# apple/ml-unigen

Measured on AMD Instinct MI355X. Metric: train-step samples/s (1.5B, 256^2 img), higher is better.
Workload: dtype bf16

## Files before the change

### include/unigen_hip.h

```cpp
#ifndef UNIGEN_HIP_H
#define UNIGEN_HIP_H

#include <stdint.h>
#include <hip/hip_runtime_api.h>

#ifdef __cplusplus
extern "C" {
#endif

#define UG_ABI_VERSION 7

const char* ug_last_error(void);
int ug_abi_version(void);

typedef struct ug_handle ug_handle;
int ug_create(ug_handle** out);
int ug_destroy(ug_handle* h);

#define UG_EPI_BF16 0
#define UG_EPI_F32 1
#define UG_EPI_RESID 2
int ug_gemm_bf16(const ug_handle* h, const void* A, int64_t lda, int a_kmajor, const void* B, int64_t ldb, int b_kmajor,
                 void* C, int64_t ldc, int64_t M, int64_t N, int64_t K, int epilogue, const void* bias,
                 const float* resid, int64_t ldr, int beta, const float* alpha_dev, int policy, hipStream_t stream);
#define UG_GEMM_NARROW_EPILOGUE 0x100
#define UG_GEMM_ONE_BARRIER 0x200
#define UG_GEMM_TWO_BARRIERS 0x400
#define UG_GEMM_POLICY_AUTO_BITS 0xff

int ug_cast_f32_bf16(const float* in, void* out, int64_t n, hipStream_t stream);

int ug_gemm_bf16_swiglu_bwd(const ug_handle* h, const void* dy, int64_t ld_dy, const void* w_down, int64_t ldw, const void* gu,
                            int64_t ld_gu, void* dgu, int64_t ld_dgu, int64_t M, int64_t I, int64_t K, hipStream_t stream);
int ug_gemm_set_fused_tile_height(int rows);
int ug_gemm_bf16_qkv_rope(const ug_handle* h, const void* x, int64_t ldx, const void* w, int64_t ldw, const void* bias, void* qkv,
                          int64_t ldq, int64_t M, int64_t N, int64_t K, const float* cos_tab, const float* sin_tab, int64_t L,
                          int64_t rope_cols, int head_dim, hipStream_t stream);
int ug_gemm_bf16_swiglu(const ug_handle* h, const void* x, int64_t ldx, const void* w_gate_up, int64_t ldw, void* gu,
                        int64_t ld_gu, void* act, int64_t ld_act, int64_t M, int64_t I, int64_t K, hipStream_t stream);

int ug_gemm_bf16_wgrad_group(int n, const void* const* dy, const int64_t* ld_dy, const void* const* x, const int64_t* ld_x,
                             float* const* dw, const int64_t* ld_dw, const int64_t* rows, const int64_t* cols,
                             const int* beta, const int64_t* K, hipStream_t stream);

int ug_rmsnorm_fwd(const float* x, const float* w, void* y, float* rstd, int64_t rows, int64_t cols,
                   float eps, int out_f32, hipStream_t stream);
int ug_rmsnorm_bwd(const void* dy, const float* x, const float* rstd, const float* w, float* dres,
                   float* dw, void* dres_bf16, int64_t rows, int64_t cols, hipStream_t stream);
int ug_rope(void* qkv, const float* cos_tab, const float* sin_tab, int64_t tokens, int64_t L, int64_t ldq,
            int nheads, int head_dim, int backward, hipStream_t stream);
int ug_swiglu_fwd(const void* gate_up, void* act, int64_t tokens, int64_t I, hipStream_t stream);
int ug_swiglu_bwd(const void* gate_up, const void* dact, void* dgate_up, int64_t tokens, int64_t I,
                  hipStream_t stream);
int ug_gelu(const void* x, const void* dy_or_null, void* out, int64_t n, hipStream_t stream);
int ug_embed_fwd(const int64_t* ids, const float* W, float* out, int64_t tokens, int64_t H, int64_t V,
                 int* err_flag, hipStream_t stream);
int ug_embed_bwd(const int64_t* ids, const float* dout, float* dW, int64_t tokens, int64_t H, int64_t V,
                 hipStream_t stream);
int ug_embed_bwd_sorted(const int64_t* ids_sorted, const int64_t* order, const float* rows, float* dW, int64_t n,
                        int64_t H, int64_t V, float scale, hipStream_t stream);
int ug_gather_rows_bf16(const void* in, int64_t ld_in, const int64_t* idx, void* out, int64_t ld_out,
                        int64_t n, int64_t C, int scatter, hipStream_t stream);
int ug_colsum_bf16(const void* in, int64_t ld, float* out, int64_t R, int64_t C, hipStream_t stream);

#define UG_MASK_F32 0
#define UG_MASK_BF16 1
#define UG_MASK_I64 2
#define UG_MASK_BOOL 3
int ug_attn_mask_compress(const void* mask, int mask_dtype, int64_t stride_b, int64_t stride_row,
                          uint64_t* bits, uint8_t* tileany, int64_t B, int64_t L, int* err_flag,
                          hipStream_t stream);
int ug_attn_mask_causal(const uint8_t* key_valid , uint64_t* bits, uint8_t* tileany,
                        int64_t B, int64_t L, hipStream_t stream);
int ug_attn_fwd(const void* q, const void* k, const void* v, int64_t ldq, void* o,
                int64_t ldo, float* lse, const uint64_t* bits, const uint8_t* tileany, int64_t B, int64_t L,
                int64_t Lp, int H, int HKV, int head_dim, float scale, hipStream_t stream);
int ug_attn_bwd(const void* q, const void* k, const void* v, int64_t ldq,
                const void* o, const void* dout, int64_t ldo, const float* lse,
                float* delta, void* dq, void* dk, void* dv, int64_t ldg, const uint64_t* bits,
                const uint8_t* tileany, int64_t B, int64_t L, int64_t Lp, int H, int HKV, int head_dim,
                float scale, float* dkv_ws, const float* rope_cos, const float* rope_sin, float* dbias_qkv, hipStream_t stream);

int ug_kv_store(const void* qkv, int64_t ldq, int64_t k_col, int64_t v_col, void* cache_k, void* cache_v,
                int64_t rows, int64_t L, int HKV, int head_dim, int64_t Tmax, const int* pos_dev, int pos_host,
                hipStream_t stream);
int ug_rope_at(void* qkv, const float* cos_tab, const float* sin_tab, int64_t rows, int64_t ldq, int nheads,
               int head_dim, const int* pos_dev, int64_t max_pos, hipStream_t stream);
int ug_attn_decode(const void* q, int64_t ldq, const void* cache_k, const void* cache_v, const uint8_t* key_valid,
                   void* o, int64_t ldo, int64_t rows, int H, int HKV, int head_dim, int64_t Tmax,
                   const int* len_dev, float scale, hipStream_t stream);
int ug_attn_prefill_cached(const void* q, int64_t ldq, const void* cache_k, const void* cache_v,
                           const uint8_t* key_valid , void* o, int64_t ldo,
                           int64_t rows, int64_t S, int64_t P, int H, int HKV, int head_dim, int64_t Tmax,
                           float scale, hipStream_t stream);
int ug_gemv_bf16(const void* x, int64_t ldx, int64_t R, const void* W, int64_t ldw, float* acc, int64_t acc_stride_r,
                 int64_t acc_stride_n, int64_t N, int64_t K, hipStream_t stream);
int ug_decode_finish_resid_norm(float* acc, int64_t ldacc, float* x, const float* w, void* xn, int64_t rows, int64_t cols,
                                float eps, int* pos_inc, int* len_inc, hipStream_t stream);
int ug_decode_gemv(const void* x, int64_t ldx, int64_t R, const void* W, int64_t ldw, float* acc, int64_t ldacc, int64_t N,
                   int64_t K, float* zero0, int64_t n0, float* zero1, int64_t n1, float* ss_zero, hipStream_t stream);
int ug_decode_gemv_resid_norm(const float* x_in, const float* pending, int64_t ld_pending, const float* norm_w, float* x_out,
                              float* ss_out, int64_t R, const void* W, int64_t ldw, float* acc, int64_t ldacc, int64_t N,
                              int64_t K, float* zero0, int64_t n0, float* zero1, int64_t n1, float* ss_zero,
                              hipStream_t stream);
int ug_decode_gemv_swiglu(const float* gate_up_acc, int64_t ld_gu, const float* ss_in, float eps, int64_t norm_cols, int64_t R,
                          const void* W, int64_t ldw, float* acc, int64_t ldacc, int64_t N, int64_t K, float* zero0, int64_t n0,
                          float* zero1, int64_t n1, float* ss_zero, hipStream_t stream);
int ug_attn_decode_fused(const float* acc_qkv, int64_t ldacc, const float* ss_in, float eps, int64_t norm_cols, const void* bias,
                         const float* cos_tab, const float* sin_tab, const int* pos_dev, void* cache_k, void* cache_v,
                         const uint8_t* key_valid, void* o, int64_t ldo, int64_t rows, int H, int HKV, int head_dim,
                         int64_t Tmax, int64_t max_pos, float scale, hipStream_t stream);
int ug_decode_sw_supported(int64_t hidden, int64_t inter, int64_t q_dim, int head_dim);
int ug_decode_sw_kblock(const void* x, int64_t ldx, int64_t R, const void* W, int64_t ldw, float* acc, int64_t ldacc, int64_t N, int64_t K,
                        float* zero0, int64_t n0, float* zero1, int64_t n1, float* ss_zero, hipStream_t stream);
int ug_decode_sw_resid(const void* x, int64_t ldx, int64_t R, const void* W, int64_t ldw, int64_t N, int64_t K, float* h,
                       hipStream_t stream);
int ug_decode_sw_gate_up(const float* h, const float* pend, int64_t ld_pend, float* x_out, const float* norm_w, float eps, int64_t R,
                         int64_t H, const void* W, int64_t ldw, int64_t I, void* act, int64_t ld_act, hipStream_t stream);
int ug_decode_sw_head(const float* h, const float* pend, int64_t ld_pend, float* x_out, const float* norm_w, float eps, int64_t R,
                      int64_t H, const void* W, int64_t ldw, int64_t N, float* logits, int64_t ld_logits, int* pos_inc, int* len_inc,
                      hipStream_t stream);
int ug_skinny_finish(const float* acc, const void* bias, void* out_bf16, float* resid, int64_t M, int64_t N,
                     int mode, hipStream_t stream);
int ug_gemv_bf16_ord(const void* x, int64_t ldx, int64_t R, const void* W, int64_t ldw, float* part, int64_t ldpart, int64_t part_stride,
                     int64_t N, int64_t K, hipStream_t stream);
int ug_skinny_finish_ord(const float* parts, int64_t nparts, int64_t part_stride, const void* bias, void* out_bf16, float* out_f32,
                         float* resid, int64_t M, int64_t N, hipStream_t stream);
int ug_decode_gemv_resid_norm_ord(const float* x_in, const float* pend_parts, int64_t ld_pending, int64_t npend, const float* norm_w,
                                  float* x_out, float* ss_part, int64_t R, const void* W, int64_t ldw, float* part, int64_t ldpart,
                                  int64_t N, int64_t K, hipStream_t stream);
int ug_attn_decode_fused_ord(const float* qkv_part, int64_t ldpart, int64_t nparts, const float* ss_part, float eps, int64_t norm_cols,
                             const void* bias, const float* cos_tab, const float* sin_tab, const int* pos_dev, void* cache_k,
                             void* cache_v, const uint8_t* key_valid, void* o, int64_t ldo, int64_t rows, int H, int HKV, int head_dim,
                             int64_t Tmax, int64_t max_pos, float scale, hipStream_t stream);
int ug_decode_sw_kblock_ord(const void* x, int64_t ldx, int64_t R, const void* W, int64_t ldw, float* part, int64_t ldpart, int64_t N,
                            int64_t K, hipStream_t stream);
int ug_decode_finish_resid_norm_ord(const float* parts, int64_t ldp, int64_t nparts, float* x, const float* w, void* xn, int64_t rows,
                                    int64_t cols, float eps, int* pos_inc, int* len_inc, hipStream_t stream);

int ug_t2i_assemble(const int64_t* text_ids, const int64_t* text_offsets, const int64_t* conv_start, int64_t n_start,
                    const int64_t* conv_end, int64_t n_end, const int64_t* image_in, const int64_t* image_labels, int64_t B,
                    int64_t n_image, int64_t max_seq_len, int64_t pad_id, int64_t soi_id, int64_t eoi_id, int64_t ignore_id,
                    int64_t* input_ids, int64_t* labels, uint8_t* attn01, hipStream_t stream);
int ug_attn_mask_from_ids(const int64_t* ids, int64_t B, int64_t L, int64_t pad_id, int64_t soi_id, int64_t eoi_id, int mode,
                          int* meta_ws, uint8_t* flags_ws, uint64_t* bits, uint8_t* tileany, hipStream_t stream);

int ug_maskgit_train_mask(const int64_t* tokens, const float* scores, const float* num_masked, int64_t B, int64_t n,
                          int64_t mask_id, int64_t ignore_id, int64_t* input_ids, int64_t* labels, hipStream_t stream);

int ug_maskgit_step(const void* logits, int64_t ld, int64_t V, int64_t N, int64_t n, int cfg, float guidance_scale,
                    const float* u_sample, const float* u_conf, const int64_t* cur_ids, int64_t mask_id, int64_t id_offset,
                    int64_t mask_len_sched, float temperature, int64_t* sampled, float* sel_ws, int64_t* next_cur,
                    int64_t* next_ids, uint8_t* masking_out, hipStream_t stream);

int ug_maskgit_step_ex(const void* logits, int64_t ld, int64_t V, int64_t N, int64_t n, int cfg, float guidance_scale,
                       const float* u_sample, const float* u_conf, const int64_t* cur_ids, int64_t mask_id, int64_t id_offset,
                       int64_t mask_len_sched, float temperature, float sample_temperature, int64_t top_k, float top_p, float min_p,
                       int64_t* sampled, float* sel_ws, int64_t* next_cur, int64_t* next_ids, uint8_t* masking_out, float* logp,
                       float* stats, hipStream_t stream);

int ug_ar_sample(float* acc, int64_t ldacc, int64_t bsz, int64_t V, float guidance_scale, float temperature, int greedy,
                 const float* uniforms, const int* pos_dev, int64_t pos0, int64_t nsteps, const float* embed, int64_t ld_embed,
                 int64_t H, int64_t id_offset, int64_t* tok, int* out_tokens, float* x, hipStream_t stream);

int ug_ar_sample_filtered(float* acc, int64_t ldacc, int64_t bsz, int64_t V, float guidance_scale, float temperature, int greedy,
                          const float* uniforms, const int* pos_dev, int64_t pos0, int64_t nsteps, const float* embed,
                          int64_t ld_embed, int64_t H, int64_t id_offset, int64_t* tok, int* out_tokens, float* x, int64_t top_k,
                          float top_p, float min_p, float* stats, hipStream_t stream);

int ug_ar_sample_logp(float* acc, int64_t ldacc, int64_t bsz, int64_t V, float guidance_scale, float temperature, int greedy,
                      const float* uniforms, const int* pos_dev, int64_t pos0, int64_t nsteps, const float* embed, int64_t ld_embed,
                      int64_t H, int64_t id_offset, int64_t* tok, int* out_tokens, float* x, float* logp, hipStream_t stream);
int ug_ar_sample_filtered_logp(float* acc, int64_t ldacc, int64_t bsz, int64_t V, float guidance_scale, float temperature, int greedy,
                               const float* uniforms, const int* pos_dev, int64_t pos0, int64_t nsteps, const float* embed,
                               int64_t ld_embed, int64_t H, int64_t id_offset, int64_t* tok, int* out_tokens, float* x, int64_t top_k,
                               float top_p, float min_p, float* stats, float* logp, hipStream_t stream);

int ug_text_pick(float* logits, int64_t ld, int64_t R, int64_t V, int clear, const int64_t* stop_ids, int64_t n_stop, int64_t pad_id,
                 const float* embed, int64_t ld_embed, int64_t embed_rows, int64_t H, int* state, int64_t nsteps, int64_t* tok,
                 int* out_tokens, int* lengths, float* x, hipStream_t stream);

int ug_text_sample_workspace_ints(int64_t R);

int ug_text_sample(float* logits, int64_t ld, int64_t R, int64_t V, int clear, float temperature, int64_t top_k, float top_p,
                   const float* uniforms, int* workspace, float* stats, const int64_t* stop_ids, int64_t n_stop, int64_t pad_id,
                   const float* embed, int64_t ld_embed, int64_t embed_rows, int64_t H, int* state, int64_t nsteps, int64_t* tok,
                   int* out_tokens, int* lengths, float* x, hipStream_t stream);

int ug_text_pick_logp(float* logits, int64_t ld, int64_t R, int64_t V, int clear, const int64_t* stop_ids, int64_t n_stop, int64_t pad_id,
                      const float* embed, int64_t ld_embed, int64_t embed_rows, int64_t H, int* state, int64_t nsteps, int64_t* tok,
                      int* out_tokens, int* lengths, float* x, float* logp, hipStream_t stream);
int ug_text_sample_logp(float* logits, int64_t ld, int64_t R, int64_t V, int clear, float temperature, int64_t top_k, float top_p,
                        const float* uniforms, int* workspace, float* stats, const int64_t* stop_ids, int64_t n_stop, int64_t pad_id,
                        const float* embed, int64_t ld_embed, int64_t embed_rows, int64_t H, int* state, int64_t nsteps, int64_t* tok,
                        int* out_tokens, int* lengths, float* x, float* logp, hipStream_t stream);


int ug_text_seen_mark(int* seen, int64_t ld_words, const int64_t* ids, int64_t ld_ids, int64_t R, int64_t L, const uint8_t* valid,
                      int64_t V, hipStream_t stream);

int ug_text_penalize(float* logits, int64_t ld, int64_t R, int64_t V, float penalty, int* seen, int64_t ld_words, const int64_t* tok,
                     hipStream_t stream);


int ug_text_constrain(float* logits, int64_t ld, int64_t R, int64_t V, const void* bias, int64_t n_bias, int64_t min_new,
                      const int64_t* stop_ids, int64_t n_stop, int64_t ngram, const int* hist, int64_t ld_hist, const int* hist_len,
                      const int* out_tokens, int64_t nsteps, const int* state, hipStream_t stream);

int ug_text_stop_seq(const int* seq_ids, const int* seq_off, int64_t ns, int64_t n_ids, const int* out_tokens, int64_t nsteps, int64_t R,
                     int* state, int* lengths, hipStream_t stream);

int ug_ce_fwd(const void* logits, int64_t ld, int64_t R, int64_t V, const int64_t* labels,
              int64_t ignore_index, float* lse, float* loss_row, float* logp_label, float* loss_and_count,
              hipStream_t stream);
int ug_ce_bwd(void* logits_inout, int64_t ld, int64_t R, int64_t V, const int64_t* labels,
              int64_t ignore_index, const float* lse, const float* loss_and_count, const float* gscale,
              const float* row_scale, hipStream_t stream);

int ug_head_score_ws_bytes(int64_t R, int64_t V);
int ug_head_score(const void* x, int64_t ldx, int64_t R, const void* W, int64_t ldw, int64_t V, int64_t K,
                  const int64_t* labels, int64_t ignore_index, void* ws, float* logp, float* lse, int64_t* best, float* best_logit,
                  hipStream_t stream);

int ug_adamw_flat(float* p, const float* g, float* m, float* v, void* p_bf16, int64_t n, float lr,
                  float beta1, float beta2, float eps, float weight_decay, int64_t step, float grad_scale,
                  int max_blocks ,
                  hipStream_t stream);
int ug_adamw_flat_dev(float* p, const float* g, float* m, float* v, void* p_bf16, int64_t n, float lr,
                      float beta1, float beta2, float eps, float weight_decay, int64_t step, float grad_scale,
                      const float* grad_factor, int max_blocks, hipStream_t stream);

int ug_sumsq_spans_f32(const int64_t* spans, int64_t n_spans, double* partials, int blocks, int accum, hipStream_t stream);
int ug_clip_finish(const double* partials, int64_t n_partials, float max_norm, float grad_scale, float* result, hipStream_t stream);
int ug_scale_spans_f32(const int64_t* spans, int64_t n_spans, const float* coef, int blocks, hipStream_t stream);

int ug_grad_pack_bf16(const float* in, void* out_bf16, int64_t n, float scale, hipStream_t stream);
int ug_zero_ranges_f32(float* buf, const int64_t* ranges, int64_t n_ranges, int64_t max_len, hipStream_t stream);
int ug_grad_unpack_bf16(const void* in_bf16, float* out, int64_t n, hipStream_t stream);
int ug_grad_sum_shards_bf16(const void* shards_bf16, int world, int64_t stride, void* out_bf16, int64_t n, float scale,
                            hipStream_t stream);

typedef struct ug_comm ug_comm;
#define UG_COMM_ID_BYTES 128
#define UG_COMM_FP32 0
#define UG_COMM_BF16_FP32ACC 1
#define UG_COMM_BF16 2
#define UG_COMM_FP32_RSAG 3
int ug_comm_unique_id(void* id128);
int ug_comm_init(ug_comm** out, int world, int rank, const void* id128, int64_t max_bucket_elems);
int ug_comm_allreduce_bucket(ug_comm* comm, float* grad, int64_t n, int mode, hipStream_t producer);
int ug_comm_allgather(ug_comm* comm, const void* send, void* recv, int64_t bytes_per_rank, hipStream_t producer);
int ug_comm_wait(ug_comm* comm, hipStream_t consumer);
int ug_comm_destroy(ug_comm* comm);
int64_t ug_comm_bytes_on_wire(const ug_comm* comm);

int ug_conv2d_f32(const float* x, const float* w_packed, const float* bias, const float* residual, float* y,
                  int64_t B, int Hin, int Win, int Cin, int Cout, int cout_pad, int ksize, int stride,
                  int pad_top, int pad_left, int Hout, int Wout, int upsample2x, hipStream_t stream);
int ug_conv_split_weights(const float* w_packed, uint16_t* w_split, int taps, int Cin, int cout_pad, hipStream_t stream);
int ug_amax_f32(const float* x, int64_t rows, int64_t cols, int64_t ld, float* out_amax, hipStream_t stream);
int ug_amax_f32_into_zeroed(const float* x, int64_t rows, int64_t cols, int64_t ld, float* out_amax, hipStream_t stream);
int ug_conv2d_split(const float* x, const float* x_amax, const uint16_t* w_split, const float* bias, const float* residual,
                    float* y, int64_t B, int Hin, int Win, int Cin, int Cout, int cout_pad, int ksize, int stride,
                    int pad_top, int pad_left, int Hout, int Wout, int upsample2x, double* out_stats, int out_groups,
                    hipStream_t stream);
int ug_conv3x3_split(const float* x, const float* x_amax, const uint16_t* w_split, const float* bias, const float* residual,
                     float* y, int64_t B, int H, int W, int Cin, int Cout, int cout_pad, const float* gn_mu_rstd,
                     const float* gn_gamma, const float* gn_beta, int gn_groups, int gn_swish, double* out_stats, int out_groups,
                     hipStream_t stream);
int ug_groupnorm_finalize(const double* stats, float* mu_rstd, int64_t B, int64_t HW, int C, int groups, float eps,
                          hipStream_t stream);
int ug_groupnorm_stats(const float* x, double* stats_ws, float* mu_rstd, int64_t B, int64_t HW, int C, int groups,
                       float eps, hipStream_t stream);
int ug_siglip_attn_f32(const float* qkv, int64_t ld, const float* qkv_amax, float* out, int64_t ldo, int64_t B, int64_t T,
                       int H, int head_dim, float scale, hipStream_t stream);
int ug_linear_split(const float* x, int64_t ldx, const float* x_amax, const uint16_t* w_split, const float* bias,
                    const float* residual, int64_t ldres, float* y, int64_t ldy, int64_t M, int64_t N, int64_t K, int n_pad,
                    int act, hipStream_t stream);
int ug_gemm_f32(const float* A, int64_t lda, int64_t stride_a, const float* B, int64_t ldb, int64_t stride_b,
                int b_is_nk, float* C, int64_t ldc, int64_t stride_c, int64_t M, int64_t N, int64_t K,
                int64_t batch, float alpha, hipStream_t stream);
int ug_gemm_f32_nested(const float* A, int64_t lda, int64_t sa_in, int64_t sa_out, const float* B, int64_t ldb,
                       int64_t sb_in, int64_t sb_out, int b_is_nk, float* C, int64_t ldc, int64_t sc_in, int64_t sc_out,
                       int64_t M, int64_t N, int64_t K, int64_t batch_in, int64_t batch_out, float alpha,
                       hipStream_t stream);
int ug_groupnorm_swish(const float* x, const float* gamma, const float* beta, float* y, double* stats_ws,
                       int64_t B, int64_t HW, int C, int groups, float eps, int apply_swish, hipStream_t stream);
int ug_softmax_rows_f32(float* x, int64_t rows, int64_t cols, int64_t ld, float scale, hipStream_t stream);
int ug_linear_f32(const float* x, int64_t ldx, const float* W, int64_t ldw, const float* bias,
                  const float* residual, int64_t ldres, float* y, int64_t ldy, int64_t M, int64_t N, int64_t K,
                  int act, hipStream_t stream);
int ug_layernorm_f32(const float* x, const float* gamma, const float* beta, float* y, int64_t rows, int64_t cols,
                     float eps, hipStream_t stream);
int ug_layernorm_bwd_f32(const float* dy, const float* x, const float* gamma, const float* dres_in, float* dx, float* dgamma,
                         float* dbeta, int64_t rows, int64_t cols, float eps, hipStream_t stream);
int ug_gelu_tanh_f32(const float* pre, const float* dy_or_null, float* out, int64_t n, hipStream_t stream);
int ug_softmax_bwd_rows_f32(const float* P, float* dP, int64_t rows, int64_t cols, int64_t ld, float scale, hipStream_t stream);
int ug_colsum_f32(const float* x, int64_t ld, float* out, int64_t rows, int64_t cols, hipStream_t stream);
int ug_transpose_f32(const float* in, int64_t ld_in, int64_t stride_in, float* out, int64_t ld_out, int64_t stride_out,
                     int64_t rows, int64_t cols, int64_t batch, hipStream_t stream);
int ug_nchw_to_nhwc(const float* in, float* out, int64_t B, int C, int64_t HW, int c_pad, hipStream_t stream);
int ug_nhwc_to_nchw(const float* in, float* out, int64_t B, int C, int64_t HW, int c_pad, hipStream_t stream);
int ug_lfq_pack(const float* z, int64_t ldz, int64_t* idx, int64_t n, int nbits, hipStream_t stream);
int ug_lfq_unpack(const int64_t* idx, float* z, int64_t n, int nbits, int* err_flag, hipStream_t stream);

int ug_probe_layouts(float* out, int64_t n_floats, hipStream_t stream);

#ifdef __cplusplus
}
#endif
#endif
```

### ml-unigen_amd/csrc/elementwise.hip

```cpp
#include <algorithm>
#include "common.h"
#include "unigen_hip.h"

namespace {

typedef unsigned int ntu4_t __attribute__((ext_vector_type(4)));
typedef unsigned int ntu2_t __attribute__((ext_vector_type(2)));
template <int NT, typename T>
__device__ __forceinline__ T ld_stream(const T* p) {
  static_assert(sizeof(T) == 16 || sizeof(T) == 8, "ld_stream: 8- or 16-byte accesses");
  if constexpr ((NT & 2) && sizeof(T) == 16) return __builtin_bit_cast(T, __builtin_nontemporal_load(reinterpret_cast<const ntu4_t*>(p)));
  else if constexpr ((NT & 2) && sizeof(T) == 8) return __builtin_bit_cast(T, __builtin_nontemporal_load(reinterpret_cast<const ntu2_t*>(p)));
  else return *p;
}
template <int NT, typename T>
__device__ __forceinline__ void st_stream(T* p, T v) {
  static_assert(sizeof(T) == 16 || sizeof(T) == 8, "st_stream: 8- or 16-byte accesses");
  if constexpr ((NT & 1) && sizeof(T) == 16) __builtin_nontemporal_store(__builtin_bit_cast(ntu4_t, v), reinterpret_cast<ntu4_t*>(p));
  else if constexpr ((NT & 1) && sizeof(T) == 8) __builtin_nontemporal_store(__builtin_bit_cast(ntu2_t, v), reinterpret_cast<ntu2_t*>(p));
  else *p = v;
}
constexpr int NT_ADAMW = 3, NT_RMSNORM_BWD = 0, NT_SWIGLU_BWD = 3, NT_SWIGLU_FWD = 2;

template <bool OUT_F32>
__global__ __launch_bounds__(256) void rmsnorm_fwd_kernel(const float* __restrict__ x, const float* __restrict__ w,
                                                          void* __restrict__ y, float* __restrict__ rstd,
                                                          int rows, int cols, float eps) {
  const int row = blockIdx.x * 4 + (threadIdx.x >> 6);
  const int lane = threadIdx.x & 63;
  if (row >= rows) return;
  const float4* xr = reinterpret_cast<const float4*>(x + (int64_t)row * cols);
  const int nv = cols >> 2;
  float ss = 0.f;
  for (int i = lane; i < nv; i += 64) {
    const float4 v = xr[i];
    ss += v.x * v.x + v.y * v.y + v.z * v.z + v.w * v.w;
  }
  ss = wave_sum(ss);
  const float r = rsqrtf(ss / (float)cols + eps);
  if (lane == 0 && rstd) rstd[row] = r;
  const float4* wr = reinterpret_cast<const float4*>(w);
  for (int i = lane; i < nv; i += 64) {
    const float4 v = xr[i], g = wr[i];
    const float o0 = g.x * (v.x * r), o1 = g.y * (v.y * r), o2 = g.z * (v.z * r), o3 = g.w * (v.w * r);
    if constexpr (OUT_F32) {
      reinterpret_cast<float4*>(reinterpret_cast<float*>(y) + (int64_t)row * cols)[i] = make_float4(o0, o1, o2, o3);
    } else {
      uint2 o; o.x = pack_bf2(o0, o1); o.y = pack_bf2(o2, o3);
      reinterpret_cast<uint2*>(reinterpret_cast<bf16_t*>(y) + (int64_t)row * cols)[i] = o;
    }
  }
}

template <bool OUT_F32, int NV>
__global__ __launch_bounds__(256) void rmsnorm_fwd_reg_kernel(const float* __restrict__ x, const float* __restrict__ w,
                                                              void* __restrict__ y, float* __restrict__ rstd,
                                                              int rows, int cols, float eps, int rows_per_wave) {
  const int lane = threadIdx.x & 63;
  const int nv = cols >> 2;
  const float4* wr = reinterpret_cast<const float4*>(w);
  const int r0 = (blockIdx.x * 4 + (threadIdx.x >> 6)) * rows_per_wave;
  for (int row = r0; row < min(rows, r0 + rows_per_wave); ++row) {
    const float4* xr = reinterpret_cast<const float4*>(x + (int64_t)row * cols);
    float4 v[NV];
    float ss = 0.f;
#pragma unroll
    for (int k = 0; k < NV; ++k) {
      const int i = lane + k * 64;
      if (i < nv) { v[k] = xr[i]; }
    }
#pragma unroll
    for (int k = 0; k < NV; ++k) {
      const int i = lane + k * 64;
      if (i < nv) ss += v[k].x * v[k].x + v[k].y * v[k].y + v[k].z * v[k].z + v[k].w * v[k].w;
    }
    ss = wave_sum(ss);
    const float r = rsqrtf(ss / (float)cols + eps);
    if (lane == 0 && rstd) rstd[row] = r;
#pragma unroll
    for (int k = 0; k < NV; ++k) {
      const int i = lane + k * 64;
      if (i < nv) {
        const float4 g = wr[i];
        const float o0 = g.x * (v[k].x * r), o1 = g.y * (v[k].y * r), o2 = g.z * (v[k].z * r), o3 = g.w * (v[k].w * r);
        if constexpr (OUT_F32) {
          reinterpret_cast<float4*>(reinterpret_cast<float*>(y) + (int64_t)row * cols)[i] = make_float4(o0, o1, o2, o3);
        } else {
          uint2 o; o.x = pack_bf2(o0, o1); o.y = pack_bf2(o2, o3);
          reinterpret_cast<uint2*>(reinterpret_cast<bf16_t*>(y) + (int64_t)row * cols)[i] = o;
        }
      }
    }
  }
}

constexpr int RN_MAXV = 8;
template <int NV, int NT>
__global__ __launch_bounds__(256) void rmsnorm_bwd_kernel(const bf16_t* __restrict__ dy, const float* __restrict__ x,
                                                          const float* __restrict__ rstd, const float* __restrict__ w,
                                                          float* __restrict__ dres, float* __restrict__ dw,
                                                          bf16_t* __restrict__ dres_bf16, int rows, int cols,
                                                          int rows_per_block) {
  __shared__ float red[4][64 * 4];
  const int wave = threadIdx.x >> 6, lane = threadIdx.x & 63;
  const int nv = cols >> 2;
  float4 dwp[NV];
#pragma unroll
  for (int k = 0; k < NV; ++k) dwp[k] = make_float4(0.f, 0.f, 0.f, 0.f);
  const float4* wr = reinterpret_cast<const float4*>(w);
  const int r0 = blockIdx.x * rows_per_block;
  const int r1 = min(rows, r0 + rows_per_block);
  for (int row = r0 + wave; row < r1; row += 4) {
    const float4* xr = reinterpret_cast<const float4*>(x + (int64_t)row * cols);
    const uint2* dyr = reinterpret_cast<const uint2*>(dy + (int64_t)row * cols);
    float4* dr = reinterpret_cast<float4*>(dres + (int64_t)row * cols);
    const float r = rstd[row];
    float4 g[NV], xh[NV], acc[NV];
    uint2 dyv[NV];
    float dot = 0.f;
#pragma unroll
    for (int k = 0; k < NV; ++k) {
      const int i = lane + k * 64;
      if (i < nv) { xh[k] = ld_stream<NT>(xr + i); dyv[k] = ld_stream<NT>(dyr + i); }
    }
#pragma unroll
    for (int k = 0; k < NV; ++k) {
      const int i = lane + k * 64;
      if (i < nv) acc[k] = dr[i];
    }
#pragma unroll
    for (int k = 0; k < NV; ++k) {
      const int i = lane + k * 64;
      if (i < nv) {
        const float4 v = xh[k], ww = wr[i]; const uint2 d = dyv[k];
        const float d0 = bf2f(d.x & 0xffff), d1 = bf2f(d.x >> 16), d2 = bf2f(d.y & 0xffff), d3 = bf2f(d.y >> 16);
        xh[k] = make_float4(v.x * r, v.y * r, v.z * r, v.w * r);
        g[k] = make_float4(d0 * ww.x, d1 * ww.y, d2 * ww.z, d3 * ww.w);
        dot += g[k].x * xh[k].x + g[k].y * xh[k].y + g[k].z * xh[k].z + g[k].w * xh[k].w;
        dwp[k].x += d0 * xh[k].x; dwp[k].y += d1 * xh[k].y; dwp[k].z += d2 * xh[k].z; dwp[k].w += d3 * xh[k].w;
      }
    }
    dot = wave_sum(dot) / (float)cols;
#pragma unroll
    for (int k = 0; k < NV; ++k) {
      const int i = lane + k * 64;
      if (i < nv) {
        float4 o = acc[k];
        o.x += r * (g[k].x - xh[k].x * dot); o.y += r * (g[k].y - xh[k].y * dot);
        o.z += r * (g[k].z - xh[k].z * dot); o.w += r * (g[k].w - xh[k].w * dot);
        st_stream<NT>(dr + i, o);
        if (dres_bf16) {
          uint2 ob; ob.x = pack_bf2(o.x, o.y); ob.y = pack_bf2(o.z, o.w);
          reinterpret_cast<uint2*>(dres_bf16 + (int64_t)row * cols)[i] = ob;
        }
      }
    }
  }
#pragma unroll
  for (int k = 0; k < NV; ++k) {
    if (k * 64 >= nv) break;
    __syncthreads();
    red[wave][lane * 4 + 0] = dwp[k].x; red[wave][lane * 4 + 1] = dwp[k].y;
    red[wave][lane * 4 + 2] = dwp[k].z; red[wave][lane * 4 + 3] = dwp[k].w;
    __syncthreads();
    const int c = threadIdx.x;
    const int col = k * 256 + c;
    if constexpr (!(NT & 4))
      if (col < cols) atomicAdd(dw + col, red[0][c] + red[1][c] + red[2][c] + red[3][c]);
  }
}

template <bool BWD>
__global__ __launch_bounds__(256) void rope_kernel(bf16_t* __restrict__ qkv, const float* __restrict__ cs,
                                                   const float* __restrict__ sn, int64_t tokens, int L, int ldq,
                                                   int nheads, int hd) {
#pragma clang fp contract(off)
  const int half = hd >> 1, per_head = half >> 2;
  const int64_t total = tokens * nheads * per_head;
  for (int64_t idx = blockIdx.x * (int64_t)blockDim.x + threadIdx.x; idx < total; idx += (int64_t)gridDim.x * blockDim.x) {
    const int p4 = (int)(idx % per_head);
    const int h = (int)((idx / per_head) % nheads);
    const int64_t t = idx / ((int64_t)per_head * nheads);
    const int pos = (int)(t % L);
    bf16_t* base = qkv + t * ldq + h * hd + p4 * 4;
    const uint2 lo = *reinterpret_cast<const uint2*>(base);
    const uint2 hi = *reinterpret_cast<const uint2*>(base + half);
    const float4 c = *reinterpret_cast<const float4*>(cs + (int64_t)pos * half + p4 * 4);
    const float4 s = *reinterpret_cast<const float4*>(sn + (int64_t)pos * half + p4 * 4);
    const float x1[4] = {bf2f(lo.x & 0xffff), bf2f(lo.x >> 16), bf2f(lo.y & 0xffff), bf2f(lo.y >> 16)};
    const float x2[4] = {bf2f(hi.x & 0xffff), bf2f(hi.x >> 16), bf2f(hi.y & 0xffff), bf2f(hi.y >> 16)};
    const float cc[4] = {c.x, c.y, c.z, c.w}, ss[4] = {s.x, s.y, s.z, s.w};
    float o1[4], o2[4];
#pragma unroll
    for (int k = 0; k < 4; ++k) {
      const float a1 = x1[k] * cc[k], a2 = x2[k] * cc[k];
      const float b1 = x2[k] * ss[k], b2 = x1[k] * ss[k];
      if constexpr (!BWD) { o1[k] = a1 - b1; o2[k] = a2 + b2; }
      else { o1[k] = a1 + b1; o2[k] = a2 - b2; }
    }
    uint2 olo, ohi;
    olo.x = pack_bf2(o1[0], o1[1]); olo.y = pack_bf2(o1[2], o1[3]);
    ohi.x = pack_bf2(o2[0], o2[1]); ohi.y = pack_bf2(o2[2], o2[3]);
    *reinterpret_cast<uint2*>(base) = olo;
    *reinterpret_cast<uint2*>(base + half) = ohi;
  }
}

__device__ __forceinline__ float silu_f(float g) { return silu_train(g); }

template <int NT>
__global__ __launch_bounds__(256) void swiglu_fwd_kernel(const bf16_t* __restrict__ gu, bf16_t* __restrict__ act,
                                                         int64_t tokens, int I) {
  const int per_row = I >> 3;
  const int64_t total = tokens * per_row;
  for (int64_t idx = blockIdx.x * (int64_t)blockDim.x + threadIdx.x; idx < total; idx += (int64_t)gridDim.x * blockDim.x) {
    const int64_t t = idx / per_row; const int c = (int)(idx % per_row) * 8;
    const bf16x8_t g = ld_stream<NT>(reinterpret_cast<const bf16x8_t*>(gu + t * 2 * I + c));
    const bf16x8_t u = ld_stream<NT>(reinterpret_cast<const bf16x8_t*>(gu + t * 2 * I + I + c));
    bf16x8_t o;
#pragma unroll
    for (int k = 0; k < 8; ++k) {
      const float s = bf2f(f2bf(silu_f(bf2f((bf16_t)g[k]))));
      o[k] = (short)f2bf(s * bf2f((bf16_t)u[k]));
    }
    st_stream<NT>(reinterpret_cast<bf16x8_t*>(act + t * I + c), o);
  }
}

template <int NT>
__global__ __launch_bounds__(256) void swiglu_bwd_kernel(const bf16_t* __restrict__ gu, const bf16_t* __restrict__ dact,
                                                         bf16_t* __restrict__ dgu, int64_t tokens, int I) {
  const int per_row = I >> 3;
  const int64_t total = tokens * per_row;
  for (int64_t idx = blockIdx.x * (int64_t)blockDim.x + threadIdx.x; idx < total; idx += (int64_t)gridDim.x * blockDim.x) {
    const int64_t t = idx / per_row; const int c = (int)(idx % per_row) * 8;
    const bf16x8_t g = ld_stream<NT>(reinterpret_cast<const bf16x8_t*>(gu + t * 2 * I + c));
    const bf16x8_t u = ld_stream<NT>(reinterpret_cast<const bf16x8_t*>(gu + t * 2 * I + I + c));
    const bf16x8_t d = ld_stream<NT>(reinterpret_cast<const bf16x8_t*>(dact + t * I + c));
    bf16x8_t og, ou;
#pragma unroll
    for (int k = 0; k < 8; ++k) {
      float dg_, du_;
      swiglu_bwd_elem(bf2f((bf16_t)g[k]), bf2f((bf16_t)u[k]), bf2f((bf16_t)d[k]), dg_, du_);
      ou[k] = (short)f2bf(du_);
      og[k] = (short)f2bf(dg_);
    }
    st_stream<NT>(reinterpret_cast<bf16x8_t*>(dgu + t * 2 * I + c), og);
    st_stream<NT>(reinterpret_cast<bf16x8_t*>(dgu + t * 2 * I + I + c), ou);
  }
}

__global__ __launch_bounds__(256) void gelu_kernel(const bf16_t* __restrict__ x, const bf16_t* __restrict__ dy,
                                                   bf16_t* __restrict__ out, int64_t n8) {
  for (int64_t i = blockIdx.x * (int64_t)blockDim.x + threadIdx.x; i < n8; i += (int64_t)gridDim.x * blockDim.x) {
    const bf16x8_t v = reinterpret_cast<const bf16x8_t*>(x)[i];
    bf16x8_t g, o;
    if (dy) g = reinterpret_cast<const bf16x8_t*>(dy)[i];
#pragma unroll
    for (int k = 0; k < 8; ++k) {
      const float f = bf2f((bf16_t)v[k]);
      const float cdf = 0.5f * (1.f + erff(f * 0.70710678118654752f));
      if (!dy) o[k] = (short)f2bf(f * cdf);
      else o[k] = (short)f2bf(bf2f((bf16_t)g[k]) * (cdf + f * 0.3989422804014327f * __expf(-0.5f * f * f)));
    }
    reinterpret_cast<bf16x8_t*>(out)[i] = o;
  }
}

__global__ __launch_bounds__(256) void embed_fwd_kernel(const int64_t* __restrict__ ids, const float* __restrict__ W,
                                                        float* __restrict__ out, int64_t tokens, int H, int64_t V,
                                                        int* __restrict__ err) {
  const int per_row = H >> 2;
  const int64_t total = tokens * per_row;
  for (int64_t idx = blockIdx.x * (int64_t)blockDim.x + threadIdx.x; idx < total; idx += (int64_t)gridDim.x * blockDim.x) {
    const int64_t t = idx / per_row; const int c = (int)(idx % per_row);
    int64_t id = ids[t];
    if (id < 0 || id >= V) { if (err) atomicOr(err, 1); id = 0; }
    reinterpret_cast<float4*>(out + t * H)[c] = reinterpret_cast<const float4*>(W + id * H)[c];
  }
}

// ... 263 lines not shown
    sh[threadIdx.x] = i < n ? partials[i] : 0.0;
    __syncthreads();
    if (threadIdx.x == 0) {
      const int c = min(256, n - base);
      for (int k = 0; k < c; ++k) s += sh[k];
    }
    __syncthreads();
  }
  if (threadIdx.x == 0) {
    const float total = (float)(sqrt(s) * fabs((double)grad_scale));
    const float raw = max_norm / (total + 1e-6f);
    const float coef = raw > 1.f ? 1.f : raw;
    result[0] = total;
    result[1] = coef;
    result[2] = grad_scale * coef;
    result[3] = (total != total || fabsf(total) == INFINITY) ? 1.f : 0.f;
    reinterpret_cast<double*>(result)[2] = s;
    result[6] = 0.f;
    result[7] = 0.f;
  }
}

__global__ __launch_bounds__(256) void scale_spans_kernel(const int64_t* __restrict__ spans, int n_spans, const float* __restrict__ coef) {
  const float c = *coef;
  if (c == 1.0f) return;
  const int64_t stride = (int64_t)gridDim.x * 256;
  for (int r = 0; r < n_spans; ++r) {
    const SpanGeom sp = span_geom(spans, r);
    const unsigned vb = (blockIdx.x + (unsigned)r) % gridDim.x;
    if (vb == 0) {
      const int64_t t = threadIdx.x;
      const int64_t e = t < sp.head ? t : sp.tail0 + (t - sp.head);
      if (e < sp.n) sp.base[e] *= c;
    }
    for (int64_t i = (int64_t)vb * 256 + threadIdx.x; i < sp.body4; i += stride) {
      sp.body[i] = sp.body[i] * c;
    }
  }
}

__global__ __launch_bounds__(256) void cast_f32_bf16_kernel(const float* __restrict__ in, bf16_t* __restrict__ out, int64_t n) {
  const int64_t n4 = n >> 2;
  for (int64_t i = blockIdx.x * (int64_t)blockDim.x + threadIdx.x; i < n4; i += (int64_t)gridDim.x * blockDim.x) {
    const float4 v = reinterpret_cast<const float4*>(in)[i];
    uint2 o; o.x = pack_bf2(v.x, v.y); o.y = pack_bf2(v.z, v.w);
    reinterpret_cast<uint2*>(out)[i] = o;
  }
  const int64_t ti = (n4 << 2) + blockIdx.x * (int64_t)blockDim.x + threadIdx.x;
  if (ti < n) out[ti] = f2bf(in[ti]);
}

__global__ __launch_bounds__(256) void grad_pack_kernel(const float* __restrict__ in, bf16_t* __restrict__ out, int64_t n, float scale) {
  const int64_t n8 = n >> 3;
  for (int64_t i = blockIdx.x * (int64_t)blockDim.x + threadIdx.x; i < n8; i += (int64_t)gridDim.x * blockDim.x) {
    const float4 a = reinterpret_cast<const float4*>(in)[2 * i], b = reinterpret_cast<const float4*>(in)[2 * i + 1];
    uint4 o;
    o.x = pack_bf2(a.x * scale, a.y * scale); o.y = pack_bf2(a.z * scale, a.w * scale);
    o.z = pack_bf2(b.x * scale, b.y * scale); o.w = pack_bf2(b.z * scale, b.w * scale);
    reinterpret_cast<uint4*>(out)[i] = o;
  }
  const int64_t ti = (n8 << 3) + blockIdx.x * (int64_t)blockDim.x + threadIdx.x;
  if (ti < n) out[ti] = f2bf(in[ti] * scale);
}
__global__ __launch_bounds__(256) void grad_sum_shards_kernel(const bf16_t* __restrict__ shards, int world, int64_t stride,
                                                              bf16_t* __restrict__ out, int64_t n, float scale) {
  const int64_t n8 = n >> 3;
  for (int64_t i = blockIdx.x * (int64_t)blockDim.x + threadIdx.x; i < n8; i += (int64_t)gridDim.x * blockDim.x) {
    float acc[8] = {0.f, 0.f, 0.f, 0.f, 0.f, 0.f, 0.f, 0.f};
    for (int r = 0; r < world; ++r) {
      const uint4 v = reinterpret_cast<const uint4*>(shards + r * stride)[i];
      acc[0] += __uint_as_float(v.x << 16); acc[1] += __uint_as_float(v.x & 0xffff0000u);
      acc[2] += __uint_as_float(v.y << 16); acc[3] += __uint_as_float(v.y & 0xffff0000u);
      acc[4] += __uint_as_float(v.z << 16); acc[5] += __uint_as_float(v.z & 0xffff0000u);
      acc[6] += __uint_as_float(v.w << 16); acc[7] += __uint_as_float(v.w & 0xffff0000u);
    }
    uint4 o;
    o.x = pack_bf2(acc[0] * scale, acc[1] * scale); o.y = pack_bf2(acc[2] * scale, acc[3] * scale);
    o.z = pack_bf2(acc[4] * scale, acc[5] * scale); o.w = pack_bf2(acc[6] * scale, acc[7] * scale);
    reinterpret_cast<uint4*>(out)[i] = o;
  }
  const int64_t ti = (n8 << 3) + blockIdx.x * (int64_t)blockDim.x + threadIdx.x;
  if (ti < n) {
    float a = 0.f;
    for (int r = 0; r < world; ++r) a += bf2f(shards[r * stride + ti]);
    out[ti] = f2bf(a * scale);
  }
}
__global__ __launch_bounds__(256) void grad_unpack_kernel(const bf16_t* __restrict__ in, float* __restrict__ out, int64_t n) {
  const int64_t n8 = n >> 3;
  for (int64_t i = blockIdx.x * (int64_t)blockDim.x + threadIdx.x; i < n8; i += (int64_t)gridDim.x * blockDim.x) {
    const uint4 v = reinterpret_cast<const uint4*>(in)[i];
    float4 a, b;
    a.x = __uint_as_float(v.x << 16); a.y = __uint_as_float(v.x & 0xffff0000u);
    a.z = __uint_as_float(v.y << 16); a.w = __uint_as_float(v.y & 0xffff0000u);
    b.x = __uint_as_float(v.z << 16); b.y = __uint_as_float(v.z & 0xffff0000u);
    b.z = __uint_as_float(v.w << 16); b.w = __uint_as_float(v.w & 0xffff0000u);
    reinterpret_cast<float4*>(out)[2 * i] = a; reinterpret_cast<float4*>(out)[2 * i + 1] = b;
  }
  const int64_t ti = (n8 << 3) + blockIdx.x * (int64_t)blockDim.x + threadIdx.x;
  if (ti < n) out[ti] = bf2f(in[ti]);
}

__global__ __launch_bounds__(256) void gather_rows_kernel(const bf16_t* __restrict__ in, int64_t ld_in,
                                                          const int64_t* __restrict__ idx, bf16_t* __restrict__ out,
                                                          int64_t ld_out, int64_t n, int C, int scatter) {
  const int per_row = C >> 3;
  const int64_t total = n * per_row;
  for (int64_t i = blockIdx.x * (int64_t)blockDim.x + threadIdx.x; i < total; i += (int64_t)gridDim.x * blockDim.x) {
    const int64_t r = i / per_row; const int c = (int)(i % per_row) * 8;
    const int64_t src = scatter ? r : idx[r], dst = scatter ? idx[r] : r;
    *reinterpret_cast<bf16x8_t*>(out + dst * ld_out + c) = *reinterpret_cast<const bf16x8_t*>(in + src * ld_in + c);
  }
}

inline int grid_for(int64_t work_items, int block = 256, int cap = 256 * 8) {
  int64_t g = (work_items + block - 1) / block;
  if (g < 1) g = 1;
  if (g > cap) g = cap;
  return (int)g;
}

}

extern "C" int ug_rmsnorm_fwd(const float* x, const float* w, void* y, float* rstd, int64_t rows, int64_t cols,
                              float eps, int out_f32, hipStream_t st) {
  UG_REQUIRE(rows > 0 && cols > 0 && cols % 4 == 0, "ug_rmsnorm_fwd: cols=%ld must be a positive multiple of 4", (long)cols);
  UG_REQUIRE(ug_aligned16(x) && ug_aligned16(w) && ug_aligned16(y), "ug_rmsnorm_fwd: pointers must be 16B aligned");
  dim3 grid((unsigned)((rows + 3) / 4)), block(256);
  constexpr int reg = 1;
  if (reg > 0 && cols <= 2048 && !out_f32) {
    dim3 g2((unsigned)((rows + 4 * reg - 1) / (4 * reg)));
    hipLaunchKernelGGL((rmsnorm_fwd_reg_kernel<false, 8>), g2, block, 0, st, x, w, y, rstd, (int)rows, (int)cols, eps, reg);
  } else if (out_f32) hipLaunchKernelGGL(rmsnorm_fwd_kernel<true>, grid, block, 0, st, x, w, y, rstd, (int)rows, (int)cols, eps);
  else hipLaunchKernelGGL(rmsnorm_fwd_kernel<false>, grid, block, 0, st, x, w, y, rstd, (int)rows, (int)cols, eps);
  UG_CHECK_LAUNCH("ug_rmsnorm_fwd");
  return UG_OK;
}

extern "C" int ug_rmsnorm_bwd(const void* dy, const float* x, const float* rstd, const float* w, float* dres,
                              float* dw, void* dres_bf16, int64_t rows, int64_t cols, hipStream_t st) {
  UG_REQUIRE(rows > 0 && cols > 0 && cols % 4 == 0 && cols <= 64 * 4 * RN_MAXV,
             "ug_rmsnorm_bwd: cols=%ld unsupported (multiple of 4, <= %d)", (long)cols, 64 * 4 * RN_MAXV);
  UG_REQUIRE(ug_aligned16(x) && ug_aligned16(w) && ug_aligned16(dres) && ((uintptr_t)dy & 7) == 0,
             "ug_rmsnorm_bwd: pointers must be aligned");
  const int rpb = (int)std::max<int64_t>(16, ((rows + 479) / 480 + 3) / 4 * 4);
  dim3 grid((unsigned)((rows + rpb - 1) / rpb)), block(256);
  UG_REQUIRE(((uintptr_t)dres_bf16 & 7) == 0, "ug_rmsnorm_bwd: dres_bf16 must be 8-byte aligned");
  hipLaunchKernelGGL((rmsnorm_bwd_kernel<RN_MAXV, NT_RMSNORM_BWD>), grid, block, 0, st, (const bf16_t*)dy, x, rstd, w, dres, dw,
                     (bf16_t*)dres_bf16, (int)rows, (int)cols, rpb);
  UG_CHECK_LAUNCH("ug_rmsnorm_bwd");
  return UG_OK;
}

extern "C" int ug_rope(void* qkv, const float* cos_tab, const float* sin_tab, int64_t tokens, int64_t L, int64_t ldq,
                       int nheads, int head_dim, int backward, hipStream_t st) {
  UG_REQUIRE(tokens > 0 && L > 0 && tokens % L == 0, "ug_rope: tokens=%ld must be a multiple of L=%ld", (long)tokens, (long)L);
  UG_REQUIRE(head_dim % 8 == 0 && ldq % 4 == 0, "ug_rope: head_dim must be a multiple of 8");
  UG_REQUIRE(((uintptr_t)qkv & 7) == 0 && ug_aligned16(cos_tab) && ug_aligned16(sin_tab), "ug_rope: alignment");
  const int64_t total = tokens * nheads * (head_dim / 8);
  dim3 grid(grid_for(total)), block(256);
  if (backward) hipLaunchKernelGGL(rope_kernel<true>, grid, block, 0, st, (bf16_t*)qkv, cos_tab, sin_tab, tokens, (int)L, (int)ldq, nheads, head_dim);
  else hipLaunchKernelGGL(rope_kernel<false>, grid, block, 0, st, (bf16_t*)qkv, cos_tab, sin_tab, tokens, (int)L, (int)ldq, nheads, head_dim);
  UG_CHECK_LAUNCH("ug_rope");
  return UG_OK;
}

extern "C" int ug_swiglu_fwd(const void* gate_up, void* act, int64_t tokens, int64_t I, hipStream_t st) {
  UG_REQUIRE(tokens > 0 && I % 8 == 0, "ug_swiglu_fwd: I=%ld must be a multiple of 8", (long)I);
  UG_REQUIRE(ug_aligned16(gate_up) && ug_aligned16(act), "ug_swiglu_fwd: alignment");
  dim3 grid(grid_for(tokens * (I / 8))), block(256);
  hipLaunchKernelGGL(swiglu_fwd_kernel<NT_SWIGLU_FWD>, grid, block, 0, st, (const bf16_t*)gate_up, (bf16_t*)act, tokens, (int)I);
  UG_CHECK_LAUNCH("ug_swiglu_fwd");
  return UG_OK;
}

extern "C" int ug_swiglu_bwd(const void* gate_up, const void* dact, void* dgate_up, int64_t tokens, int64_t I,
                             hipStream_t st) {
  UG_REQUIRE(tokens > 0 && I % 8 == 0, "ug_swiglu_bwd: I=%ld must be a multiple of 8", (long)I);
  UG_REQUIRE(ug_aligned16(gate_up) && ug_aligned16(dact) && ug_aligned16(dgate_up), "ug_swiglu_bwd: alignment");
  dim3 grid(grid_for(tokens * (I / 8))), block(256);
  hipLaunchKernelGGL(swiglu_bwd_kernel<NT_SWIGLU_BWD>, grid, block, 0, st, (const bf16_t*)gate_up, (const bf16_t*)dact, (bf16_t*)dgate_up, tokens, (int)I);
  UG_CHECK_LAUNCH("ug_swiglu_bwd");
  return UG_OK;
}

extern "C" int ug_gelu(const void* x, const void* dy_or_null, void* out, int64_t n, hipStream_t st) {
  UG_REQUIRE(n > 0 && n % 8 == 0 && ug_aligned16(x) && ug_aligned16(out), "ug_gelu: n must be a multiple of 8, 16B-aligned buffers");
  dim3 grid(grid_for(n / 8)), block(256);
  hipLaunchKernelGGL(gelu_kernel, grid, block, 0, st, (const bf16_t*)x, (const bf16_t*)dy_or_null, (bf16_t*)out, n / 8);
  UG_CHECK_LAUNCH("ug_gelu");
  return UG_OK;
}

extern "C" int ug_embed_fwd(const int64_t* ids, const float* W, float* out, int64_t tokens, int64_t H, int64_t V,
                            int* err_flag, hipStream_t st) {
  UG_REQUIRE(tokens > 0 && H % 4 == 0, "ug_embed_fwd: H must be a multiple of 4");
  dim3 grid(grid_for(tokens * (H / 4))), block(256);
  hipLaunchKernelGGL(embed_fwd_kernel, grid, block, 0, st, ids, W, out, tokens, (int)H, V, err_flag);
  UG_CHECK_LAUNCH("ug_embed_fwd");
  return UG_OK;
}

extern "C" int ug_embed_bwd(const int64_t* ids, const float* dout, float* dW, int64_t tokens, int64_t H, int64_t V,
                            hipStream_t st) {
  UG_REQUIRE(tokens > 0 && H > 0, "ug_embed_bwd: empty");
  dim3 grid(grid_for(tokens * H)), block(256);
  hipLaunchKernelGGL(embed_bwd_kernel, grid, block, 0, st, ids, dout, dW, tokens, (int)H, V);
  UG_CHECK_LAUNCH("ug_embed_bwd");
  return UG_OK;
}

extern "C" int ug_embed_bwd_sorted(const int64_t* ids_sorted, const int64_t* order, const float* rows, float* dW, int64_t n,
                                   int64_t H, int64_t V, float scale, hipStream_t st) {
  UG_REQUIRE(ids_sorted && order && rows && dW && n > 0 && H > 0 && H % 4 == 0 && n < (1ll << 31) && ug_aligned16(rows) && ug_aligned16(dW),
             "ug_embed_bwd_sorted: need sorted ids, their permutation, 16B-aligned rows / table and H %% 4 == 0");
  hipLaunchKernelGGL(embed_bwd_sorted_kernel, dim3((unsigned)n), dim3(256), 0, st, ids_sorted, order, rows, dW, n, (int)H, V, scale);
  UG_CHECK_LAUNCH("ug_embed_bwd_sorted");
  return UG_OK;
}

extern "C" int ug_colsum_bf16(const void* in, int64_t ld, float* out, int64_t R, int64_t C, hipStream_t st) {
  UG_REQUIRE(R > 0 && C > 0, "ug_colsum_bf16: empty");
  const int rpb = 256;
  dim3 grid((unsigned)((C + 63) / 64), (unsigned)((R + rpb - 1) / rpb)), block(256);
  hipLaunchKernelGGL(colsum_kernel, grid, block, 0, st, (const bf16_t*)in, ld, out, (int)R, (int)C, rpb);
  UG_CHECK_LAUNCH("ug_colsum_bf16");
  return UG_OK;
}

static int adamw_flat_launch(float* p, const float* g, float* m, float* v, void* p_bf16, int64_t n, float lr,
                             float beta1, float beta2, float eps, float weight_decay, int64_t step, float grad_scale,
                             const float* gfac, int max_blocks, hipStream_t st) {
  UG_REQUIRE(n > 0 && step >= 1, "ug_adamw_flat: n=%ld step=%ld", (long)n, (long)step);
  UG_REQUIRE(ug_aligned16(p) && ug_aligned16(g) && ug_aligned16(m) && ug_aligned16(v) && ((uintptr_t)p_bf16 & 7) == 0,
             "ug_adamw_flat: buffers must be 16B aligned");
  const double bc1 = 1.0 - pow((double)beta1, (double)step);
  const double bc2 = 1.0 - pow((double)beta2, (double)step);
  const dim3 block(256);
  if (max_blocks == 0 && n < (1LL << 29)) max_blocks = 256;
  if (max_blocks > 0) {
    dim3 lgrid(grid_for(n / 2 + 1, 256, max_blocks));
    if (n < (1LL << 29))
      hipLaunchKernelGGL(adamw_lean2_kernel<NT_ADAMW>, lgrid, block, 0, st, p, g, m, v, (bf16_t*)p_bf16, (uint32_t)n, lr, beta1, beta2, eps, weight_decay,
                         (float)bc1, (float)sqrt(bc2), grad_scale, gfac);
    else
      hipLaunchKernelGGL(adamw_lean_kernel<NT_ADAMW>, lgrid, block, 0, st, p, g, m, v, (bf16_t*)p_bf16, n, lr, beta1, beta2, eps, weight_decay,
                         (float)bc1, (float)sqrt(bc2), grad_scale, gfac);
    UG_CHECK_LAUNCH("ug_adamw_flat(lean)");
    return UG_OK;
  }
  hipLaunchKernelGGL(adamw_kernel<NT_ADAMW>, dim3(grid_for(n / 4 + 1)), block, 0, st, p, g, m, v, (bf16_t*)p_bf16, n, lr, beta1, beta2, eps,
                     weight_decay, (float)bc1, (float)sqrt(bc2), grad_scale, gfac);
  UG_CHECK_LAUNCH("ug_adamw_flat");
  return UG_OK;
}

extern "C" int ug_adamw_flat(float* p, const float* g, float* m, float* v, void* p_bf16, int64_t n, float lr,
                             float beta1, float beta2, float eps, float weight_decay, int64_t step, float grad_scale,
                             int max_blocks, hipStream_t st) {
  return adamw_flat_launch(p, g, m, v, p_bf16, n, lr, beta1, beta2, eps, weight_decay, step, grad_scale, nullptr, max_blocks, st);
}

extern "C" int ug_adamw_flat_dev(float* p, const float* g, float* m, float* v, void* p_bf16, int64_t n, float lr,
                                 float beta1, float beta2, float eps, float weight_decay, int64_t step, float grad_scale,
                                 const float* grad_factor, int max_blocks, hipStream_t st) {
  UG_REQUIRE(((uintptr_t)grad_factor & 3) == 0, "ug_adamw_flat_dev: grad_factor must be a 4-byte aligned device address (or null)");
  return adamw_flat_launch(p, g, m, v, p_bf16, n, lr, beta1, beta2, eps, weight_decay, step, grad_scale, grad_factor, max_blocks, st);
}

extern "C" int ug_sumsq_spans_f32(const int64_t* spans, int64_t n_spans, double* partials, int blocks, int accum, hipStream_t st) {
  UG_REQUIRE(spans && partials && ((uintptr_t)spans & 7) == 0 && ((uintptr_t)partials & 7) == 0 && n_spans > 0 && n_spans < 65536 &&
                 blocks > 0 && blocks <= 4096 && (accum == 0 || accum == 1),
             "ug_sumsq_spans_f32: a device span table of 1..65535 spans, a partial buffer of `blocks` doubles, 1 <= blocks <= 4096 and "
             "accum 0 (fp64) or 1 (fp32 chains) required (n_spans=%ld blocks=%d accum=%d)", (long)n_spans, blocks, accum);
  if (accum == 0) hipLaunchKernelGGL(sumsq_spans_kernel<false>, dim3((unsigned)blocks), dim3(256), 0, st, spans, (int)n_spans, partials);
  else hipLaunchKernelGGL(sumsq_spans_kernel<true>, dim3((unsigned)blocks), dim3(256), 0, st, spans, (int)n_spans, partials);
  UG_CHECK_LAUNCH("ug_sumsq_spans_f32");
  return UG_OK;
}

extern "C" int ug_clip_finish(const double* partials, int64_t n_partials, float max_norm, float grad_scale, float* result, hipStream_t st) {
  UG_REQUIRE(partials && result && ((uintptr_t)partials & 7) == 0 && ug_aligned16(result) && n_partials > 0 && n_partials <= 8192,
             "ug_clip_finish: 1..8192 fp64 partials and a 16-byte aligned result block of 8 fp32 words required (n_partials=%ld)", (long)n_partials);
  UG_REQUIRE(max_norm == max_norm && grad_scale == grad_scale, "ug_clip_finish: max_norm and grad_scale must not be NaN");
  hipLaunchKernelGGL(clip_finish_kernel, dim3(1), dim3(256), 0, st, partials, (int)n_partials, max_norm, grad_scale, result);
  UG_CHECK_LAUNCH("ug_clip_finish");
  return UG_OK;
}

extern "C" int ug_scale_spans_f32(const int64_t* spans, int64_t n_spans, const float* coef, int blocks, hipStream_t st) {
  UG_REQUIRE(spans && coef && ((uintptr_t)spans & 7) == 0 && ((uintptr_t)coef & 3) == 0 && n_spans > 0 && n_spans < 65536 && blocks >= 0 &&
                 blocks <= 4096,
             "ug_scale_spans_f32: a device span table of 1..65535 spans, a device scalar and 0 <= blocks <= 4096 required (n_spans=%ld blocks=%d)",
             (long)n_spans, blocks);
  hipLaunchKernelGGL(scale_spans_kernel, dim3((unsigned)(blocks ? blocks : 256 * 8)), dim3(256), 0, st, spans, (int)n_spans, coef);
  UG_CHECK_LAUNCH("ug_scale_spans_f32");
  return UG_OK;
}

extern "C" int ug_cast_f32_bf16(const float* in, void* out, int64_t n, hipStream_t st) {
  UG_REQUIRE(n > 0 && ug_aligned16(in) && ((uintptr_t)out & 7) == 0, "ug_cast_f32_bf16: bad args");
  dim3 grid(grid_for(n / 4 + 1)), block(256);
  hipLaunchKernelGGL(cast_f32_bf16_kernel, grid, block, 0, st, in, (bf16_t*)out, n);
  UG_CHECK_LAUNCH("ug_cast_f32_bf16");
  return UG_OK;
}
// ... 52 lines not shown
```

### ml-unigen_amd/csrc/loss.hip

```cpp
#include "common.h"
#include "unigen_hip.h"

namespace {

__global__ __launch_bounds__(256) void ce_fwd_kernel(const bf16_t* __restrict__ logits, int64_t ld, int V,
                                                     const int64_t* __restrict__ labels, int64_t ignore_index,
                                                     float* __restrict__ lse_out, float* __restrict__ loss_row,
                                                     float* __restrict__ logp_label) {
  __shared__ float red[4];
  const int row = blockIdx.x;
  const bf16_t* x = logits + (int64_t)row * ld;
  const int nv = V >> 3;
  float m = -INFINITY, s = 0.f;
  for (int i = threadIdx.x; i < nv; i += 256) {
    const bf16x8_t v = *reinterpret_cast<const bf16x8_t*>(x + i * 8);
    float f[8], mx = -INFINITY;
#pragma unroll
    for (int k = 0; k < 8; ++k) { f[k] = bf2f((bf16_t)v[k]); mx = fmaxf(mx, f[k]); }
    const float mn = fmaxf(m, mx);
    float acc = 0.f;
#pragma unroll
    for (int k = 0; k < 8; ++k) acc += __expf(f[k] - mn);
    s = s * __expf(m - mn) + acc;
    m = mn;
  }
  for (int c = (nv << 3) + threadIdx.x; c < V; c += 256) {
    const float f = bf2f(x[c]);
    const float mn = fmaxf(m, f);
    s = s * __expf(m - mn) + __expf(f - mn);
    m = mn;
  }
  const float M = block_max<4>(m, red);
  const float part = (m == -INFINITY) ? 0.f : s * __expf(m - M);
  const float S = block_sum<4>(part, red);
  if (threadIdx.x == 0) {
    const float lse = M + logf(S);
    lse_out[row] = lse;
    const int64_t lab = labels ? labels[row] : ignore_index;
    float lr = 0.f, lp = 0.f;
    if (lab != ignore_index && lab >= 0 && lab < V) { lp = bf2f(x[lab]) - lse; lr = -lp; }
    if (loss_row) loss_row[row] = lr;
    if (logp_label) logp_label[row] = lp;
  }
}

__global__ __launch_bounds__(256) void ce_reduce_kernel(const float* __restrict__ loss_row,
                                                        const int64_t* __restrict__ labels, int64_t ignore_index,
                                                        int R, float* __restrict__ out) {
  __shared__ float red[4];
  float s = 0.f, c = 0.f;
  for (int i = threadIdx.x; i < R; i += 256) {
    if (labels[i] != ignore_index) { s += loss_row[i]; c += 1.f; }
  }
  const float S = block_sum<4>(s, red);
  const float C = block_sum<4>(c, red);
  if (threadIdx.x == 0) { out[0] = S / C; out[1] = C; }
}

__global__ __launch_bounds__(256) void ce_bwd_kernel(bf16_t* __restrict__ logits, int64_t ld, int V,
                                                     const int64_t* __restrict__ labels, int64_t ignore_index,
                                                     const float* __restrict__ lse, const float* __restrict__ loss_cnt,
                                                     const float* __restrict__ gscale, const float* __restrict__ row_scale) {
  const int row = blockIdx.x;
  bf16_t* x = logits + (int64_t)row * ld;
  const int64_t lab = labels[row];
  const bool valid = (lab != ignore_index);
  const float sc = !valid ? 0.f : row_scale ? row_scale[row] : (gscale ? *gscale : 1.f) / loss_cnt[1];
  const float l = lse[row];
  const int nvp = (int)(ld >> 3);
  for (int i = threadIdx.x; i < nvp; i += 256) {
    bf16x8_t v = *reinterpret_cast<const bf16x8_t*>(x + i * 8);
#pragma unroll
    for (int k = 0; k < 8; ++k) {
      const int c = i * 8 + k;
      float g = 0.f;
      if (valid && c < V) g = (__expf(bf2f((bf16_t)v[k]) - l) - (c == lab ? 1.f : 0.f)) * sc;
      v[k] = (short)f2bf(g);
    }
    *reinterpret_cast<bf16x8_t*>(x + i * 8) = v;
  }
}

}

extern "C" int ug_ce_fwd(const void* logits, int64_t ld, int64_t R, int64_t V, const int64_t* labels,
                         int64_t ignore_index, float* lse, float* loss_row, float* logp_label, float* loss_and_count,
                         hipStream_t st) {
  UG_REQUIRE(R > 0 && V > 0 && ld >= V && ld % 8 == 0, "ug_ce_fwd: need ld>=V and ld%%8==0 (ld=%ld V=%ld)", (long)ld, (long)V);
  UG_REQUIRE(ug_aligned16(logits), "ug_ce_fwd: logits must be 16B aligned");
  hipLaunchKernelGGL(ce_fwd_kernel, dim3((unsigned)R), dim3(256), 0, st, (const bf16_t*)logits, ld, (int)V, labels,
                     ignore_index, lse, loss_row, logp_label);
  UG_CHECK_LAUNCH("ug_ce_fwd");
  if (loss_and_count) {
    UG_REQUIRE(labels && loss_row, "ug_ce_fwd: loss reduction needs labels and loss_row");
    hipLaunchKernelGGL(ce_reduce_kernel, dim3(1), dim3(256), 0, st, loss_row, labels, ignore_index, (int)R, loss_and_count);
    UG_CHECK_LAUNCH("ug_ce_fwd(reduce)");
  }
  return UG_OK;
}

extern "C" int ug_ce_bwd(void* logits_inout, int64_t ld, int64_t R, int64_t V, const int64_t* labels,
                         int64_t ignore_index, const float* lse, const float* loss_and_count, const float* gscale,
                         const float* row_scale, hipStream_t st) {
  UG_REQUIRE(R > 0 && V > 0 && ld >= V && ld % 8 == 0, "ug_ce_bwd: need ld>=V and ld%%8==0");
  UG_REQUIRE(ug_aligned16(logits_inout) && labels && lse && (loss_and_count || row_scale), "ug_ce_bwd: bad pointers");
  hipLaunchKernelGGL(ce_bwd_kernel, dim3((unsigned)R), dim3(256), 0, st, (bf16_t*)logits_inout, ld, (int)V, labels,
                     ignore_index, lse, loss_and_count, gscale, row_scale);
  UG_CHECK_LAUNCH("ug_ce_bwd");
  return UG_OK;
}
```

### ml-unigen_amd/models/unigen.py

```python
import collections
import dataclasses
import json
import math
import os
import time
import weakref
from typing import Optional

import torch

from unigen_hip import ops
from unigen_hip.lib import UniGenHipError
from unigen_hip.modules import (HipProjector, HipQwen2ForCausalLM, LazyLogits, _CrossEntropyFn, _HeadLossFn, _LinearFn,
                                _TableEmbedFn)
from unigen_hip.qwen2 import Qwen2Dims

from .modeling_utils import ConfigMixin, ModelMixin, register_to_config
from .sampling import cosine_schedule, mask_by_random_topk

_KNOWN_LLM = {
    "qwen2.5-1.5b": dict(hidden_size=1536, intermediate_size=8960, num_hidden_layers=28, num_attention_heads=12,
                         num_key_value_heads=2, rope_theta=1000000.0, rms_norm_eps=1e-6, vocab_size=151936),
}

# ... 517 lines not shown
            finally:
                eng.require_grad_sync = prev
        return ctx()

    def _load_hf_llm_weights(self, llm_model_path, ckpt_base_path):
        path = llm_model_path
        if ckpt_base_path and not os.path.exists(str(path)):
            path = os.path.join(ckpt_base_path, os.path.basename(str(llm_model_path).rstrip("/")))
        files = [f for f in os.listdir(path) if f.endswith(".safetensors")]
        if not files:
            raise UniGenHipError(f"no *.safetensors under {path}")
        from safetensors.torch import load_file
        sd = {}
        for f in files:
            sd.update(load_file(os.path.join(path, f)))
        own = self.llm.state_dict()
        V_ckpt = sd["model.embed_tokens.weight"].shape[0]
        with torch.no_grad():
            for k, v in sd.items():
                if k == "lm_head.weight" or k not in own:
                    continue
                if k == "model.embed_tokens.weight":
                    n = min(V_ckpt, own[k].shape[0])
                    own[k][:n].copy_(v[:n])
                else:
                    own[k].copy_(v)

    def _set_gradient_checkpointing(self, module, value=False):
        self.gradient_checkpointing = True

    def resize_token_embeddings(self, vocab_size):
        self.vocab_size = vocab_size
        self.llm.resize_token_embeddings(self.vocab_size)
        self.output_size = self.vocab_size

    def init_vision_tower(self, vision_tower_name):
        from .multimodal_encoder.builder import get_vision_tower
        self.register_to_config(vision_tower_name=vision_tower_name)
        if self.config.ckpt_base_path:
            vision_tower_name = os.path.join(self.config.ckpt_base_path, os.path.basename(vision_tower_name.rstrip("/")))
        self.vision_tower = get_vision_tower(vision_tower_name, freeze=False)

    def add_vision_tower(self, config):
        vision_tower_name = config.model.vision_tower.name
        self.init_vision_tower(vision_tower_name)
        vt = self.vision_tower
        mm_input_dim = vt.config.hidden_size if hasattr(vt, 'config') else vt.hidden_size
        self.add_mm_projector(config.model.unigen.get('und_proj_depth', 2), mm_input_dim)

    def add_mm_projector(self, mlp_depth, mm_input_dim):
        self.register_to_config(w_und_encoder=True)
        self.register_to_config(mm_input_dim=mm_input_dim)
        self.register_to_config(und_proj_depth=mlp_depth)
        hidden = self.config.hidden_size
        layers = [torch.nn.Linear(mm_input_dim, hidden)]
        for _ in range(1, mlp_depth):
            layers += [torch.nn.GELU(), torch.nn.Linear(hidden, hidden)]
        from unigen_hip.modules import HipProjector
        self.mm_projector = HipProjector(*layers).to(self.llm.engine.device)

    def _use_gen(self):
        return self.config.get('gen_proj_depth', 0) > 0

    def get_gen_embed(self, img_tokens):
        if not self._use_gen():
            raise UniGenHipError("get_gen_embed needs a model built with gen_proj_depth > 0")
        eng = self.llm.engine
        e = _TableEmbedFn.apply(self.gen_embed.weight, img_tokens.to(eng.device), eng.err_flag)
        return self.gen_projector(e)

    def prepare_inputs_for_t2i(self, input_ids, num_vq_tokens):
        emb = self.llm.model.embed_tokens(input_ids)
        if self._use_gen():
            img = self.get_gen_embed(input_ids[:, -(num_vq_tokens + 1):-1].contiguous()).to(emb.dtype)
            emb = torch.cat([emb[:, :-(num_vq_tokens + 1)], img, emb[:, -1:]], dim=1)
        return emb

    def _img_head(self, hn):
        return _LinearFn.apply(hn, self.img_head.weight, None)

    def prepare_inputs_for_mmu(self, image_feats, spatial_shapes, input_ids, label_ids, prompt_template, input_ids_system=None):
        pt = prompt_template
        dev = input_ids.device
        B, Lt = input_ids.shape
        N = image_feats.shape[1]
        pad_id, ignore, max_len = pt.text_tokenizer.pad_token_id, pt.ignore_id, pt.max_seq_len
        sp = pt.sptids_dict
        head = ['<|mmu|>', '<|im_start|>', '<|soi|>'] if pt.task_token_first else ['<|im_start|>', '<|mmu|>', '<|soi|>']
        part1 = torch.tensor([int(sp[t]) for t in head], dtype=torch.long, device=dev)[None].expand(B, 3)
        if input_ids_system is not None:
            part1 = torch.cat([input_ids_system.to(dev).long(), part1], dim=1)
        part1 = part1.contiguous()
        L1 = part1.shape[1]
        n_img = (spatial_shapes[:, 0] * spatial_shapes[:, 1]).to(dev).long()
        emb_len = L1 + n_img + Lt + (N if self.training else int(n_img.max()) - n_img)
        lab_len = L1 + n_img + Lt + N

        def common_length(lens, what):
            lo, hi = int(lens.min()), int(lens.max())
            if lo < max_len and lo != hi:
                raise UniGenHipError(f"prepare_inputs_for_mmu: {what} rows shorter than max_seq_len differ in length")
            return min(lo, max_len)
        T, T_lab = common_length(emb_len, "embedding"), common_length(lab_len, "label")
        const = lambda v: torch.full((), int(v), dtype=torch.long, device=dev)

        p = torch.arange(T, device=dev)[None]
        q = p - L1 - n_img[:, None]
        is_img = (p >= L1) & (q < 0)
        text = torch.cat([const(sp['<|eoi|>']).expand(B, 1), input_ids[:, 1:].long()], dim=1)
        ids = torch.where((q >= 0) & (q < Lt), text.gather(1, q.clamp(0, Lt - 1)), const(pad_id))
        head_ids = torch.nn.functional.pad(part1, (0, max(0, T - L1)), value=pad_id)[:, :T]
        ids = torch.where(p < L1, head_ids, ids)
        image_embeds = self.mm_projector(image_feats)
        emb = self.llm.model.embed_tokens(ids)
        slot = (p - L1).clamp(0, N - 1).expand(B, T)
        img_rows = image_embeds.gather(1, slot[..., None].expand(B, T, image_embeds.shape[-1])).to(emb.dtype)
        full_embeddings = torch.where(is_img[..., None], img_rows, emb)

        if label_ids is None:
            label_ids = input_ids.clone()
        ql = torch.arange(T_lab, device=dev)[None] - L1 - n_img[:, None]
        labels = torch.where((ql >= 1) & (ql < Lt), label_ids.to(dev).long().gather(1, ql.clamp(0, Lt - 1)), const(ignore))
        labels = torch.where(labels == pad_id, const(ignore), labels)
        is_eos = labels == pt.eos_token_id
        has = is_eos.any(1)
        first_row = torch.where(has.any(), has.long().argmax(), const(-1))
        last_eos = T_lab - 1 - is_eos.flip(-1).long().argmax(1)
        cut = torch.where(torch.arange(B, device=dev) == first_row, last_eos, const(T_lab - 1))
        attention_mask = torch.arange(max_len, device=dev)[None] <= cut[:, None]
        return full_embeddings, attention_mask, labels, part1

    def _loss_rows(self, B, L, bt, blm, bmmu, n, mode, device, lm_start=None):
        lm0 = bt if lm_start is None else lm_start
        key = (B, L, bt, blm, bmmu, n, mode, lm0)
        if key not in self._loss_idx_cache:
            def grid(b0, b1, p0, p1):
                b = torch.arange(b0, b1, device=device)[:, None] * L
                return (b + torch.arange(p0, p1, device=device)[None, :]).reshape(-1)
            segs = []
            if mode == 'mask':
                segs.append((grid(0, bt, L - (n + 1), L - 1), 0))
            else:
                segs.append((grid(0, bt, L - (n + 2), L - 1), 1))
            if blm > 0:
                segs.append((grid(lm0, lm0 + blm, 0, L - 1), 1))
            if bmmu > 0:
                segs.append((grid(B - bmmu, B, 0, L - 1), 1))
            bounds, r = [], 0
            for ix, _ in segs:
                bounds.append((r, r + ix.numel()))
                r += ix.numel()
            idx = torch.cat([ix for ix, _ in segs]) if r > 0 else torch.zeros(0, dtype=torch.long, device=device)
            lab = torch.cat([ix + s for ix, s in segs]) if r > 0 else idx
            self._loss_idx_cache[key] = (idx, lab, bounds)
        return self._loss_idx_cache[key]

    def forward(
            self,
            input_ids: torch.LongTensor,
            input_embeddings: Optional[torch.Tensor] = None,
            attention_mask: Optional[torch.Tensor] = None,
            labels: Optional[torch.LongTensor] = None,
            label_smoothing: float = 0.0,
            batch_size_t2i: int = 0,
            batch_size_lm: int = 0,
            batch_size_mmu: int = 0,
            max_seq_length: int = 128,
            num_vq_tokens: int = 256,
            t2i_mode: str = 'mask',
            **kwargs,
    ):
        eng = self.llm.engine
        gen = self._use_gen() and batch_size_t2i > 0
        if gen and input_embeddings is None:
            n = num_vq_tokens
            safe = input_ids.clone()
            safe[:, -(n + 1):-1] = 0
            emb = self.llm.model.embed_tokens(safe)
            img = self.get_gen_embed(input_ids[:, -(n + 1):-1].contiguous()).to(emb.dtype)
            input_embeddings = torch.cat([emb[:, :-(n + 1)], img, emb[:, -1:]], dim=1)
        if input_embeddings is None:
            out = self.llm.model(input_ids=input_ids, attention_mask=attention_mask)
        else:
            out = self.llm.model(inputs_embeds=input_embeddings, attention_mask=attention_mask)
        hn = out.last_hidden_state
        if gen:
            return self._forward_gen_head(hn, labels, batch_size_t2i, batch_size_lm, batch_size_mmu, num_vq_tokens, t2i_mode)
        if labels is None:
            return LazyLogits(eng, hn)
        logits = LazyLogits(eng, hn.detach())
        B, L, _ = hn.shape
        idx, lab_idx, bounds = self._loss_rows(B, L, batch_size_t2i, batch_size_lm, batch_size_mmu, num_vq_tokens,
                                               t2i_mode, hn.device)
        nan = torch.full((), float("nan"), device=hn.device)
        if idx.numel() == 0:
            return logits, nan, 0., 0.
        lab = labels.to(hn.device).reshape(-1)[lab_idx].contiguous()
        live = [(s, b) for s, b in enumerate(bounds) if b[1] > b[0]]
        losses = _HeadLossFn.apply(eng._anchor, hn, eng, idx, lab, tuple(b for _, b in live))
        by_seg = {s: losses[j] for j, (s, _) in enumerate(live)}
        s = 0
        loss_t2i = by_seg.get(s, nan)
        s += 1
        loss_lm = 0.
        if batch_size_lm > 0:
            loss_lm = by_seg[s]
            s += 1
        loss_mmu = 0.
        if batch_size_mmu > 0:
            loss_mmu = by_seg[s]
        return logits, loss_t2i, loss_lm, loss_mmu

    def _forward_gen_head(self, hn, labels, bt, blm, bmmu, n, t2i_mode):
        eng = self.llm.engine
        B, L, _ = hn.shape
        img_logits = self._img_head(hn[:bt])
        if labels is None:
            return img_logits
        labels = labels.to(hn.device)
        C = self.img_output_size
        if t2i_mode == 'mask':
            lg, lb = img_logits[:, -(n + 1):-1], labels[:bt, -(n + 1):-1]
        else:
            lg, lb = img_logits[:, -(n + 2):-1], labels[:bt, -(n + 1):]
        loss_t2i = _CrossEntropyFn.apply(lg.reshape(-1, C), lb.reshape(-1).contiguous())
        loss_lm, loss_mmu = 0., 0.
        if blm > 0 or bmmu > 0:
            idx, lab_idx, bounds = self._loss_rows(B, L, 0, blm, bmmu, n, t2i_mode, hn.device, lm_start=bt)
            lab = labels.reshape(-1)[lab_idx].contiguous()
            live = [(s, b) for s, b in enumerate(bounds) if b[1] > b[0]]
            losses = _HeadLossFn.apply(eng._anchor, hn, eng, idx, lab, tuple(b for _, b in live))
            by_seg = {s: losses[j] for j, (s, _) in enumerate(live)}
            s = 1
            if blm > 0:
                loss_lm = by_seg[s]
                s += 1
            if bmmu > 0:
                loss_mmu = by_seg[s]
        return img_logits, loss_t2i, loss_lm, loss_mmu

    @torch.no_grad()
    def t2i_generate(
            self,
            input_ids: Optional[torch.LongTensor] = None,
            uncond_input_ids: Optional[torch.LongTensor] = None,
            input_embeddings: Optional[torch.Tensor] = None,
            uncond_input_embeddings: Optional[torch.Tensor] = None,
            attention_mask: Optional[torch.Tensor] = None,
            temperature: float = 1.0,
            timesteps: int = 18,
            guidance_scale: int = 0,
            noise_schedule=cosine_schedule,
            generator: Optional[torch.Generator] = None,
            image_token_num_per_image: int = 256,
            text_vocab_size: int = 151936,
            top_k: Optional[int] = 0,
            top_p: Optional[float] = 1.0,
            min_p: Optional[float] = 0.0,
            sampling_temperature: Optional[float] = 1.0,
            return_logprobs: bool = False,
            **kwargs,
    ):
        top_k = 0 if top_k is None else top_k
        top_p = 1.0 if top_p is None else float(top_p)
        min_p = 0.0 if min_p is None else float(min_p)
        sampling_temperature = 1.0 if sampling_temperature is None else float(sampling_temperature)
        if not (isinstance(top_k, int) and top_k >= 0 and 0.0 < top_p <= 1.0 and 0.0 <= min_p <= 1.0 and sampling_temperature > 0.0):
            raise UniGenHipError(f"t2i_generate: need an int top_k >= 0, 0 < top_p <= 1, 0 <= min_p <= 1 and sampling_temperature > 0 "
                                 f"(got top_k={top_k!r}, top_p={top_p!r}, min_p={min_p!r}, sampling_temperature={sampling_temperature!r})")
        n = image_token_num_per_image
        mask_token_id = self.config.mask_token_id
        embed = self.llm.model.embed_tokens
        cur_ids = input_ids[:, -(n + 1):-1].clone()
        gen = self._use_gen()
        if input_embeddings is None:
            input_embeddings = embed(input_ids)
        image_embeddings = (self.get_gen_embed(cur_ids).to(input_embeddings.dtype) if gen
                            else input_embeddings[:, -(n + 1):-1])
        bsz = image_embeddings.shape[0]
        prefix = input_embeddings[:, :-(n + 1)]
        suffix = input_embeddings[:, -1:]
        cfg = guidance_scale > 1
        if cfg:
            un_prefix = (embed(uncond_input_ids[:, :-(n + 1)]) if uncond_input_embeddings is None
                         else uncond_input_embeddings[:, :-(n + 1)])
            prefix = torch.cat([prefix, un_prefix])
            suffix = torch.cat([suffix, suffix])
        sampled_ids = None
        eng = self.llm.engine
        L = prefix.shape[1] + n + 1
        seg_start = L - n - 2
        incremental = bool(kwargs.get("incremental", True)) and not torch.is_grad_enabled() and attention_mask is not None
        if incremental and isinstance(attention_mask, ops.MaskBits):
            w0, sh = seg_start // 64, seg_start % 64
            words = attention_mask.bits[:, :seg_start, w0:]
            keep = torch.full((words.shape[-1],), -1, dtype=torch.int64, device=words.device)
            keep[0] = -1 << sh
            incremental = not bool(((words & keep) != 0).any())
        elif incremental:
            incremental = torch.is_tensor(attention_mask) and attention_mask.dim() == 4 \
                and not bool((attention_mask[:, 0, :seg_start, seg_start:] == 0).any())
        sess = None
        trace = kwargs.get("trace", None)
        logit_trace = kwargs.get("logit_trace", None)
        logp = torch.zeros((bsz * n, 2), dtype=torch.float32, device=image_embeddings.device) if return_logprobs else None
        for step in range(timesteps):
            img = torch.cat([image_embeddings, image_embeddings]) if cfg else image_embeddings
            if incremental:
                R = img.shape[0]
                if sess is None:
                    seq = torch.cat([prefix, img, suffix], 1).float()
                    mb = eng.mask_bits(attention_mask, R, L)
                    sess, hn = eng.maskgit_begin(seq.reshape(R * L, -1).contiguous(), mb, L, seg_start)
                    eng.check_errors()
                else:
                    seg = torch.cat([prefix[:, -1:], img, suffix], 1).float()
                    hn = eng.maskgit_step(sess, seg.reshape(R * (n + 2), -1).contiguous())
                rows = hn.view(R, n + 2, -1)[:, 1:n + 1].reshape(R * n, -1).contiguous()
                lg = (self._img_head(rows) if gen else eng.head_slice(rows, text_vocab_size, self.vocab_size - 1)).reshape(R, n, -1)
            elif gen:
                seq = torch.cat([prefix, img, suffix], 1)
                hn = self.llm.model(inputs_embeds=seq, attention_mask=attention_mask).last_hidden_state
                lg = self._img_head(hn[:, -(n + 1):-1].contiguous())
            else:
                seq = torch.cat([prefix, img, suffix], 1)
                out = self(input_ids=input_ids, input_embeddings=seq, attention_mask=attention_mask)
                lg = out[:, -(n + 1):-1, text_vocab_size:-1]
            ratio = 1.0 * (step + 1) / timesteps
            mask_len = int(torch.floor(n * noise_schedule(torch.tensor(ratio))).item())
            temperature = temperature * (1.0 - ratio)
            u_dev = lg.device if generator is None else generator.device
            u = torch.rand((2, bsz, n), device=u_dev, generator=generator).to(lg.device)
            lg = lg.contiguous()
            if logit_trace is not None:
                logit_trace.append(lg.clone())
            sampled_ids, cur_ids, next_ids = ops.maskgit_step(lg, bsz, n, cfg, guidance_scale, u[0], u[1], cur_ids,
                                                              mask_token_id, 0 if gen else text_vocab_size, mask_len, temperature,
                                                              top_k=top_k, top_p=top_p, min_p=min_p,
                                                              sample_temperature=sampling_temperature, logp=logp)
            if trace is not None:
                trace.append((sampled_ids.clone(), next_ids.clone()))
            image_embeddings = self.get_gen_embed(next_ids).to(input_embeddings.dtype) if gen else embed(next_ids)
        if return_logprobs:
            logp = logp.view(bsz, n, 2)
            return sampled_ids, logp[..., 0].contiguous(), logp[..., 1].contiguous()
        return sampled_ids

    def drop_decode_session(self):
        eng = getattr(getattr(self, "llm", None), "engine", None)
        if eng is not None:
            eng._ar_session = None
            eng._text_session = None

    def train(self, mode: bool = True):
        if mode:
            self.drop_decode_session()
        return super().train(mode)

    @torch.no_grad()
    def t2i_generate_ar(
            self,
            input_ids: Optional[torch.LongTensor] = None,
            uncond_input_ids: Optional[torch.LongTensor] = None,
            input_embeddings: Optional[torch.Tensor] = None,
            uncond_input_embeddings: Optional[torch.Tensor] = None,
            attention_mask: Optional[torch.Tensor] = None,
            guidance_scale: int = 0,
            temperature: float = 1.0,
            text_vocab_size: int = 151936,
            image_token_num_per_image: int = 256,
            generator: Optional[torch.Generator] = None,
            deterministic: Optional[bool] = None,
            top_k: Optional[int] = 0,
            top_p: Optional[float] = 1.0,
            min_p: Optional[float] = 0.0,
            return_logprobs: bool = False,
            **kwargs,
    ):
        from unigen_hip.qwen2 import ArDecodeSession, decode_loop, put_session, resolve_deterministic, take_session
        want_lp = bool(return_logprobs)
        top_k = 0 if top_k is None else top_k
        top_p = 1.0 if top_p is None else float(top_p)
        min_p = 0.0 if min_p is None else float(min_p)
        if not (isinstance(top_k, int) and top_k >= 0 and 0.0 < top_p <= 1.0 and 0.0 <= min_p <= 1.0):
# ... 449 lines not shown
```

### ml-unigen_amd/unigen_hip/lib.py

```python
import ctypes
import os
import subprocess

_HERE = os.path.dirname(os.path.abspath(__file__))
CSRC_DIR = os.path.normpath(os.path.join(_HERE, "..", "csrc"))
LIB_PATH = os.environ.get("UNIGEN_HIP_LIB") or os.path.join(CSRC_DIR, "libunigen_hip.so")

ABI_VERSION = 7
P = ctypes.c_void_p
I64 = ctypes.c_int64
I32 = ctypes.c_int
F32 = ctypes.c_float

SIGNATURES = {
    "ug_abi_version": [],
    "ug_create": [P],
    "ug_destroy": [P],
    "ug_gemm_bf16": [P, P, I64, I32, P, I64, I32, P, I64, I64, I64, I64, I32, P, P, I64, I32, P, I32, P],
    "ug_gemm_bf16_qkv_rope": [P, P, I64, P, I64, P, P, I64, I64, I64, I64, P, P, I64, I64, I32, P],
    "ug_gemm_bf16_swiglu_bwd": [P, P, I64, P, I64, P, I64, P, I64, I64, I64, I64, P],
    "ug_gemm_bf16_swiglu": [P, P, I64, P, I64, P, I64, P, I64, I64, I64, I64, P],
    "ug_cast_f32_bf16": [P, P, I64, P],
    "ug_rmsnorm_fwd": [P, P, P, P, I64, I64, F32, I32, P],
    "ug_rmsnorm_bwd": [P, P, P, P, P, P, P, I64, I64, P],
    "ug_rope": [P, P, P, I64, I64, I64, I32, I32, I32, P],
    "ug_swiglu_fwd": [P, P, I64, I64, P],
    "ug_swiglu_bwd": [P, P, P, I64, I64, P],
    "ug_gelu": [P, P, P, I64, P],
    "ug_embed_fwd": [P, P, P, I64, I64, I64, P, P],
    "ug_embed_bwd": [P, P, P, I64, I64, I64, P],
    "ug_embed_bwd_sorted": [P, P, P, P, I64, I64, I64, F32, P],
    "ug_gather_rows_bf16": [P, I64, P, P, I64, I64, I64, I32, P],
    "ug_colsum_bf16": [P, I64, P, I64, I64, P],
    "ug_attn_mask_compress": [P, I32, I64, I64, P, P, I64, I64, P, P],
    "ug_attn_mask_causal": [P, P, P, I64, I64, P],
    "ug_attn_fwd": [P, P, P, I64, P, I64, P, P, P, I64, I64, I64, I32, I32, I32, F32, P],
    "ug_attn_bwd": [P, P, P, I64, P, P, I64, P, P, P, P, P, I64, P, P, I64, I64, I64, I32, I32, I32, F32, P, P, P, P, P],
    "ug_kv_store": [P, I64, I64, I64, P, P, I64, I64, I32, I32, I64, P, I32, P],
    "ug_rope_at": [P, P, P, I64, I64, I32, I32, P, I64, P],
    "ug_attn_decode": [P, I64, P, P, P, P, I64, I64, I32, I32, I32, I64, P, F32, P],
    "ug_attn_prefill_cached": [P, I64, P, P, P, P, I64, I64, I64, I64, I32, I32, I32, I64, F32, P],
    "ug_gemv_bf16": [P, I64, I64, P, I64, P, I64, I64, I64, I64, P],
    "ug_decode_gemv": [P, I64, I64, P, I64, P, I64, I64, I64, P, I64, P, I64, P, P],
    "ug_decode_gemv_resid_norm": [P, P, I64, P, P, P, I64, P, I64, P, I64, I64, I64, P, I64, P, I64, P, P],
    "ug_decode_gemv_swiglu": [P, I64, P, F32, I64, I64, P, I64, P, I64, I64, I64, P, I64, P, I64, P, P],
    "ug_gemm_set_fused_tile_height": [I32],
    "ug_attn_decode_fused": [P, I64, P, F32, I64, P, P, P, P, P, P, P, P, I64, I64, I32, I32, I32, I64, I64, F32, P],
    "ug_decode_finish_resid_norm": [P, I64, P, P, P, I64, I64, F32, P, P, P],
    "ug_decode_sw_supported": [I64, I64, I64, I32],
    "ug_decode_sw_kblock": [P, I64, I64, P, I64, P, I64, I64, I64, P, I64, P, I64, P, P],
    "ug_decode_sw_resid": [P, I64, I64, P, I64, I64, I64, P, P],
    "ug_decode_sw_gate_up": [P, P, I64, P, P, F32, I64, I64, P, I64, I64, P, I64, P],
    "ug_decode_sw_head": [P, P, I64, P, P, F32, I64, I64, P, I64, I64, P, I64, P, P, P],
    "ug_t2i_assemble": [P, P, P, I64, P, I64, P, P, I64, I64, I64, I64, I64, I64, I64, P, P, P, P],
    "ug_attn_mask_from_ids": [P, I64, I64, I64, I64, I64, I32, P, P, P, P, P],
    "ug_maskgit_train_mask": [P, P, P, I64, I64, I64, I64, P, P, P],
    "ug_ar_sample": [P, I64, I64, I64, F32, F32, I32, P, P, I64, I64, P, I64, I64, I64, P, P, P, P],
    "ug_ar_sample_filtered": [P, I64, I64, I64, F32, F32, I32, P, P, I64, I64, P, I64, I64, I64, P, P, P, I64, F32, F32, P, P],
    "ug_text_pick": [P, I64, I64, I64, I32, P, I64, I64, P, I64, I64, I64, P, I64, P, P, P, P, P],
    "ug_text_sample_workspace_ints": [I64],
    "ug_text_sample": [P, I64, I64, I64, I32, F32, I64, F32, P, P, P, P, I64, I64, P, I64, I64, I64, P, I64, P, P, P, P, P],
    "ug_ar_sample_logp": [P, I64, I64, I64, F32, F32, I32, P, P, I64, I64, P, I64, I64, I64, P, P, P, P, P],
    "ug_ar_sample_filtered_logp": [P, I64, I64, I64, F32, F32, I32, P, P, I64, I64, P, I64, I64, I64, P, P, P, I64, F32, F32, P, P, P],
    "ug_text_pick_logp": [P, I64, I64, I64, I32, P, I64, I64, P, I64, I64, I64, P, I64, P, P, P, P, P, P],
    "ug_text_sample_logp": [P, I64, I64, I64, I32, F32, I64, F32, P, P, P, P, I64, I64, P, I64, I64, I64, P, I64, P, P, P, P, P, P],
    "ug_text_seen_mark": [P, I64, P, I64, I64, I64, P, I64, P],
    "ug_text_penalize": [P, I64, I64, I64, F32, P, I64, P, P],
    "ug_text_constrain": [P, I64, I64, I64, P, I64, I64, P, I64, I64, P, I64, P, P, I64, P, P],
    "ug_text_stop_seq": [P, P, I64, I64, P, I64, I64, P, P, P],
    "ug_maskgit_step": [P, I64, I64, I64, I64, I32, F32, P, P, P, I64, I64, I64, F32, P, P, P, P, P, P],
    "ug_maskgit_step_ex": [P, I64, I64, I64, I64, I32, F32, P, P, P, I64, I64, I64, F32, F32, I64, F32, F32, P, P, P, P, P, P, P, P],
    "ug_skinny_finish": [P, P, P, P, I64, I64, I32, P],
    "ug_gemv_bf16_ord": [P, I64, I64, P, I64, P, I64, I64, I64, I64, P],
    "ug_skinny_finish_ord": [P, I64, I64, P, P, P, P, I64, I64, P],
    "ug_decode_gemv_resid_norm_ord": [P, P, I64, I64, P, P, P, I64, P, I64, P, I64, I64, I64, P],
    "ug_attn_decode_fused_ord": [P, I64, I64, P, F32, I64, P, P, P, P, P, P, P, P, I64, I64, I32, I32, I32, I64, I64, F32, P],
    "ug_decode_sw_kblock_ord": [P, I64, I64, P, I64, P, I64, I64, I64, P],
    "ug_decode_finish_resid_norm_ord": [P, I64, I64, P, P, P, I64, I64, F32, P, P, P],
    "ug_ce_fwd": [P, I64, I64, I64, P, I64, P, P, P, P, P],
    "ug_ce_bwd": [P, I64, I64, I64, P, I64, P, P, P, P, P],
    "ug_head_score_ws_bytes": [I64, I64],
    "ug_head_score": [P, I64, I64, P, I64, I64, I64, P, I64, P, P, P, P, P, P],
    "ug_adamw_flat": [P, P, P, P, P, I64, F32, F32, F32, F32, F32, I64, F32, I32, P],
    "ug_adamw_flat_dev": [P, P, P, P, P, I64, F32, F32, F32, F32, F32, I64, F32, P, I32, P],
    "ug_sumsq_spans_f32": [P, I64, P, I32, I32, P],
    "ug_clip_finish": [P, I64, F32, F32, P, P],
    "ug_scale_spans_f32": [P, I64, P, I32, P],
    "ug_gemm_bf16_wgrad_group": [I32, P, P, P, P, P, P, P, P, P, P, P],
    "ug_grad_pack_bf16": [P, P, I64, F32, P],
    "ug_comm_unique_id": [P],
    "ug_comm_init": [P, I32, I32, P, I64],
    "ug_comm_allreduce_bucket": [P, P, I64, I32, P],
    "ug_comm_allgather": [P, P, P, I64, P],
    "ug_comm_wait": [P, P],
    "ug_comm_destroy": [P],
    "ug_comm_bytes_on_wire": [P],
    "ug_zero_ranges_f32": [P, P, I64, I64, P],
    "ug_grad_unpack_bf16": [P, P, I64, P],
    "ug_grad_sum_shards_bf16": [P, I32, I64, P, I64, F32, P],
    "ug_conv2d_f32": [P, P, P, P, P, I64, I32, I32, I32, I32, I32, I32, I32, I32, I32, I32, I32, I32, P],
    "ug_conv_split_weights": [P, P, I32, I32, I32, P],
    "ug_amax_f32": [P, I64, I64, I64, P, P],
    "ug_amax_f32_into_zeroed": [P, I64, I64, I64, P, P],
    "ug_conv2d_split": [P, P, P, P, P, P, I64, I32, I32, I32, I32, I32, I32, I32, I32, I32, I32, I32, I32, P, I32, P],
    "ug_conv3x3_split": [P, P, P, P, P, P, I64, I32, I32, I32, I32, I32, P, P, P, I32, I32, P, I32, P],
    "ug_groupnorm_finalize": [P, P, I64, I64, I32, I32, F32, P],
    "ug_groupnorm_stats": [P, P, P, I64, I64, I32, I32, F32, P],
    "ug_siglip_attn_f32": [P, I64, P, P, I64, I64, I64, I32, I32, F32, P],
    "ug_linear_split": [P, I64, P, P, P, P, I64, P, I64, I64, I64, I64, I32, I32, P],
    "ug_gemm_f32_nested": [P, I64, I64, I64, P, I64, I64, I64, I32, P, I64, I64, I64, I64, I64, I64, I64, I64, F32, P],
    "ug_gemm_f32": [P, I64, I64, P, I64, I64, I32, P, I64, I64, I64, I64, I64, I64, F32, P],
    "ug_groupnorm_swish": [P, P, P, P, P, I64, I64, I32, I32, F32, I32, P],
    "ug_softmax_rows_f32": [P, I64, I64, I64, F32, P],
    "ug_linear_f32": [P, I64, P, I64, P, P, I64, P, I64, I64, I64, I64, I32, P],
    "ug_layernorm_f32": [P, P, P, P, I64, I64, F32, P],
    "ug_layernorm_bwd_f32": [P, P, P, P, P, P, P, I64, I64, F32, P],
    "ug_gelu_tanh_f32": [P, P, P, I64, P],
    "ug_softmax_bwd_rows_f32": [P, P, I64, I64, I64, F32, P],
    "ug_colsum_f32": [P, I64, P, I64, I64, P],
    "ug_transpose_f32": [P, I64, I64, P, I64, I64, I64, I64, I64, P],
    "ug_nchw_to_nhwc": [P, P, I64, I32, I64, I32, P],
    "ug_nhwc_to_nchw": [P, P, I64, I32, I64, I32, P],
    "ug_lfq_pack": [P, I64, P, I64, I32, P],
    "ug_lfq_unpack": [P, P, I64, I32, P, P],
    "ug_probe_layouts": [P, I64, P],
}

_lib = None

PROFILE = None


def family_of(name):
    if name.startswith("ug_gemm_bf16"):
        return "gemm"
    if name in ("ug_attn_fwd", "ug_attn_bwd", "ug_attn_prefill_cached"):
        return "attention"
    if name.startswith(("ug_conv", "ug_groupnorm", "ug_amax", "ug_lfq", "ug_nchw", "ug_nhwc", "ug_gemm_f32", "ug_softmax_rows", "ug_linear_",
                        "ug_layernorm", "ug_siglip")):
        return "tokenizer_and_towers"
    if name in ("ug_adamw_flat", "ug_adamw_flat_dev"):
        return "adamw"
    return "elementwise"


def _profiled(name, fn):
    fam = family_of(name)

    def call(*args):
        prof = PROFILE
        if prof is None:
            return fn(*args)
        import torch
        e0, e1 = torch.cuda.Event(enable_timing=True), torch.cuda.Event(enable_timing=True)
        sp = args[-1]
        sp = getattr(sp, "value", sp) or 0
        st = torch.cuda.current_stream() if sp == torch.cuda.current_stream().cuda_stream else torch.cuda.ExternalStream(sp)
        e0.record(st)
        rc = fn(*args)
        e1.record(st)
        tag = name
        if name == "ug_gemm_bf16":
            tag = "ug_gemm_bf16[M=%d N=%d K=%d ak=%d bk=%d epi=%d]" % (args[9], args[10], args[11], args[3], args[6], args[12])
        elif name == "ug_conv3x3_split":
            tag = "ug_conv3x3_split[B=%d %dx%d %d->%d gn=%d]" % (args[6], args[7], args[8], args[9], args[10], 1 if args[12] else 0)
        elif name == "ug_gemm_bf16_wgrad_group":
            tag = "ug_gemm_bf16_wgrad_group[%s]" % " ".join("%dx%dx%d" % (args[7][i], args[8][i], args[10][i]) for i in range(args[0]))
        prof.setdefault(fam, []).append((e0, e1, tag))
        return rc
    call.__name__ = name
    return call


class UniGenHipError(RuntimeError):
    pass


def build(verbose=False):
    cmd = ["make", "-C", CSRC_DIR, "-j8"]
    res = subprocess.run(cmd, capture_output=True, text=True)
    if verbose or res.returncode != 0:
        print(res.stdout[-4000:])
        print(res.stderr[-4000:])
    if res.returncode != 0:
        raise UniGenHipError("building libunigen_hip.so failed (see output above)")
    return LIB_PATH


def load():
    global _lib
    if _lib is not None:
        return _lib
    if not os.path.exists(LIB_PATH):
        raise UniGenHipError(
            f"{LIB_PATH} is missing: the HIP extension is the only implementation of this path "
            f"(no CPU fallback). Build it with `make -C {CSRC_DIR}` or `python -c 'import __graft_entry__ as g; g.build()'`.")
    import torch
    lib = ctypes.CDLL(LIB_PATH)
    lib.ug_last_error.restype = ctypes.c_char_p
    lib.ug_last_error.argtypes = []
    for name, argtypes in SIGNATURES.items():
        fn = getattr(lib, name)
        fn.argtypes = argtypes
        fn.restype = ctypes.c_int64 if name == "ug_comm_bytes_on_wire" else ctypes.c_int
        if name.startswith("ug_comm_") or name in ("ug_abi_version", "ug_create", "ug_destroy"):
            continue
        setattr(lib, name, _profiled(name, fn))
    if lib.ug_abi_version() != ABI_VERSION:
        raise UniGenHipError(f"ABI version mismatch: library reports {lib.ug_abi_version()}, binding expects {ABI_VERSION}")
    _lib = lib
    return lib


def check(rc, name="ug call"):
    if rc != 0:
        msg = load().ug_last_error().decode("utf-8", "replace")
        raise UniGenHipError(f"{name} failed (rc={rc}): {msg}")
```

### ml-unigen_amd/unigen_hip/modules.py

```python
import math
from types import SimpleNamespace

import torch
import torch.nn as nn

from . import ops
from .lib import UniGenHipError
from .qwen2 import Qwen2Dims, Qwen2Engine, _hf_name_map


def anchor_of(engine):
    return engine._anchor


class _EmbedFn(torch.autograd.Function):
    @staticmethod
    def forward(ctx, anchor, ids, engine):
        flat_ids = ids.reshape(-1).contiguous()
        engine.fp.wait_pending_update()
        out = ops.embed_fwd(flat_ids, engine.fp.p("embed"), engine.err_flag)
        ctx.engine, ctx.ids = engine, flat_ids
        if ctx.needs_input_grad[0]:
            engine._lookup_rows_live += flat_ids.numel()
        return out.view(*ids.shape, engine.dims.hidden_size)

    @staticmethod
    def backward(ctx, dout):
        eng = ctx.engine
        eng.begin_grad_pass()
        drows = dout.reshape(-1, eng.dims.hidden_size).float().contiguous()
        eng.flush_deferred_head()
        sync = eng.grad_sync
        if sync is not None and sync.wants_lookups() and eng._lookup_rows_kept + ctx.ids.numel() <= eng._lookup_rows_cap:
            eng._lookup_rows_kept += ctx.ids.numel()
            sync.add_lookup(ctx.ids, drows)
        else:
            if sync is not None:
                sync.before_dense_embed_write()
            eng.fp.ensure_zeroed("embed")
            ops.embed_bwd(ctx.ids, drows, eng.fp.g("embed"))
        if eng.grad_ready_hook:
            eng.grad_ready_hook("embed")
        return None, None, None


class _StackFn(torch.autograd.Function):
    @staticmethod
    def forward(ctx, anchor, h0, engine, mb):
        B, L, H = h0.shape
        need = any(ctx.needs_input_grad)
        saved = [] if need else None
        if need:
            engine._forward_entry()
            engine._stack_graphs_live += 1
        h_last, hn, rstd = engine.stack_fwd(h0.reshape(B * L, H).float().contiguous(), mb, L, saved)
        if need:
            ctx.engine, ctx.saved, ctx.h_last, ctx.rstd, ctx.mb, ctx.shape = engine, saved, h_last, rstd, mb, (B, L, H)
        return hn.view(B, L, H)

    @staticmethod
    def backward(ctx, dhn):
        eng = ctx.engine
        B, L, H = ctx.shape
        eng.begin_grad_pass()
        last_writer = eng._stack_graphs_live <= 1
        eng._stack_graphs_live = max(0, eng._stack_graphs_live - 1)
        if eng.grad_sync is not None:
            eng.grad_sync.set_overlap(last_writer)
        dhn = dhn.reshape(B * L, H).to(torch.bfloat16).contiguous()
        dh0 = eng.stack_bwd(ctx.saved, ctx.h_last, ctx.rstd, dhn, ctx.mb, L)
        ctx.saved = None
        danchor = torch.zeros_like(anchor_of(eng)) if ctx.needs_input_grad[0] else None
        return danchor, dh0.view(B, L, H), None, None


class _HeadLossFn(torch.autograd.Function):

    @staticmethod
    def forward(ctx, anchor, hn, engine, idx, labels, bounds):
        B, L, H = hn.shape
        V = engine.dims.vocab_size
        rows = ops.gather_rows(hn.reshape(B * L, H), idx)
        logits = engine.logits_rows(rows)
        outs, stats = [], []
        for (r0, r1) in bounds:
            lc, lse, _, _ = ops.ce_fwd(logits[r0:r1], V, labels[r0:r1])
            outs.append(lc[:1])
            stats.append((lse, lc))
        ctx.engine, ctx.rows, ctx.logits, ctx.idx, ctx.labels, ctx.bounds, ctx.stats = engine, rows, logits, idx, labels, bounds, stats
        ctx.shape = (B, L, H)
        if any(ctx.needs_input_grad):
            engine._head_graphs_live += 1
        return torch.cat(outs)

    @staticmethod
    def backward(ctx, dloss):
        eng = ctx.engine
        B, L, H = ctx.shape
        V = eng.dims.vocab_size
        eng.begin_grad_pass()
        dloss = dloss.float().contiguous()
        for s, (r0, r1) in enumerate(ctx.bounds):
            lse, lc = ctx.stats[s]
            ops.ce_bwd_(ctx.logits[r0:r1], V, ctx.labels[r0:r1], lse, lc, dloss[s:s + 1])
        drows = eng.head_bwd(ctx.logits, ctx.rows)
        eng.head_written()
        ctx.logits = None
        dhn = torch.zeros((B * L, H), dtype=torch.bfloat16, device=drows.device)
        ops.scatter_rows_(drows, ctx.idx, dhn)
        return None, dhn.view(B, L, H), None, None, None, None


class _HeadRowsFn(torch.autograd.Function):

    @staticmethod
    def forward(ctx, anchor, hn, engine, idx, v0, v1):
        B, L, H = hn.shape
        rows = ops.gather_rows(hn.reshape(B * L, H), idx)
        n = v1 - v0
        npad = ops.round_up(max(n, 1), 8)
        out = torch.empty((rows.shape[0], npad), dtype=torch.bfloat16, device=hn.device)
        ops.gemm(rows, engine.fp.w("embed")[v0:v1], out=out, N=n, K=H)
        ctx.engine, ctx.rows, ctx.idx, ctx.rng, ctx.shape = engine, rows, idx, (v0, v1), (B, L, H)
        if any(ctx.needs_input_grad):
            engine._head_graphs_live += 1
        return out[:, :n]

    @staticmethod
    def backward(ctx, dout):
        eng = ctx.engine
        B, L, H = ctx.shape
        v0, v1 = ctx.rng
        n, R = v1 - v0, ctx.rows.shape[0]
        eng.begin_grad_pass()
        npad = ops.round_up(n, 8)
        dl = torch.zeros((R, npad), dtype=torch.bfloat16, device=dout.device)
        dl[:, :n] = dout
        eng.flush_deferred_head()
        if eng.grad_sync is not None:
            eng.grad_sync.before_dense_embed_write()
        eng.fp.ensure_zeroed("embed")
        ops.gemm(dl, ctx.rows, out=eng.fp.g("embed")[v0:v1], M=n, N=H, K=R, a_kmajor=True, b_kmajor=True,
                 epilogue=ops.UG_EPI_F32, beta=1)
        eng.head_written()
        drows = ops.gemm(dl, eng.fp.w("embed")[v0:v1], M=R, N=H, K=n, b_kmajor=True)
        dhn = torch.zeros((B * L, H), dtype=torch.bfloat16, device=dout.device)
        ops.scatter_rows_(drows, ctx.idx, dhn)
        return None, dhn.view(B, L, H), None, None, None, None


class LazyLogits:

    def __init__(self, engine, hn, dtype=torch.bfloat16):
        self.engine, self.hn = engine, hn
        B, L, _ = hn.shape
        self.shape = torch.Size((B, L, engine.dims.vocab_size))
        self.dtype, self.device = dtype, hn.device

    def size(self, dim=None):
        return self.shape if dim is None else self.shape[dim]

    def dim(self):
        return 3

    def _rows(self, bsel, psel, vsel):
        eng = self.engine
        B, L, V = self.shape
        bs = list(range(B))[bsel] if isinstance(bsel, slice) else [int(bsel) % B]
        ps = list(range(L))[psel] if isinstance(psel, slice) else [int(psel) % L]
        v0, v1, vstep = vsel.indices(V) if isinstance(vsel, slice) else (int(vsel) % V, int(vsel) % V + 1, 1)
        if vstep != 1:
            raise UniGenHipError("strided vocabulary slices are not supported")
        idx = (torch.tensor(bs, device=self.device)[:, None] * L + torch.tensor(ps, device=self.device)[None, :]).reshape(-1)
        n = v1 - v0
        out = _HeadRowsFn.apply(eng._anchor, self.hn, eng, idx, v0, v1)
        if self.dtype != torch.bfloat16:
            out = out.to(self.dtype)
        out = out.reshape(len(bs), len(ps), n)
        if not isinstance(vsel, slice):
            out = out[..., 0]
        if not isinstance(psel, slice):
            out = out[:, 0]
        if not isinstance(bsel, slice):
            out = out[0]
        return out

    def __getitem__(self, key):
        if not isinstance(key, tuple):
            key = (key,)
        if any(k is Ellipsis for k in key):
            raise UniGenHipError("LazyLogits does not support Ellipsis indexing; call .materialize()")
        key = tuple(key) + (slice(None),) * (3 - len(key))
        if not all(isinstance(k, (slice, int)) for k in key):
            return self.materialize()[key]
        return self._rows(*key)

    def materialize(self):
        return self._rows(slice(None), slice(None), slice(None))

    def float(self):
        return self.to(torch.float32)

    def to(self, *a, **k):
        dt = k.get("dtype")
        for x in a:
            if isinstance(x, torch.dtype):
                dt = x
        return LazyLogits(self.engine, self.hn, dt or self.dtype)

    def chunk(self, n, dim=0):
        B = self.shape[0]
        step = (B + n - 1) // n
        return tuple(self[i:i + step] for i in range(0, B, step))


class _ParamHolder(nn.Module):
    """Container giving parameters the reference's dotted names; forward is never called."""


class HipEmbedding(nn.Module):
    def __init__(self, engine, weight):
        super().__init__()
        self.__dict__["_engine"] = engine
        self.weight = weight
        self.num_embeddings, self.embedding_dim = weight.shape

    def forward(self, ids):
        eng = self.__dict__["_engine"]
        if torch.is_grad_enabled():
            eng._forward_entry()
        return _EmbedFn.apply(eng._anchor, ids.to(eng.device), eng)


class HipLMHead(nn.Module):
    def __init__(self, engine, weight):
        super().__init__()
        self.__dict__["_engine"] = engine
        self.weight = weight

    def forward(self, hidden):
        eng = self.__dict__["_engine"]
        h = hidden if hidden.dim() == 3 else hidden[None]
        return LazyLogits(eng, h.to(torch.bfloat16).contiguous())


class HipQwen2Model(nn.Module):

    def __init__(self, engine):
        super().__init__()
        self.__dict__["_engine"] = engine
        d = engine.dims
        params = engine.named_param_views()
        self.embed_tokens = HipEmbedding(engine, params["model.embed_tokens.weight"])
        self.layers = nn.ModuleList()
        for i in range(d.num_hidden_layers):
            layer = _ParamHolder()
            layer.self_attn = _ParamHolder()
            for proj in ("q_proj", "k_proj", "v_proj", "o_proj"):
                holder = _ParamHolder()
                holder.weight = params[f"model.layers.{i}.self_attn.{proj}.weight"]
                if proj != "o_proj":
                    holder.bias = params[f"model.layers.{i}.self_attn.{proj}.bias"]
                setattr(layer.self_attn, proj, holder)
            layer.mlp = _ParamHolder()
            for proj in ("gate_proj", "up_proj", "down_proj"):
                holder = _ParamHolder()
                holder.weight = params[f"model.layers.{i}.mlp.{proj}.weight"]
                setattr(layer.mlp, proj, holder)
            for nm in ("input_layernorm", "post_attention_layernorm"):
                holder = _ParamHolder()
                holder.weight = params[f"model.layers.{i}.{nm}.weight"]
                setattr(layer, nm, holder)
            self.layers.append(layer)
        self.norm = _ParamHolder()
        self.norm.weight = params["model.norm.weight"]

    def forward(self, input_ids=None, attention_mask=None, inputs_embeds=None, output_hidden_states=False,
                return_dict=True, **kwargs):
        eng = self.__dict__["_engine"]
        if (input_ids is None) == (inputs_embeds is None):
            raise ValueError("You must specify exactly one of input_ids or inputs_embeds")
        if inputs_embeds is None:
            inputs_embeds = self.embed_tokens(input_ids)
        B, L, _ = inputs_embeds.shape
        mb = eng.mask_bits(attention_mask, B, L)
        hn = _StackFn.apply(eng._anchor, inputs_embeds, eng, mb)
        return SimpleNamespace(last_hidden_state=hn, past_key_values=None)


class HipQwen2ForCausalLM(nn.Module):

    def __init__(self, dims, device, seed=None):
        super().__init__()
        engine = TrainEngine(dims, device)
        self.__dict__["_engine"] = engine
        self.config = SimpleNamespace(vocab_size=dims.vocab_size, hidden_size=dims.hidden_size, use_cache=False,
                                      num_hidden_layers=dims.num_hidden_layers, intermediate_size=dims.intermediate_size,
                                      num_attention_heads=dims.num_attention_heads,
                                      num_key_value_heads=dims.num_key_value_heads, rope_theta=dims.rope_theta,
                                      rms_norm_eps=dims.rms_norm_eps)
        self.model = HipQwen2Model(engine)
        self.lm_head = HipLMHead(engine, self.model.embed_tokens.weight)
        self.vocab_size = dims.vocab_size
        if seed is not None:
            self.init_weights(seed)

    @property
    def engine(self):
        return self.__dict__["_engine"]

    def init_weights(self, seed):
        g = torch.Generator().manual_seed(seed)
        std = self.engine.dims.initializer_range
        with torch.no_grad():
            for name, p in self.named_parameters():
                if name.endswith("norm.weight") or name.endswith("layernorm.weight"):
                    p.fill_(1.0)
                elif name.endswith(".bias"):
                    p.zero_()
                else:
                    p.copy_((torch.randn(p.shape, generator=g) * std).to(p.device))

    def init_weights_device(self, seed):
        eng = self.engine
        g = torch.Generator(device=eng.device).manual_seed(seed)
        std = eng.dims.initializer_range
        with torch.no_grad():
            eng.fp.master.zero_()
            for key, shp in eng.fp.spec:
                v = eng.fp.p(key)
                if key.endswith(("ln1", "ln2")) or key == "norm":
                    v.fill_(1.0)
                elif key.endswith("bqkv"):
                    v.zero_()
                else:
                    v.normal_(0.0, std, generator=g)

    def gradient_checkpointing_enable(self, *a, **k):
        return None

    def gradient_checkpointing_disable(self):
        return None

    def resize_token_embeddings(self, vocab_size):
        if vocab_size != self.engine.dims.vocab_size:
            raise UniGenHipError("resize_token_embeddings after construction is not implemented: build the model "
                                 "with the final vocab_size (the reference does, models/unigen.py:59-60)")
        return self.model.embed_tokens

    def forward(self, input_ids=None, attention_mask=None, inputs_embeds=None, **kwargs):
        out = self.model(input_ids=input_ids, attention_mask=attention_mask, inputs_embeds=inputs_embeds)
        return SimpleNamespace(logits=self.lm_head(out.last_hidden_state), past_key_values=None)


class TrainEngine(Qwen2Engine):

    def __init__(self, dims, device):
        super().__init__(dims, device)
        self._anchor = torch.zeros(1, device=device, requires_grad=True)
        self._params = None
        self._mask_cache = (None, None)
        self.grad_sync = None
        self.auto_data_parallel = True
        self.require_grad_sync = True
        self.extra_grad_params = None
        self._in_backward = False
        self._stack_graphs_live = 0
        self._head_graphs_live = 0
        self._lookup_rows_live = 0
        self._lookup_rows_cap = 0
        self._lookup_rows_kept = 0

    def head_written(self):
        self._head_graphs_live = max(0, self._head_graphs_live - 1)
        if self._head_graphs_live == 0 and self.grad_ready_hook:
            self.grad_ready_hook("head")

    def named_param_views(self):
        if self._params is None:
            self._params = {}
            for name, (key, rows) in _hf_name_map(self.dims).items():
                v, g = self.fp.p(key), self.fp.g(key)
                if rows is not None:
                    v, g = v[rows[0]:rows[1]], g[rows[0]:rows[1]]
                p = nn.Parameter(v, requires_grad=True)
                p.grad = g
                self.__dict__.setdefault("_grad_views", {})[name] = (p, g)
                self._params[name] = p
        return self._params

    def _dp_sync(self):
        if self.grad_sync is None and self.auto_data_parallel:
            import torch.distributed as dist
            import os
            forced = os.environ.get("UNIGEN_DDP_FORCE", "0") == "1"
            if dist.is_available() and dist.is_initialized() and (dist.get_world_size() > 1 or forced):
                from .ddp import FlatGradSync
                self.grad_sync = FlatGradSync(self, extra_params=lambda: self.extra_grad_params() if self.extra_grad_params else [])
                with torch.no_grad():
                    dist.broadcast(self.fp.master, 0)
                    for p in (self.extra_grad_params() if self.extra_grad_params else []):
                        dist.broadcast(p.data, 0)
                self.fp._seen_version = -1
        return self.grad_sync

    def _forward_entry(self):
        self._in_backward = False
        return self._dp_sync()

    def _sync_this_pass(self):
        if not self.require_grad_sync:
            return False
        import sys
        st = sys.modules.get("accelerate.state")
        gs = getattr(st, "GradientState", None) if st is not None else None
        if gs is not None and getattr(gs, "_shared_state", None):
            return bool(gs().sync_gradients)
        return True

    def _end_of_backward(self):
        self._in_backward = False
        self._stack_graphs_live = 0
        self._head_graphs_live = 0
        self._lookup_rows_live = 0
        if self.grad_sync is not None:
            self.grad_sync.finish()

    def begin_grad_pass(self):
        self.fp.wait_pending_update()
        views = self.__dict__.get("_grad_views", {})
        if any(p.grad is None for p, _ in views.values() if p.requires_grad):
            if all(p.grad is None for p, _ in views.values() if p.requires_grad):
                self.fp.clear_grads()
            else:
                for p, g in views.values():
                    if p.grad is None and p.requires_grad:
                        g.zero_()
            for p, g in views.values():
                if p.grad is None and p.requires_grad:
                    p.grad = g
        if not self._in_backward:
            sync = self._dp_sync()
            if sync is not None:
                self._in_backward = True
                self._lookup_rows_cap, self._lookup_rows_kept = self._lookup_rows_live, 0
                sync.begin(enabled=self._sync_this_pass(), lookup_rows=self._lookup_rows_live, heads_live=self._head_graphs_live)
                torch.autograd.Variable._execution_engine.queue_callback(self._end_of_backward)

    def mask_bits(self, attention_mask, B, L):
        if attention_mask is None:
            key = ("causal", B, L)
            if self._mask_cache[0] != key:
                self._mask_cache = (key, ops.mask_causal(B, L, self.device))
            return self._mask_cache[1]
        if isinstance(attention_mask, ops.MaskBits):
            return attention_mask
        if attention_mask.dim() == 2:
            return ops.mask_causal(B, L, self.device, key_valid=attention_mask.to(self.device) != 0)
        cached = self._mask_cache[0]
        if not (isinstance(cached, tuple) and cached[0] is attention_mask and cached[1] == attention_mask._version):
            mb = ops.mask_compress(attention_mask.to(self.device), self.err_flag)
            self._mask_cache = ((attention_mask, attention_mask._version), mb)
        return self._mask_cache[1]


class _TableEmbedFn(torch.autograd.Function):

    @staticmethod
    def forward(ctx, weight, ids, err_flag):
        flat = ids.reshape(-1).contiguous()
        out = ops.embed_fwd(flat, weight.detach().float().contiguous(), err_flag)
        ctx.ids, ctx.shape = flat, tuple(weight.shape)
        return out.view(*ids.shape, weight.shape[1])

    @staticmethod
    def backward(ctx, dout):
        dW = torch.zeros(ctx.shape, dtype=torch.float32, device=dout.device)
        ops.embed_bwd(ctx.ids, dout.reshape(-1, ctx.shape[1]).float().contiguous(), dW)
        return dW, None, None


class _CrossEntropyFn(torch.autograd.Function):

    @staticmethod
    def forward(ctx, logits, labels):
        R, V = logits.shape
        lg = torch.empty((R, ops.round_up(V, 8)), dtype=torch.bfloat16, device=logits.device)
        lg[:, :V] = logits
        lc, lse, _, _ = ops.ce_fwd(lg, V, labels)
        ctx.save_for_backward(lg, labels, lse, lc)
        ctx.in_dtype, ctx.V = logits.dtype, V
        return lc[0].clone()

    @staticmethod
    def backward(ctx, dloss):
        lg, labels, lse, lc = ctx.saved_tensors
        g = lg.clone()
        ops.ce_bwd_(g, ctx.V, labels, lse, lc, dloss.float().reshape(1).contiguous())
        return g[:, :ctx.V].to(ctx.in_dtype), None


class _LinearFn(torch.autograd.Function):

    @staticmethod
    def forward(ctx, x, w, b):
        shp = x.shape
        x2 = x.reshape(-1, shp[-1]).to(torch.bfloat16).contiguous()
        wb = ops.cast_bf16(w.detach().float().contiguous())
        bb = ops.cast_bf16(b.detach().float().contiguous()) if b is not None else None
        y = ops.gemm(x2, wb, bias=bb)
        ctx.save_for_backward(x2, wb)
        ctx.shp, ctx.has_bias, ctx.in_dtype = shp, b is not None, x.dtype
        return y.view(*shp[:-1], w.shape[0])

    @staticmethod
    def backward(ctx, dy):
        x2, wb = ctx.saved_tensors
        N, K = wb.shape
        dy2 = dy.reshape(-1, N).to(torch.bfloat16)
        if N % 8:
            pad = torch.zeros((dy2.shape[0], ops.round_up(N, 8)), dtype=torch.bfloat16, device=dy2.device)
            pad[:, :N] = dy2
            dy2 = pad
        else:
            dy2 = dy2.contiguous()
        M = dy2.shape[0]
        dx = (ops.gemm(dy2, wb, M=M, N=K, K=N, b_kmajor=True).view(ctx.shp).to(ctx.in_dtype)
              if ctx.needs_input_grad[0] else None)
        dw = ops.gemm(dy2, x2, M=N, N=K, K=M, a_kmajor=True, b_kmajor=True, epilogue=ops.UG_EPI_F32)
        db = None
        if ctx.has_bias:
            db = torch.zeros(N, dtype=torch.float32, device=dy2.device)
            ops.colsum_(dy2[:, :N], db)
        return dx, dw, db


class _GeluFn(torch.autograd.Function):
    @staticmethod
    def forward(ctx, x):
        xb = x.to(torch.bfloat16).contiguous()
        ctx.save_for_backward(xb)
        return ops.gelu(xb)

    @staticmethod
    def backward(ctx, dy):
        (xb,) = ctx.saved_tensors
        return ops.gelu(xb, dy.to(torch.bfloat16).contiguous())


class HipProjector(nn.Sequential):

    def forward(self, x):
        for m in self:
            if isinstance(m, nn.Linear):
                x = _LinearFn.apply(x, m.weight, m.bias)
            elif isinstance(m, nn.GELU):
                x = _GeluFn.apply(x)
            else:
                raise UniGenHipError(f"unexpected module in mm_projector: {type(m).__name__}")
        return x
```

### ml-unigen_amd/unigen_hip/ops.py

```python
import contextlib
import ctypes
import math
import torch

from . import lib as _l

UG_EPI_BF16, UG_EPI_F32, UG_EPI_RESID = 0, 1, 2
_MASK_DTYPES = {torch.float32: 0, torch.bfloat16: 1, torch.int64: 2, torch.bool: 3}


GEMM_PROFILE = None
GEMM_PROFILE_FUSED = None


class _GemmTimed:

    def __init__(self, prof, flops, fused):
        self.prof, self.flops, self.fused = prof, flops, fused

    def __enter__(self):
        self.e0, self.e1 = torch.cuda.Event(enable_timing=True), torch.cuda.Event(enable_timing=True)
        self.e0.record()

    def __exit__(self, exc_type, exc, tb):
# ... 37 lines not shown
        _l.check(_l.load().ug_create(ctypes.byref(out)), "ug_create")
        h = _HANDLES[key] = out.value
    return h


def release_handles():
    lib = _l.load()
    for h in _HANDLES.values():
        lib.ug_destroy(h)
    _HANDLES.clear()


def _need_cuda(*ts):
    for t in ts:
        if t is not None and not t.is_cuda:
            raise _l.UniGenHipError("unigen_hip ops need tensors in GPU memory (no CPU fallback exists)")


def round_up(x, m):
    return (x + m - 1) // m * m


def gemm(a, b, out=None, *, M=None, N=None, K=None, a_kmajor=False, b_kmajor=False, epilogue=UG_EPI_BF16,
         bias=None, resid=None, beta=0, alpha_dev=None, out_dtype=None):
    _need_cuda(a, b)
    if M is None:
        M = a.shape[1] if a_kmajor else a.shape[0]
    if N is None:
        N = b.shape[1] if b_kmajor else b.shape[0]
    if K is None:
        K = a.shape[0] if a_kmajor else a.shape[1]
    if out is None:
        dt = out_dtype or (torch.bfloat16 if epilogue == UG_EPI_BF16 else torch.float32)
        out = torch.empty((M, N), dtype=dt, device=a.device)
    lib = _l.load()
    with _gemm_timed(2.0 * M * N * K):
        rc = lib.ug_gemm_bf16(_handle(), _p(a), a.stride(0), int(a_kmajor), _p(b), b.stride(0), int(b_kmajor), _p(out), out.stride(0),
                              M, N, K, epilogue, _p(bias), _p(resid), resid.stride(0) if resid is not None else 0, beta,
                              _p(alpha_dev), GEMM_POLICY, _stream())
        _l.check(rc, "ug_gemm_bf16")
    return out


FUSED_SWIGLU = __import__("os").environ.get("UNIGEN_FUSED_SWIGLU", "1") == "1"


def gemm_swiglu(x, w_gate_up):
    _need_cuda(x, w_gate_up)
    if not FUSED_SWIGLU or GEMM_POLICY != -1:
        gu = gemm(x, w_gate_up)
        return gu, swiglu_fwd(gu)
    M, K = x.shape
    I = w_gate_up.shape[0] // 2
    gu = torch.empty((M, 2 * I), dtype=torch.bfloat16, device=x.device)
    act = torch.empty((M, I), dtype=torch.bfloat16, device=x.device)
    with _gemm_timed(2.0 * M * 2 * I * K, fused=True):
        _l.check(_l.load().ug_gemm_bf16_swiglu(_handle(), _p(x), x.stride(0), _p(w_gate_up), w_gate_up.stride(0), _p(gu), gu.stride(0),
                                               _p(act), act.stride(0), M, I, K, _stream()), "ug_gemm_bf16_swiglu")
    return gu, act


WGRAD_GROUP_MIN_TILES = 256


def gemm_wgrad_group(problems):
    tiles = sum(((dy.shape[1] + 255) // 256) * ((x.shape[1] + 255) // 256) for dy, x, _, _ in problems)
    if tiles < WGRAD_GROUP_MIN_TILES or len(problems) > 8 or GEMM_POLICY != -1:
        for dy, x, dw, beta in problems:
            gemm(dy, x, out=dw, a_kmajor=True, b_kmajor=True, epilogue=UG_EPI_F32, beta=beta)
        return
    n = len(problems)
    PA, LA, IA = ctypes.c_void_p * n, ctypes.c_int64 * n, ctypes.c_int * n
    for dy, x, dw, _ in problems:
        _need_cuda(dy, x, dw)
        assert dy.shape[0] == x.shape[0] and dw.shape == (dy.shape[1], x.shape[1])
    with _gemm_timed(sum(2.0 * dy.shape[1] * x.shape[1] * dy.shape[0] for dy, x, _, _ in problems)):
        rc = _l.load().ug_gemm_bf16_wgrad_group(
            n, PA(*[_p(dy) for dy, _, _, _ in problems]), LA(*[dy.stride(0) for dy, _, _, _ in problems]),
            PA(*[_p(x) for _, x, _, _ in problems]), LA(*[x.stride(0) for _, x, _, _ in problems]),
            PA(*[_p(dw) for _, _, dw, _ in problems]), LA(*[dw.stride(0) for _, _, dw, _ in problems]),
            LA(*[dy.shape[1] for dy, _, _, _ in problems]), LA(*[x.shape[1] for _, x, _, _ in problems]),
            IA(*[int(b) for _, _, _, b in problems]), LA(*[dy.shape[0] for dy, _, _, _ in problems]), _stream())
        _l.check(rc, "ug_gemm_bf16_wgrad_group")


def set_gemm_tile_policy(policy):
    global GEMM_POLICY
    policy = int(policy)
    if policy == 100:
        GEMM_POLICY = UG_GEMM_POLICY_AUTO_BITS | UG_GEMM_NARROW_EPILOGUE
    elif policy == 101:
        GEMM_POLICY = -1
    elif policy in (102, 104):
        GEMM_POLICY = UG_GEMM_POLICY_AUTO_BITS | (0x200 if policy == 102 else 0x400)
    elif policy in (103, 105):
        GEMM_POLICY = 3 | (0x200 if policy == 103 else 0x400)
    else:
        GEMM_POLICY = policy


def set_fused_tile_height(rows):
    _l.check(_l.load().ug_gemm_set_fused_tile_height(int(rows)), "ug_gemm_set_fused_tile_height")


def gemm_nt(a, b, out=None, **kw):
    return gemm(a, b, out, **kw)


def cast_bf16(x, out=None):
    _need_cuda(x)
    if out is None:
        out = torch.empty(x.shape, dtype=torch.bfloat16, device=x.device)
    _l.check(_l.load().ug_cast_f32_bf16(_p(x), _p(out), x.numel(), _stream()), "ug_cast_f32_bf16")
    return out


def zero_ranges_(buf, ranges, max_len):
    _l.check(_l.load().ug_zero_ranges_f32(_p(buf), _p(ranges), ranges.shape[0], int(max_len), _stream()), "ug_zero_ranges_f32")
    return buf


def grad_pack_bf16(g, out, scale):
    _need_cuda(g, out)
    _l.check(_l.load().ug_grad_pack_bf16(_p(g), _p(out), g.numel(), float(scale), _stream()), "ug_grad_pack_bf16")


def grad_unpack_bf16(src, g):
    _need_cuda(src, g)
    _l.check(_l.load().ug_grad_unpack_bf16(_p(src), _p(g), g.numel(), _stream()), "ug_grad_unpack_bf16")


def grad_sum_shards_bf16(shards, world, stride, out, scale):
    _need_cuda(shards, out)
    _l.check(_l.load().ug_grad_sum_shards_bf16(_p(shards), int(world), int(stride), _p(out), out.numel(), float(scale), _stream()),
             "ug_grad_sum_shards_bf16")


def rmsnorm_fwd(x, w, eps, out_f32=False, want_rstd=True, out=None):
    _need_cuda(x, w)
    rows, cols = x.shape
    y = out if out is not None else torch.empty((rows, cols), dtype=torch.float32 if out_f32 else torch.bfloat16, device=x.device)
    rstd = torch.empty((rows,), dtype=torch.float32, device=x.device) if want_rstd else None
    _l.check(_l.load().ug_rmsnorm_fwd(_p(x), _p(w), _p(y), _p(rstd), rows, cols, eps, int(out_f32), _stream()),
             "ug_rmsnorm_fwd")
    return y, rstd


def rmsnorm_bwd(dy, x, rstd, w, dres, dw, want_bf16=False):
    rows, cols = x.shape
    out = torch.empty((rows, cols), dtype=torch.bfloat16, device=x.device) if want_bf16 else None
    _l.check(_l.load().ug_rmsnorm_bwd(_p(dy), _p(x), _p(rstd), _p(w), _p(dres), _p(dw), _p(out), rows, cols, _stream()),
             "ug_rmsnorm_bwd")
    return out


def rope_inv_freq(head_dim, theta, scaling=None, seq_len=None):
    base = float(theta)
    kind = (scaling or {}).get("rope_type", (scaling or {}).get("type", "default"))
    factor = float((scaling or {}).get("factor", 1.0))
    if kind == "dynamic":
        max_pos = int((scaling or {}).get("max_position_embeddings", 32768))
        sl = torch.tensor(max(int(seq_len or 0), max_pos))
        base = base * ((factor * sl / max_pos) - (factor - 1)) ** (head_dim / (head_dim - 2))
    elif kind not in ("default", "linear"):
        raise _l.UniGenHipError(f"rope_type {kind!r} is not implemented (default, linear and dynamic are)")
    inv_freq = 1.0 / (base ** (torch.arange(0, head_dim, 2, dtype=torch.float) / head_dim))
    if kind == "linear":
        inv_freq = inv_freq / factor
    return inv_freq


def rope_tables(L, head_dim, theta, device, scaling=None):
    inv_freq = rope_inv_freq(head_dim, theta, scaling, L)
    pos = torch.arange(L, dtype=torch.float)
    freqs = (inv_freq[None, :, None] @ pos[None, None, :]).transpose(1, 2)[0]
    return freqs.cos().contiguous().to(device), freqs.sin().contiguous().to(device)


def rope_(qkv, cos, sin, L, nheads, head_dim, backward=False):
    tokens = qkv.shape[0]
    _l.check(_l.load().ug_rope(_p(qkv), _p(cos), _p(sin), tokens, L, qkv.stride(0), nheads, head_dim,
                               int(backward), _stream()), "ug_rope")
    return qkv


def gemm_qkv_rope(x, w, bias, cos, sin, L, nheads, head_dim):
    _need_cuda(x, w)
    M, K = x.shape
    N = w.shape[0]
    if GEMM_POLICY != -1:
        qkv = gemm(x, w, bias=bias)
        return rope_(qkv, cos, sin, L, nheads, head_dim)
    qkv = torch.empty((M, N), dtype=torch.bfloat16, device=x.device)
    with _gemm_timed(2.0 * M * N * K, fused=True):
        _l.check(_l.load().ug_gemm_bf16_qkv_rope(_handle(), _p(x), x.stride(0), _p(w), w.stride(0), _p(bias), _p(qkv), qkv.stride(0), M, N, K,
                                                  _p(cos), _p(sin), L, nheads * head_dim, head_dim, _stream()), "ug_gemm_bf16_qkv_rope")
    return qkv


def swiglu_fwd(gu):
    tokens, two_i = gu.shape
    act = torch.empty((tokens, two_i // 2), dtype=torch.bfloat16, device=gu.device)
    _l.check(_l.load().ug_swiglu_fwd(_p(gu), _p(act), tokens, two_i // 2, _stream()), "ug_swiglu_fwd")
    return act


FUSED_SWIGLU_BWD = __import__("os").environ.get("UNIGEN_FUSED_SWIGLU_BWD", "1") == "1"


def gemm_swiglu_bwd(dy, w_down, gu):
    _need_cuda(dy, w_down, gu)
    M, K = dy.shape
    I = gu.shape[1] // 2
    ok = (FUSED_SWIGLU_BWD and GEMM_POLICY == -1 and I % 256 == 0 and K % 32 == 0 and w_down.shape == (K, I)
          and dy.stride(0) % 8 == 0 and w_down.stride(0) % 8 == 0 and gu.stride(0) % 8 == 0)
    if not ok:
        return swiglu_bwd(gu, gemm(dy, w_down, b_kmajor=True))
    dgu = torch.empty_like(gu)
    with _gemm_timed(2.0 * M * I * K, fused=True):
        _l.check(_l.load().ug_gemm_bf16_swiglu_bwd(_handle(), _p(dy), dy.stride(0), _p(w_down), w_down.stride(0), _p(gu), gu.stride(0),
                                                    _p(dgu), dgu.stride(0), M, I, K, _stream()), "ug_gemm_bf16_swiglu_bwd")
    return dgu


def swiglu_bwd(gu, dact):
    dgu = torch.empty_like(gu)
    _l.check(_l.load().ug_swiglu_bwd(_p(gu), _p(dact), _p(dgu), gu.shape[0], gu.shape[1] // 2, _stream()),
             "ug_swiglu_bwd")
    return dgu


def embed_fwd(ids, W, err_flag=None):
    tokens = ids.numel()
    V, H = W.shape
    out = torch.empty((tokens, H), dtype=torch.float32, device=W.device)
    _l.check(_l.load().ug_embed_fwd(_p(ids), _p(W), _p(out), tokens, H, V, _p(err_flag), _stream()), "ug_embed_fwd")
    return out


def embed_bwd(ids, dout, dW):
    V, H = dW.shape
    _l.check(_l.load().ug_embed_bwd(_p(ids), _p(dout), _p(dW), ids.numel(), H, V, _stream()), "ug_embed_bwd")


def embed_bwd_sorted(ids_sorted, order, rows, dW, scale):
    V, H = dW.shape
    _l.check(_l.load().ug_embed_bwd_sorted(_p(ids_sorted), _p(order), _p(rows), _p(dW), ids_sorted.numel(), H, V, float(scale), _stream()),
             "ug_embed_bwd_sorted")


def gather_rows(x, idx):
    n, C = idx.numel(), x.shape[1]
    out = torch.empty((n, C), dtype=torch.bfloat16, device=x.device)
    _l.check(_l.load().ug_gather_rows_bf16(_p(x), x.stride(0), _p(idx), _p(out), C, n, C, 0, _stream()), "ug_gather_rows_bf16")
    return out


def scatter_rows_(src, idx, out):
    n, C = idx.numel(), src.shape[1]
    _l.check(_l.load().ug_gather_rows_bf16(_p(src), src.stride(0), _p(idx), _p(out), out.stride(0), n, C, 1, _stream()),
             "ug_gather_rows_bf16")
    return out


def colsum_(x, out, R=None, C=None):
    R = x.shape[0] if R is None else R
    C = x.shape[1] if C is None else C
    _l.check(_l.load().ug_colsum_bf16(_p(x), x.stride(0), _p(out), R, C, _stream()), "ug_colsum_bf16")


class MaskBits:

    def __init__(self, bits, tileany, B, L):
        self.bits, self.tileany, self.B, self.L = bits, tileany, B, L
        self.nW = (L + 63) // 64
        self.Lp = self.nW * 64


def _alloc_mask(B, L, device):
    nW = (L + 63) // 64
    bits = torch.empty((B, L, nW), dtype=torch.int64, device=device)
    tileany = torch.empty((B, nW, nW), dtype=torch.uint8, device=device)
    return bits, tileany


def mask_compress(mask4d, err_flag=None):
    _need_cuda(mask4d)
    if mask4d.dim() == 4:
        if mask4d.shape[1] != 1:
            raise _l.UniGenHipError("per-head attention masks are not part of the reference path")
        m = mask4d[:, 0]
    else:
        m = mask4d
    B, L, L2 = m.shape
    if L != L2 or m.stride(2) != 1:
        raise _l.UniGenHipError(f"attention mask must be [B,1,L,L] with contiguous rows, got {tuple(mask4d.shape)}")
    if m.dtype not in _MASK_DTYPES:
        raise _l.UniGenHipError(f"unsupported attention-mask dtype {m.dtype}")
    bits, tileany = _alloc_mask(B, L, m.device)
    _l.check(_l.load().ug_attn_mask_compress(_p(m), _MASK_DTYPES[m.dtype], m.stride(0), m.stride(1), _p(bits),
                                             _p(tileany), B, L, _p(err_flag), _stream()), "ug_attn_mask_compress")
    return MaskBits(bits, tileany, B, L)


def mask_causal(B, L, device, key_valid=None):
    bits, tileany = _alloc_mask(B, L, device)
# ... 341 lines not shown
        _l.check(_l.load().ug_ar_sample_filtered_logp(*args, _p(_logp_buffer(logp, (bsz, int(nsteps), 2))), _stream()),
                 "ug_ar_sample_filtered_logp")


def _logp_buffer(logp, shape, what="logp"):
    if not (torch.is_tensor(logp) and logp.is_cuda and logp.dtype == torch.float32 and logp.is_contiguous() and tuple(logp.shape) == tuple(shape)):
        raise _l.UniGenHipError(f"{what} must be a contiguous fp32 device tensor of shape {tuple(shape)}")
    return logp


TEXT_MAX_ROWS, TEXT_MAX_STOP = 32, 8
TEXT_STATE_INTS = 4 + TEXT_MAX_ROWS


def text_state(rows, device):
    return text_state_reset_(torch.empty(TEXT_STATE_INTS, dtype=torch.int32, device=device), rows)


def text_state_reset_(state, rows):
    state.zero_()
    state[1:2].fill_(int(rows))
    return state


def text_sample_workspace(rows, device):
    n = _l.load().ug_text_sample_workspace_ints(int(rows))
    if n <= 0:
        _l.check(n, "ug_text_sample_workspace_ints")
    return torch.zeros(n, dtype=torch.int32, device=device)


def _text_out(stop_ids, pad_id, embed_master):
    return (_p(stop_ids), 0 if stop_ids is None else stop_ids.numel(), -1 if pad_id is None else int(pad_id), _p(embed_master),
            embed_master.stride(0), embed_master.shape[0], embed_master.shape[1])


def text_pick_(logits, V, state, nsteps, embed_master, tok, out_tokens, x, clear=False, stop_ids=None, pad_id=None, lengths=None, logp=None):
    _need_cuda(logits, state, embed_master, tok, out_tokens, x)
    args = (_p(logits), logits.stride(0), logits.shape[0], int(V), int(bool(clear)), *_text_out(stop_ids, pad_id, embed_master), _p(state),
            int(nsteps), _p(tok), _p(out_tokens), _p(lengths), _p(x))
    if logp is None:
        _l.check(_l.load().ug_text_pick(*args, _stream()), "ug_text_pick")
    else:
        _l.check(_l.load().ug_text_pick_logp(*args, _p(_logp_buffer(logp, (logits.shape[0], int(nsteps)))), _stream()), "ug_text_pick_logp")


def text_sample_(logits, V, state, nsteps, embed_master, tok, out_tokens, x, uniforms, workspace, temperature=1.0, top_k=0, top_p=1.0,
                 clear=False, stop_ids=None, pad_id=None, lengths=None, stats=None, logp=None):
    _need_cuda(logits, state, embed_master, tok, out_tokens, x, uniforms, workspace)
    args = (_p(logits), logits.stride(0), logits.shape[0], int(V), int(bool(clear)), float(temperature), int(top_k), float(top_p),
            _p(uniforms), _p(workspace), _p(stats), *_text_out(stop_ids, pad_id, embed_master), _p(state), int(nsteps), _p(tok),
            _p(out_tokens), _p(lengths), _p(x))
    if logp is None:
        _l.check(_l.load().ug_text_sample(*args, _stream()), "ug_text_sample")
    else:
        _l.check(_l.load().ug_text_sample_logp(*args, _p(_logp_buffer(logp, (logits.shape[0], int(nsteps)))), _stream()), "ug_text_sample_logp")


def text_seen(rows, V, device):
    return torch.zeros((int(rows), (int(V) + 31) // 32), dtype=torch.int32, device=device)


def text_seen_mark_(seen, ids, V, valid=None):
    ids = ids.long()
    if ids.stride(1) != 1:
        ids = ids.contiguous()
    if valid is not None:
        valid = valid.to(torch.uint8).contiguous()
        if tuple(valid.shape) != tuple(ids.shape):
            raise _l.UniGenHipError(f"text_seen_mark_: valid {tuple(valid.shape)} against ids {tuple(ids.shape)}")
    _need_cuda(seen, ids)
    if seen.shape[0] != ids.shape[0] or seen.stride(1) != 1:
        raise _l.UniGenHipError(f"text_seen_mark_: seen {tuple(seen.shape)} against ids {tuple(ids.shape)}")
    _l.check(_l.load().ug_text_seen_mark(_p(seen), seen.stride(0), _p(ids), ids.stride(0), ids.shape[0], ids.shape[1], _p(valid), int(V),
                                         _stream()), "ug_text_seen_mark")
    return seen


def text_penalize_(logits, V, penalty, seen, tok=None):
    _need_cuda(logits, seen)
    if seen.shape[0] != logits.shape[0] or seen.stride(1) != 1 or logits.stride(1) != 1:
        raise _l.UniGenHipError(f"text_penalize_: seen {tuple(seen.shape)} against logits {tuple(logits.shape)}")
    _l.check(_l.load().ug_text_penalize(_p(logits), logits.stride(0), logits.shape[0], int(V), float(penalty), _p(seen), seen.stride(0),
                                        _p(tok), _stream()), "ug_text_penalize")


TEXT_MAX_BIAS, TEXT_MAX_NGRAM, TEXT_MAX_STOP_SEQS, TEXT_MAX_STOP_SEQ_LEN = 1024, 16, 8, 16


def text_bias_pairs(entries, device):
    if not entries:
        return None
    pairs = torch.empty((len(entries), 2), dtype=torch.int32)
    pairs[:, 0] = torch.tensor([int(e) for e, _ in entries], dtype=torch.int32)
    pairs[:, 1] = torch.tensor([float(b) for _, b in entries], dtype=torch.float32).view(torch.int32)
    return pairs.to(device)


def text_stop_seqs(seqs, device):
    ids = [int(t) for s in seqs for t in s]
    off = [0]
    for s in seqs:
        off.append(off[-1] + len(s))
    return torch.tensor(ids, dtype=torch.int32, device=device), torch.tensor(off, dtype=torch.int32, device=device)


def text_constrain_(logits, V, state, out_tokens, bias=None, min_new=0, stop_ids=None, ngram=0, hist=None, hist_len=None):
    _need_cuda(logits, state, out_tokens, bias, stop_ids, hist, hist_len)
    R = logits.shape[0]
    if logits.stride(1) != 1 or out_tokens.shape[0] != R or not out_tokens.is_contiguous() or out_tokens.dtype != torch.int32:
        raise _l.UniGenHipError(f"text_constrain_: out_tokens {tuple(out_tokens.shape)} {out_tokens.dtype} against logits {tuple(logits.shape)}")
    if bias is not None and not (bias.dtype == torch.int32 and bias.dim() == 2 and bias.shape[1] == 2 and bias.is_contiguous()):
        raise _l.UniGenHipError("text_constrain_: bias must be ops.text_bias_pairs' contiguous int32 [n, 2]")
    if (hist is None) != (hist_len is None) or (hist is not None and not (
            hist.dtype == torch.int32 and hist_len.dtype == torch.int32 and hist.dim() == 2 and hist.shape[0] == R and hist.stride(1) == 1 and
            hist_len.is_contiguous() and hist_len.numel() == R)):
        raise _l.UniGenHipError("text_constrain_: hist int32 [R, ld_hist] and hist_len int32 [R] come together")
    _l.check(_l.load().ug_text_constrain(_p(logits), logits.stride(0), R, int(V), _p(bias), 0 if bias is None else bias.shape[0], int(min_new),
                                         _p(stop_ids), 0 if stop_ids is None else stop_ids.numel(), int(ngram), _p(hist),
                                         0 if hist is None else hist.stride(0), _p(hist_len), _p(out_tokens), out_tokens.shape[1], _p(state),
                                         _stream()), "ug_text_constrain")


def text_stop_seq_(seq_ids, seq_off, out_tokens, state, lengths=None):
    _need_cuda(seq_ids, seq_off, out_tokens, state, lengths)
    if not (seq_ids.dtype == seq_off.dtype == out_tokens.dtype == torch.int32 and seq_ids.is_contiguous() and seq_off.is_contiguous() and
            out_tokens.dim() == 2 and out_tokens.is_contiguous() and seq_off.numel() >= 2):
        raise _l.UniGenHipError("text_stop_seq_: int32 contiguous seq_ids, seq_off [ns + 1] and out_tokens [R, nsteps]")
    if lengths is not None and not (lengths.dtype == torch.int32 and lengths.is_contiguous() and lengths.numel() == out_tokens.shape[0]):
        raise _l.UniGenHipError("text_stop_seq_: lengths must be int32 [R]")
    _l.check(_l.load().ug_text_stop_seq(_p(seq_ids), _p(seq_off), seq_off.numel() - 1, seq_ids.numel(), _p(out_tokens), out_tokens.shape[1],
                                        out_tokens.shape[0], _p(state), _p(lengths), _stream()), "ug_text_stop_seq")


def ce_fwd(logits, V, labels, ignore_index=-100, want_logp=False):
    R, ld = logits.shape[0], logits.stride(0)
    dev = logits.device
    lse = torch.empty((R,), dtype=torch.float32, device=dev)
    loss_row = torch.empty((R,), dtype=torch.float32, device=dev)
    logp = torch.empty((R,), dtype=torch.float32, device=dev) if want_logp else None
    lc = torch.empty((2,), dtype=torch.float32, device=dev)
    _l.check(_l.load().ug_ce_fwd(_p(logits), ld, R, V, _p(labels), ignore_index, _p(lse), _p(loss_row), _p(logp),
                                 _p(lc), _stream()), "ug_ce_fwd")
    return lc, lse, loss_row, logp


def ce_bwd_(logits, V, labels, lse, lc, gscale=None, ignore_index=-100, row_scale=None):
    R, ld = logits.shape[0], logits.stride(0)
    _l.check(_l.load().ug_ce_bwd(_p(logits), ld, R, V, _p(labels), ignore_index, _p(lse), _p(lc), _p(gscale),
                                 _p(row_scale), _stream()), "ug_ce_bwd")
    return logits


_HEAD_SCORE_WS = {}
HEAD_SCORE_WANT = ("lse", "best", "best_logit")


def head_score_ws_bytes(R, V):
    n = _l.load().ug_head_score_ws_bytes(R, V)
    if n <= 0:
        _l.check(n, "ug_head_score_ws_bytes")
    return n


def _head_score_workspace(nbytes, device):
    ws = _HEAD_SCORE_WS.get(device)
    if ws is None or ws.numel() < nbytes:
        ws = _HEAD_SCORE_WS[device] = torch.empty((nbytes,), dtype=torch.uint8, device=device)
    return ws


def head_score(x, W, V, labels, ignore_index=-100, want=("lse", "best")):
    _need_cuda(x, W, labels)
    bad = [n for n in want if n not in HEAD_SCORE_WANT]
    if bad or x.dim() != 2 or W.dim() != 2 or x.dtype != torch.bfloat16 or W.dtype != torch.bfloat16 or x.stride(1) != 1 or W.stride(1) != 1 \
            or x.shape[1] != W.shape[1] or not 1 <= V <= W.shape[0] or labels.dtype != torch.int64 or labels.dim() != 1 \
            or labels.shape[0] != x.shape[0] or not labels.is_contiguous():
        raise _l.UniGenHipError(f"head_score: need bf16 x [R, K] and W [>=V, K] with unit inner stride, int64 labels [R] and want within "
                                f"{HEAD_SCORE_WANT} (x {tuple(x.shape)} {x.dtype}, W {tuple(W.shape)} {W.dtype}, V {V}, labels "
                                f"{tuple(labels.shape)} {labels.dtype}, want {tuple(want)})")
    R, K = x.shape
    dev = x.device
    ws = _head_score_workspace(head_score_ws_bytes(R, V), dev)
    logp = torch.empty((R,), dtype=torch.float32, device=dev)
    out = {"lse": None, "best": None, "best_logit": None}
    for n in want:
        out[n] = torch.empty((R,), dtype=torch.int64 if n == "best" else torch.float32, device=dev)
    _l.check(_l.load().ug_head_score(_p(x), x.stride(0), R, _p(W), W.stride(0), V, K, _p(labels), ignore_index, _p(ws), _p(logp),
                                     _p(out["lse"]), _p(out["best"]), _p(out["best_logit"]), _stream()), "ug_head_score")
    return (logp,) + tuple(out[n] for n in want)


BF16_MIRRORS = []


def register_bf16_mirror(owner):
    import weakref
    BF16_MIRRORS.append(weakref.ref(owner))


def find_bf16_mirror(ptr, numel):
    for ref in list(BF16_MIRRORS):
        o = ref()
        if o is None:
            BF16_MIRRORS.remove(ref)
            continue
        base = o.master.data_ptr()
        if base <= ptr and ptr + 4 * numel <= base + 4 * o.master.numel():
            return o, o.bf16.data_ptr() + (ptr - base) // 2
    return None, 0


def adamw_flat_(p, g, m, v, p_bf16, lr, beta1, beta2, eps, wd, step, grad_scale=1.0, max_blocks=0):
    _l.check(_l.load().ug_adamw_flat(_p(p), _p(g), _p(m), _p(v), _p(p_bf16), p.numel(), lr, beta1, beta2, eps, wd,
                                     step, grad_scale, max_blocks, _stream()), "ug_adamw_flat")


def adamw_flat_dev_(p, g, m, v, p_bf16, lr, beta1, beta2, eps, wd, step, grad_scale=1.0, grad_factor=None, max_blocks=0):
    _l.check(_l.load().ug_adamw_flat_dev(_p(p), _p(g), _p(m), _p(v), _p(p_bf16), p.numel(), lr, beta1, beta2, eps, wd,
                                         step, grad_scale, _p(grad_factor), max_blocks, _stream()), "ug_adamw_flat_dev")


SUMSQ_BLOCKS = 256


def sumsq_spans(spans, partials, blocks=None, accum=0):
    blocks = SUMSQ_BLOCKS if blocks is None else int(blocks)
    if partials.dtype != torch.float64 or partials.numel() < blocks:
        raise _l.UniGenHipError("sumsq_spans: the partial buffer needs `blocks` fp64 values")
    _l.check(_l.load().ug_sumsq_spans_f32(_p(spans), spans.shape[0], _p(partials), blocks, accum, _stream()), "ug_sumsq_spans_f32")
    return partials


def clip_finish(partials, n_partials, max_norm, result, grad_scale=1.0):
    _l.check(_l.load().ug_clip_finish(_p(partials), int(n_partials), float(max_norm), float(grad_scale), _p(result), _stream()), "ug_clip_finish")
    return result


def scale_spans_(spans, coef, blocks=0):
    _l.check(_l.load().ug_scale_spans_f32(_p(spans), spans.shape[0], _p(coef), int(blocks), _stream()), "ug_scale_spans_f32")


def pack_conv_weight(w):
    cout, cin, kh, kw = w.shape
    cout_pad = round_up(cout, 128) if cout > 32 else 32
    wp = torch.zeros((kh * kw, cin, cout_pad), dtype=torch.float32, device=w.device)
    wp[:, :, :cout] = w.detach().float().permute(2, 3, 1, 0).reshape(kh * kw, cin, cout)
    return wp.contiguous(), cout_pad


def conv_split_eligible(cin, cout, cout_pad):
    return cin % 32 == 0 and cout % 4 == 0 and cout_pad % 128 == 0 and cout >= 64


def split_conv_weight(wp):
    taps, cin, cout_pad = wp.shape
    ws = torch.empty(2 * taps * round_up(cin, 32) * cout_pad + 8, dtype=torch.float16, device=wp.device)
    _l.check(_l.load().ug_conv_split_weights(_p(wp), _p(ws), taps, cin, cout_pad, _stream()), "ug_conv_split_weights")
    return ws


_AMAX_CONST = {}


def amax_const(value, device):
    key = (float(value), str(device))
    if key not in _AMAX_CONST:
        _AMAX_CONST[key] = torch.full((1,), float(value), dtype=torch.float32, device=device)
    return _AMAX_CONST[key]


def amax(x2d):
    _need_cuda(x2d)
    if x2d.dim() == 2 and x2d.stride(1) == 1:
        rows, cols, ld = x2d.shape[0], x2d.shape[1], x2d.stride(0)
    else:
        x2d = x2d.contiguous()
        rows, cols, ld = 1, x2d.numel(), x2d.numel()
    if torch.cuda.is_current_stream_capturing():
        out = torch.empty(1, dtype=torch.float32, device=x2d.device)
        _l.check(_l.load().ug_amax_f32(_p(x2d), rows, cols, ld, _p(out), _stream()), "ug_amax_f32")
        return out
    out = _amax_slot(x2d.device)
    _l.check(_l.load().ug_amax_f32_into_zeroed(_p(x2d), rows, cols, ld, _p(out), _stream()), "ug_amax_f32")
    return out


_AMAX_POOL = {}


def _amax_slot(device):
    key = (str(device), torch.cuda.current_stream(device).cuda_stream)
    pool = _AMAX_POOL.get(key)
    if pool is None or pool[1] >= pool[0].numel():
        pool = [torch.zeros(1024, dtype=torch.float32, device=device), 0]
        _AMAX_POOL[key] = pool
    i = pool[1]
    pool[1] = i + 1
    return pool[0][i:i + 1]


def conv2d_nhwc(x, wp, cout_pad, bias, cout, ksize, *, stride=1, pad=None, residual=None, upsample=False,
                asym_pad=False, w_split=None, x_amax=None, out_stats=None, out_groups=32):
    B, H, W, Cin = x.shape
    He, We = (2 * H, 2 * W) if upsample else (H, W)
    if asym_pad:
# ... 227 lines not shown
```

### ml-unigen_amd/unigen_hip/qwen2.py

```python
import math
import os

import types

import torch
import torch.nn as nn

from . import ops
from .lib import UniGenHipError


class Qwen2Dims:
    def __init__(self, vocab_size, hidden_size=1536, intermediate_size=8960, num_hidden_layers=28,
                 num_attention_heads=12, num_key_value_heads=2, rope_theta=1e6, rms_norm_eps=1e-6,
                 initializer_range=0.02, rope_scaling=None, max_position_embeddings=32768, **_unused):
        self.vocab_size = int(vocab_size)
        self.hidden_size = hidden_size
        self.intermediate_size = intermediate_size
        self.num_hidden_layers = num_hidden_layers
        self.num_attention_heads = num_attention_heads
        self.num_key_value_heads = num_key_value_heads
        self.head_dim = hidden_size // num_attention_heads
        self.rope_theta = float(rope_theta)
        self.rope_scaling = None
# ... 168 lines not shown
class TextDecodeSession:

    def __init__(self, eng, rows, capacity, width, vocab, deterministic=False, sampling=None, stop_ids=(), pad_id=None, key_valid=None,
                 repetition_penalty=1.0, logprobs=False, constraints=None):
        dev, d = eng.device, eng.dims
        self.rows, self.width, self.V, self.sampling = rows, width, vocab, sampling
        self.form = eng.decode_form(rows, deterministic)
        self.st = DecodeState(d, rows, capacity, dev, key_valid=key_valid, deterministic=deterministic)
        self.state = ops.text_state(rows, dev)
        self.x = torch.zeros((rows, d.hidden_size), dtype=torch.float32, device=dev)
        self.tok = torch.zeros((rows,), dtype=torch.long, device=dev)
        self.out_tokens = torch.zeros((rows, width), dtype=torch.int32, device=dev)
        self.lengths = torch.zeros((rows,), dtype=torch.int32, device=dev)
        self.logits = torch.zeros((rows, vocab if deterministic else ops.round_up(vocab, 8)), dtype=torch.float32, device=dev)
        self.stop_ids = torch.tensor([int(s) for s in stop_ids], dtype=torch.long, device=dev) if len(stop_ids) else None
        self.pad_id = pad_id
        self.workspace = self.uniforms = None
        if sampling is not None:
            self.workspace = ops.text_sample_workspace(rows, dev)
            self.uniforms = torch.zeros((width, rows), dtype=torch.float32, device=dev)
        self.penalty = float(repetition_penalty)
        self.seen = ops.text_seen(rows, vocab, dev) if self.penalty != 1.0 else None
        self.logp = torch.zeros((rows, width), dtype=torch.float32, device=dev) if logprobs else None
        c = constraints or {}
        self.bias = ops.text_bias_pairs(c.get("bias"), dev)
        self.min_new, self.ngram = int(c.get("min_new", 0)) if len(stop_ids) else 0, int(c.get("ngram", 0))
        self.constrained = self.bias is not None or self.min_new > 0 or self.ngram > 0
        self.hist = torch.zeros((rows, capacity), dtype=torch.int32, device=dev) if self.ngram else None
        self.hist_len = torch.zeros((rows,), dtype=torch.int32, device=dev) if self.ngram else None
        self.stop_seqs = ops.text_stop_seqs(c["stop_seqs"], dev) if c.get("stop_seqs") else None
        self.graph, self.key = None, None

    def begin(self, new_tokens, key_valid=None, prompt_len=0, prompt_ids=None, prompt_valid=None):
        ops.text_state_reset_(self.state, self.rows)
        self.lengths.fill_(int(new_tokens))
        if self.logp is not None:
            self.logp.zero_()
        if key_valid is not None:
            self.st.key_valid[:, :prompt_len].copy_(key_valid)
            self.st.key_valid[:, prompt_len:].fill_(1)
        if self.seen is not None:
            self.seen.zero_()
            if prompt_ids is not None and prompt_ids.shape[1] > 0:
                ops.text_seen_mark_(self.seen, prompt_ids, self.V, prompt_valid)
        if self.hist is not None:
            self.hist_len.zero_()
            if prompt_ids is not None and prompt_ids.shape[1] > 0:
                ids = prompt_ids.to(self.hist.device).long()
                ok = (ids >= 0) & (ids < self.V)
                if prompt_valid is not None:
                    ok &= prompt_valid.to(ok.device) != 0
                order = torch.argsort((~ok).to(torch.int8), dim=1, stable=True)
                self.hist[:, :ids.shape[1]].copy_(torch.gather(ids, 1, order))
                self.hist_len.copy_(ok.sum(1))


class ArDecodeSession:

    def __init__(self, eng, rows, bsz, prefix_len, steps, V, code_lo, guidance_scale, temperature, greedy=False, filt=None, deterministic=False,
                 key_valid=None, generator=None, logprobs=False, fused=True):
        dev = eng.device
        self.fused = fused
        self.bsz, self.P, self.n, self.V, self.code_lo = bsz, prefix_len, steps, V, code_lo
        self.guidance_scale, self.temperature, self.greedy, self.filt = guidance_scale, temperature, greedy, filt
        self.form = eng.decode_form(rows, deterministic)
        self.st = DecodeState(eng.dims, rows, prefix_len + steps, dev, key_valid=key_valid, deterministic=deterministic)
        self.out_tokens = torch.zeros((bsz, steps), dtype=torch.int, device=dev)
        self.x = torch.empty((rows, eng.dims.hidden_size), dtype=torch.float32, device=dev)
        self.tok = torch.zeros((bsz, 1), dtype=torch.long, device=dev)
        self.logp = torch.zeros((bsz, steps, 2), dtype=torch.float32, device=dev) if logprobs else None
        self.uniforms = self.draw_uniforms(generator)
        self.acc_head = torch.zeros((rows, V), dtype=torch.float32, device=dev) if fused else None
        self.lp_now = torch.zeros((bsz, 2), dtype=torch.float32, device=dev) if logprobs and not fused else None
        self.graph, self.key = None, None

    def draw_uniforms(self, generator):
        if self.greedy or not self.fused:
            return None
        dev = self.st.pos.device
        return torch.rand((self.n, self.bsz), device=dev if generator is None else generator.device, generator=generator).to(dev)

    def begin(self, key_valid=None, generator=None):
        if key_valid is not None:
            self.st.key_valid[:, :self.P].copy_(key_valid)
        if self.uniforms is not None:
            self.uniforms.copy_(self.draw_uniforms(generator))


def _keeping(wanted):
    return bool(wanted) and os.environ.get("UNIGEN_AR_GRAPH_CACHE", "1") != "0"


def take_session(eng, attr, key, wanted):
    sess = getattr(eng, attr, None) if _keeping(wanted) else None
    setattr(eng, attr, None)
    return sess if sess is not None and sess.key == key else None


def put_session(eng, attr, sess, wanted):
    kept = _keeping(wanted) and sess.graph is not None
    if kept:
        setattr(eng, attr, sess)
    return kept


def decode_loop(sess, step, steps, use_graph, stop=None, mark=None, after=None):
    mark = mark or (lambda name: None)
    captured = False
    for i in steps:
        if stop is not None and stop(i):
            break
        if sess.graph is None and use_graph and i == 2:
            mark("eager_step")
            torch.cuda.synchronize()
            graph = torch.cuda.CUDAGraph()
            with torch.cuda.graph(graph):
                step()
            sess.graph, captured = graph, True
            mark("capture")
            graph.replay()
        elif sess.graph is not None:
            sess.graph.replay()
        else:
            step()
        if after is not None:
            after(i)
    mark("replay")
    return captured


class _Saved:
    __slots__ =("h", "rstd1", "xn1", "qkv", "o", "lse", "h_mid", "rstd2", "xn2", "gu", "act")


class Qwen2Engine:

    def __init__(self, dims, device):
        self.dims, self.device = dims, device
        self.fp = FlatParams(dims, device)
        self._rope_cache = {}
        self.err_flag = torch.zeros(1, dtype=torch.int32, device=device)
        self.grad_ready_hook = None

    def rope(self, L):
        if L not in self._rope_cache:
            self._rope_cache[L] = ops.rope_tables(L, self.dims.head_dim, self.dims.rope_theta, self.device, self.dims.rope_scaling)
        return self._rope_cache[L]

    def check_errors(self):
        v = int(self.err_flag.item())
        if v:
            self.err_flag.zero_()
            raise UniGenHipError(f"device-side input check failed (flags={v}): 1=token id out of range, "
                                 f"2=attention mask value neither 0 nor <= -1e9, 4=VQ code out of range")

    def layer_fwd(self, i, h, mb, L, save):
        d, fp = self.dims, self.fp
        Hq, Hk, hd = d.num_attention_heads, d.num_key_value_heads, d.head_dim
        cos, sin = self.rope(L)
        xn1, rstd1 = ops.rmsnorm_fwd(h, fp.p(f"l{i}.ln1"), d.rms_norm_eps)
        qkv = ops.gemm_qkv_rope(xn1, fp.w(f"l{i}.wqkv"), fp.w(f"l{i}.bqkv"), cos, sin, L, Hq + Hk, hd)
        o, lse = ops.attn_fwd(qkv, mb, Hq, Hk, hd)
        h_mid = ops.gemm_nt(o, fp.w(f"l{i}.wo"), epilogue=ops.UG_EPI_RESID, resid=h)
        xn2, rstd2 = ops.rmsnorm_fwd(h_mid, fp.p(f"l{i}.ln2"), d.rms_norm_eps)
        gu, act = ops.gemm_swiglu(xn2, fp.w(f"l{i}.wgu"))
        h_out = ops.gemm_nt(act, fp.w(f"l{i}.wdown"), epilogue=ops.UG_EPI_RESID, resid=h_mid)
        if save is not None:
            s = _Saved()
            s.h, s.rstd1, s.xn1, s.qkv, s.o, s.lse = h, rstd1, xn1, qkv, o, lse
            s.h_mid, s.rstd2, s.xn2, s.gu, s.act = h_mid, rstd2, xn2, gu, act
            save.append(s)
        return h_out

    def stack_fwd(self, h0, mb, L, save):
        self.fp.refresh_compute_copies()
        h = h0
        for i in range(self.dims.num_hidden_layers):
            h = self.layer_fwd(i, h, mb, L, save)
        hn, rstd = ops.rmsnorm_fwd(h, self.fp.p("norm"), self.dims.rms_norm_eps)
        return h, hn, rstd

    def maskgit_begin(self, h0, mb, L, seg_start):
        self.fp.refresh_compute_copies()
        B = h0.shape[0] // L
        saved, h = [], h0
        for i in range(self.dims.num_hidden_layers):
            h = self.layer_fwd(i, h, mb, L, saved)
        sess = types.SimpleNamespace()
        sess.qkv = [s.qkv for s in saved]
        sess.mb, sess.B, sess.L, sess.P, sess.S = mb, B, L, seg_start, L - seg_start
        r = torch.arange(seg_start, L, device=self.device)
        sess.rows = (torch.arange(B, device=self.device)[:, None] * L + r[None, :]).reshape(-1).contiguous()
        cos, sin = self.rope(L)
        sess.cos, sess.sin = cos[seg_start:].contiguous(), sin[seg_start:].contiguous()
        hn, _ = ops.rmsnorm_fwd(h.view(B, L, -1)[:, seg_start:].reshape(B * sess.S, -1).contiguous(), self.fp.p("norm"),
                                self.dims.rms_norm_eps, want_rstd=False)
        return sess, hn

    def maskgit_step(self, sess, seg):
        d, fp = self.dims, self.fp
        Hq, Hk, hd = d.num_attention_heads, d.num_key_value_heads, d.head_dim
        h = seg
        for i in range(d.num_hidden_layers):
            xn1, _ = ops.rmsnorm_fwd(h, fp.p(f"l{i}.ln1"), d.rms_norm_eps, want_rstd=False)
            qkv_s = ops.gemm_qkv_rope(xn1, fp.w(f"l{i}.wqkv"), fp.w(f"l{i}.bqkv"), sess.cos, sess.sin, sess.S, Hq + Hk, hd)
            ops.scatter_rows_(qkv_s, sess.rows, sess.qkv[i])
            o, _ = ops.attn_fwd(sess.qkv[i], sess.mb, Hq, Hk, hd)
            o_s = ops.gather_rows(o, sess.rows)
            h_mid = ops.gemm_nt(o_s, fp.w(f"l{i}.wo"), epilogue=ops.UG_EPI_RESID, resid=h)
            xn2, _ = ops.rmsnorm_fwd(h_mid, fp.p(f"l{i}.ln2"), d.rms_norm_eps, want_rstd=False)
            _, act = ops.gemm_swiglu(xn2, fp.w(f"l{i}.wgu"))
            h = ops.gemm_nt(act, fp.w(f"l{i}.wdown"), epilogue=ops.UG_EPI_RESID, resid=h_mid)
        hn, _ = ops.rmsnorm_fwd(h, fp.p("norm"), d.rms_norm_eps, want_rstd=False)
        return hn

    def layer_bwd(self, i, s, dh, mb, L, dh_bf16=None):
        d, fp = self.dims, self.fp
        Hq, Hk, hd = d.num_attention_heads, d.num_key_value_heads, d.head_dim
        cos, sin = self.rope(L)
        F32 = ops.UG_EPI_F32
        wg = lambda key, dy, x: (dy, x, fp.g(key), fp.beta_for(key))
        dyd = dh_bf16 if dh_bf16 is not None else ops.cast_bf16(dh)
        w_down = wg(f"l{i}.wdown", dyd, s.act)
        dgu = ops.gemm_swiglu_bwd(dyd, fp.w(f"l{i}.wdown"), s.gu)
        w_gu = wg(f"l{i}.wgu", dgu, s.xn2)
        dxn2 = ops.gemm(dgu, fp.w(f"l{i}.wgu"), b_kmajor=True)
        dyo = ops.rmsnorm_bwd(dxn2, s.h_mid, s.rstd2, fp.p(f"l{i}.ln2"), dh, fp.g(f"l{i}.ln2"), want_bf16=True)
        w_o = wg(f"l{i}.wo", dyo, s.o)
        do = ops.gemm(dyo, fp.w(f"l{i}.wo"), b_kmajor=True)
        dqkv = ops.attn_bwd(s.qkv, s.o, s.lse, do, mb, Hq, Hk, hd, rope=(cos, sin), dbias=fp.g(f"l{i}.bqkv"))
        w_qkv = wg(f"l{i}.wqkv", dqkv, s.xn1)
        dxn1 = ops.gemm(dqkv, fp.w(f"l{i}.wqkv"), b_kmajor=True)
        dnext = ops.rmsnorm_bwd(dxn1, s.h, s.rstd1, fp.p(f"l{i}.ln1"), dh, fp.g(f"l{i}.ln1"), want_bf16=True)
        self._wgrad_tokens = dyd.shape[0]
        ops.gemm_wgrad_group([w_gu, w_down, w_qkv, w_o] + self._head_wgrad_slice())
        return dh, dnext

    def stack_bwd(self, saved, h_last, rstd_last, dhn, mb, L):
        dh = torch.zeros_like(h_last)
        dh16 = ops.rmsnorm_bwd(dhn, h_last, rstd_last, self.fp.p("norm"), dh, self.fp.g("norm"), want_bf16=True)
        if self.grad_ready_hook:
            self.grad_ready_hook("norm")
        for i in reversed(range(self.dims.num_hidden_layers)):
            dh, dh16 = self.layer_bwd(i, saved[i], dh, mb, L, dh16)
            saved[i] = None
            if self.grad_ready_hook:
                self.grad_ready_hook(i)
        self.flush_deferred_head()
        self.fp.flush_fresh()
        return dh

    def logits_rows(self, hn_rows):
        d = self.dims
        out = torch.empty((hn_rows.shape[0], d.vocab_pad), dtype=torch.bfloat16, device=self.device)
        return ops.gemm_nt(hn_rows, self.fp.w("embed"), out=out, N=d.vocab_size, K=d.hidden_size)

    def score_rows(self, hn_rows, labels, ignore_index=-100):
        self.fp.refresh_compute_copies()
        return ops.head_score(hn_rows, self.fp.w("embed"), self.dims.vocab_size, labels, ignore_index=ignore_index, want=("lse", "best"))

    def head_bwd(self, dlogits, hn_rows):
        d, fp = self.dims, self.fp
        R = hn_rows.shape[0]
        sync = getattr(self, "grad_sync", None)
        if sync is not None:
            sync.before_dense_embed_write()
        if self._may_defer_head_wgrad(R):
            self.flush_deferred_head()
            self._deferred_head = [dlogits, hn_rows, fp.beta_for("embed"), 0]
            torch.autograd.Variable._execution_engine.queue_callback(self.flush_deferred_head)
        else:
            ops.gemm(dlogits, hn_rows, out=fp.g("embed"), M=d.vocab_size, N=d.hidden_size, K=R, a_kmajor=True, b_kmajor=True,
                     epilogue=ops.UG_EPI_F32, beta=fp.beta_for("embed"))
        return ops.gemm(dlogits, fp.w("embed"), M=R, N=d.hidden_size, K=d.vocab_size, b_kmajor=True)

    def _may_defer_head_wgrad(self, R):
        if os.environ.get("UNIGEN_DEFER_HEAD_WGRAD", "1") != "1" or not torch.is_tensor(self.fp.grad) or not self.fp.grad.is_cuda:
            return False
        sync = getattr(self, "grad_sync", None)
        if sync is not None and sync.active and sync.enabled:
            return False
        d = self.dims
        layer_tiles = sum(-(-a // 256) * -(-b // 256) for a, b in ((2 * d.intermediate_size, d.hidden_size), (d.hidden_size, d.intermediate_size),
                                                                   (d.qkv_out, d.hidden_size), (d.hidden_size, d.hidden_size)))
        return layer_tiles >= ops.WGRAD_GROUP_MIN_TILES and ops.GEMM_POLICY == -1

    def _head_wgrad_slice(self):
        st = getattr(self, "_deferred_head", None)
        if not st:
            return []
        dlogits, hn_rows, beta, v0 = st
        V = self.dims.vocab_size
        d = self.dims
        layer_tiles = sum(-(-a // 256) * -(-b // 256) for a, b in ((2 * d.intermediate_size, d.hidden_size), (d.hidden_size, d.intermediate_size),
                                                                   (d.qkv_out, d.hidden_size), (d.hidden_size, d.hidden_size)))
        idle = -layer_tiles % 256
        cols = -(-d.hidden_size // 256)
        fit = int(0.8 * idle * (self._wgrad_tokens / 32 + 60) / (hn_rows.shape[0] / 32 + 60) / cols)
        per = int(os.environ.get("UNIGEN_HEAD_SLICE_TILES", "0")) or fit
        if per <= 0:
            return []
        per *= 256
        v1 = min(V, v0 + per)
        prob = (dlogits[:, v0:v1], hn_rows, self.fp.g("embed")[v0:v1], beta)
        if v1 >= V:
            self._deferred_head = None
        else:
            st[3] = v1
        return [prob]

    def flush_deferred_head(self):
        st = getattr(self, "_deferred_head", None)
        if not st:
            return
        dlogits, hn_rows, beta, v0 = st
        self._deferred_head = None
        V, H = self.dims.vocab_size, self.dims.hidden_size
        ops.gemm(dlogits[:, v0:], hn_rows, out=self.fp.g("embed")[v0:], M=V - v0, N=H, K=hn_rows.shape[0], a_kmajor=True,
                 b_kmajor=True, epilogue=ops.UG_EPI_F32, beta=beta)

    def prefill(self, st, embeds, key_valid=None, mask_bits=None):
        d = self.dims
        R, P, H = embeds.shape
        Hq, Hk, hd = d.num_attention_heads, d.num_key_value_heads, d.head_dim
        self.fp.refresh_compute_copies()
        mb = mask_bits if mask_bits is not None else ops.mask_causal(R, P, self.device, key_valid=key_valid)
        h = embeds.reshape(R * P, H).float().contiguous()
        for i in range(d.num_hidden_layers):
            saved = []
            h = self.layer_fwd(i, h, mb, P, saved)
            ops.kv_store(saved[0].qkv, st.k[i], st.v[i], R, P, Hq, Hk, hd, st.Tmax, None, 0)
        st.pos.fill_(P)
        st.len.fill_(P + 1)
        hn, _ = ops.rmsnorm_fwd(h, self.fp.p("norm"), d.rms_norm_eps, want_rstd=False)
        return hn.view(R, P, H)[:, -1].contiguous()

    def prefill_onto(self, st, embeds, P, key_valid=None, hidden_at=None):
        d, fp = self.dims, self.fp
        R, S, H = embeds.shape
        P = int(P)
        Hq, Hk, hd = d.num_attention_heads, d.num_key_value_heads, d.head_dim
        if R != st.rows or S < 1 or P < 0 or P + S > st.Tmax:
            raise UniGenHipError(f"prefill_onto: {R} rows of {S} positions at {P} do not fit a state of {st.rows} rows, {st.Tmax} positions")
        if hidden_at is not None and (hidden_at.dtype != torch.int64 or hidden_at.dim() != 1 or hidden_at.numel() < 1):
            raise UniGenHipError(f"prefill_onto: hidden_at must be a non-empty int64 vector of indices into the {R * S} new positions")
        kv = None
        if key_valid is not None:
            if tuple(key_valid.shape) != (R, P + S):
                raise UniGenHipError(f"prefill_onto: key_valid must be [{R}, {P + S}], got {tuple(key_valid.shape)}")
            kv = torch.ones((R, st.Tmax), dtype=torch.uint8, device=self.device)
            kv[:, :P + S] = key_valid.to(device=self.device, dtype=torch.uint8)
        fp.refresh_compute_copies()
        cos, sin = self.rope(P + S)
        cos, sin = cos[P:].contiguous(), sin[P:].contiguous()
        h = embeds.reshape(R * S, H).float().contiguous()
        for i in range(d.num_hidden_layers):
            xn1, _ = ops.rmsnorm_fwd(h, fp.p(f"l{i}.ln1"), d.rms_norm_eps, want_rstd=False)
            qkv = ops.gemm_qkv_rope(xn1, fp.w(f"l{i}.wqkv"), fp.w(f"l{i}.bqkv"), cos, sin, S, Hq + Hk, hd)
            ops.kv_store(qkv, st.k[i], st.v[i], R, S, Hq, Hk, hd, st.Tmax, None, P)
            o = ops.attn_prefill_cached(qkv, st.k[i], st.v[i], kv, S, P, Hq, Hk, hd, st.Tmax)
            h_mid = ops.gemm_nt(o, fp.w(f"l{i}.wo"), epilogue=ops.UG_EPI_RESID, resid=h)
            xn2, _ = ops.rmsnorm_fwd(h_mid, fp.p(f"l{i}.ln2"), d.rms_norm_eps, want_rstd=False)
            _, act = ops.gemm_swiglu(xn2, fp.w(f"l{i}.wgu"))
            h = ops.gemm_nt(act, fp.w(f"l{i}.wdown"), epilogue=ops.UG_EPI_RESID, resid=h_mid)
        st.pos.fill_(P + S)
        st.len.fill_(P + S + 1)
        hn, _ = ops.rmsnorm_fwd(h.view(R, S, H)[:, -1].contiguous(), fp.p("norm"), d.rms_norm_eps, want_rstd=False)
        if hidden_at is None:
            return hn
        hn_sel, _ = ops.rmsnorm_fwd(h.index_select(0, hidden_at.to(self.device)), fp.p("norm"), d.rms_norm_eps, want_rstd=False)
        return hn, hn_sel

    def decode_form(self, rows, deterministic):
        d = self.dims
        H, I, hd, q_dim = d.hidden_size, d.intermediate_size, d.head_dim, d.num_attention_heads * d.head_dim
        fused = getattr(self, "decode_fused", True)
        sw_ok = (fused and os.environ.get("UNIGEN_DECODE_SW", "1") != "0" and rows <= 16
                 and ops.decode_sw_supported(H, I, q_dim, hd))
        if deterministic:
            ord_dims = H == 256 * ops.ORD_QKV_SLABS and I == 1792 * ops.ORD_DOWN_KBLOCKS and d.num_hidden_layers >= 1
            return "ord_sw" if sw_ok and ord_dims else "ord_wide"
        if not fused or rows > 32 or hd != 128 or min(H, I, q_dim) < 256 or H % 32 or I % 32 or H > 4096:
            return "wide"
        return "sw" if sw_ok else "splitk"

    def decode_sw(self, st):
        return self.decode_form(st.rows, False) == "sw"

    def decode_ord_sw(self, st):
        return self.decode_form(st.rows, True) == "ord_sw"

    def _decode_layers_ord(self, st, x):
        d, fp = self.dims, self.fp
# ... 202 lines not shown
```

Before: 124.9.

## Fuse cross-entropy forward and backward and use row-sparse final-norm backward

Adds a fused cross-entropy kernel that keeps each logits row in registers and LDS, computes the LSE, and writes the gradient in place in one pass. A cheap scale kernel then applies the upstream gradient, with a fallback to the plain path when that gradient is not a safe power of two. It also adds a row-sparse RMSNorm backward for the final norm, so only the supervised rows are read and the zero-filled dense dhn scatter is skipped. The cost is a large per-thread register footprint, a mode-detection fallback that may recompute logits, and extra autograd plumbing through a marker tensor.

```diff
diff --git a/include/unigen_hip.h b/include/unigen_hip.h
--- a/include/unigen_hip.h
+++ b/include/unigen_hip.h
@@ -47,6 +47,8 @@
                    float eps, int out_f32, hipStream_t stream);
 int ug_rmsnorm_bwd(const void* dy, const float* x, const float* rstd, const float* w, float* dres,
                    float* dw, void* dres_bf16, int64_t rows, int64_t cols, hipStream_t stream);
+int ug_rmsnorm_bwd_rows(const void* dy_rows, const int64_t* idx, int64_t n_listed, const float* x, const float* rstd,
+                        const float* w, float* dres, float* dw, void* dres_bf16, int64_t rows, int64_t cols, hipStream_t stream);
 int ug_rope(void* qkv, const float* cos_tab, const float* sin_tab, int64_t tokens, int64_t L, int64_t ldq,
             int nheads, int head_dim, int backward, hipStream_t stream);
 int ug_swiglu_fwd(const void* gate_up, void* act, int64_t tokens, int64_t I, hipStream_t stream);
@@ -216,6 +218,11 @@
 int ug_ce_bwd(void* logits_inout, int64_t ld, int64_t R, int64_t V, const int64_t* labels,
               int64_t ignore_index, const float* lse, const float* loss_and_count, const float* gscale,
               const float* row_scale, hipStream_t stream);
+#define UG_CE_FUSED_MAX_LD 163840
+int ug_ce_fused(void* logits_inout, int64_t ld, int64_t R, int64_t V, const int64_t* labels, int64_t ignore_index,
+                float* lse, float* loss_row, float* loss_and_count, uint32_t* dmin, hipStream_t stream);
+int ug_ce_gscale(void* grad_inout, int64_t ld, int64_t R, const float* g, const float* loss_and_count, const uint32_t* dmin,
+                 int* status, int status_bit, hipStream_t stream);
 
 int ug_head_score_ws_bytes(int64_t R, int64_t V);
 int ug_head_score(const void* x, int64_t ldx, int64_t R, const void* W, int64_t ldw, int64_t V, int64_t K,
diff --git a/ml-unigen_amd/csrc/elementwise.hip b/ml-unigen_amd/csrc/elementwise.hip
--- a/ml-unigen_amd/csrc/elementwise.hip
+++ b/ml-unigen_amd/csrc/elementwise.hip
@@ -95,14 +95,15 @@
 }
 
 constexpr int RN_MAXV = 8;
-template <int NV, int NT>
+template <int NV, int NT, bool ROWS = false>
 __global__ __launch_bounds__(256) void rmsnorm_bwd_kernel(const bf16_t* __restrict__ dy, const float* __restrict__ x,
                                                           const float* __restrict__ rstd, const float* __restrict__ w,
                                                           float* __restrict__ dres, float* __restrict__ dw,
                                                           bf16_t* __restrict__ dres_bf16, int rows, int cols,
-                                                          int rows_per_block) {
+                                                          int rows_per_block, const int64_t* __restrict__ idx = nullptr,
+                                                          int n_listed = 0) {
   __shared__ float red[4][64 * 4];
-  const int wave = threadIdx.x >> 6, lane = threadIdx.x & 63;
+  const int wave = ROWS ? __builtin_amdgcn_readfirstlane(threadIdx.x >> 6) : threadIdx.x >> 6, lane = threadIdx.x & 63;
   const int nv = cols >> 2;
   float4 dwp[NV];
 #pragma unroll
@@ -110,10 +111,32 @@
   const float4* wr = reinterpret_cast<const float4*>(w);
   const int r0 = blockIdx.x * rows_per_block;
   const int r1 = min(rows, r0 + rows_per_block);
+  int p = 0;
+  if constexpr (ROWS) {
+    int hi = n_listed;
+    while (p < hi) {
+      const int mid = (p + hi) >> 1;
+      if (idx[mid] < r0 + wave) p = mid + 1; else hi = mid;
+    }
+  }
   for (int row = r0 + wave; row < r1; row += 4) {
     const float4* xr = reinterpret_cast<const float4*>(x + (int64_t)row * cols);
-    const uint2* dyr = reinterpret_cast<const uint2*>(dy + (int64_t)row * cols);
     float4* dr = reinterpret_cast<float4*>(dres + (int64_t)row * cols);
+    if constexpr (ROWS) {
+      while (p < n_listed && idx[p] < row) ++p;
+      if (!(p < n_listed && idx[p] == row)) {
+#pragma unroll
+        for (int k = 0; k < NV; ++k) {
+          const int i = lane + k * 64;
+          if (i < nv) {
+            st_stream<NT>(dr + i, make_float4(0.f, 0.f, 0.f, 0.f));
+            if (dres_bf16) reinterpret_cast<uint2*>(dres_bf16 + (int64_t)row * cols)[i] = make_uint2(0u, 0u);
+          }
+        }
+        continue;
+      }
+    }
+    const uint2* dyr = reinterpret_cast<const uint2*>(dy + (int64_t)(ROWS ? p : row) * cols);
     const float r = rstd[row];
     float4 g[NV], xh[NV], acc[NV];
     uint2 dyv[NV];
@@ -126,7 +149,7 @@
 #pragma unroll
     for (int k = 0; k < NV; ++k) {
       const int i = lane + k * 64;
-      if (i < nv) acc[k] = dr[i];
+      if (i < nv) acc[k] = ROWS ? make_float4(0.f, 0.f, 0.f, 0.f) : dr[i];
     }
 #pragma unroll
     for (int k = 0; k < NV; ++k) {
@@ -696,6 +719,23 @@
   return UG_OK;
 }
 
+extern "C" int ug_rmsnorm_bwd_rows(const void* dy_rows, const int64_t* idx, int64_t n_listed, const float* x, const float* rstd,
+                                   const float* w, float* dres, float* dw, void* dres_bf16, int64_t rows, int64_t cols,
+                                   hipStream_t st) {
+  UG_REQUIRE(rows > 0 && cols > 0 && cols % 4 == 0 && cols <= 64 * 4 * RN_MAXV,
+             "ug_rmsnorm_bwd_rows: cols=%ld unsupported (multiple of 4, <= %d)", (long)cols, 64 * 4 * RN_MAXV);
+  UG_REQUIRE(n_listed >= 0 && n_listed <= rows && (n_listed == 0 || (dy_rows && idx)), "ug_rmsnorm_bwd_rows: bad row list (%ld of %ld rows)",
+             (long)n_listed, (long)rows);
+  UG_REQUIRE(ug_aligned16(x) && ug_aligned16(w) && ug_aligned16(dres) && dres && ((uintptr_t)dy_rows & 7) == 0 &&
+             ((uintptr_t)dres_bf16 & 7) == 0, "ug_rmsnorm_bwd_rows: pointers must be aligned");
+  const int rpb = (int)std::max<int64_t>(16, ((rows + 479) / 480 + 3) / 4 * 4);
+  dim3 grid((unsigned)((rows + rpb - 1) / rpb)), block(256);
+  hipLaunchKernelGGL((rmsnorm_bwd_kernel<RN_MAXV, NT_RMSNORM_BWD, true>), grid, block, 0, st, (const bf16_t*)dy_rows, x, rstd, w, dres,
+                     dw, (bf16_t*)dres_bf16, (int)rows, (int)cols, rpb, idx, (int)n_listed);
+  UG_CHECK_LAUNCH("ug_rmsnorm_bwd_rows");
+  return UG_OK;
+}
+
 extern "C" int ug_rope(void* qkv, const float* cos_tab, const float* sin_tab, int64_t tokens, int64_t L, int64_t ldq,
                        int nheads, int head_dim, int backward, hipStream_t st) {
   UG_REQUIRE(tokens > 0 && L > 0 && tokens % L == 0, "ug_rope: tokens=%ld must be a multiple of L=%ld", (long)tokens, (long)L);
diff --git a/ml-unigen_amd/csrc/loss.hip b/ml-unigen_amd/csrc/loss.hip
--- a/ml-unigen_amd/csrc/loss.hip
+++ b/ml-unigen_amd/csrc/loss.hip
@@ -2,6 +2,50 @@
 #include "unigen_hip.h"
 
 namespace {
+
+__device__ __forceinline__ void ce_online8(const bf16x8_t v, float& m, float& s) {
+  float f[8], mx = -INFINITY;
+#pragma unroll
+  for (int k = 0; k < 8; ++k) { f[k] = bf2f((bf16_t)v[k]); mx = fmaxf(mx, f[k]); }
+  const float mn = fmaxf(m, mx);
+  float acc = 0.f;
+#pragma unroll
+  for (int k = 0; k < 8; ++k) acc += __expf(f[k] - mn);
+  s = s * __expf(m - mn) + acc;
+  m = mn;
+}
+
+__device__ __forceinline__ void ce_online1(const float f, float& m, float& s) {
+  const float mn = fmaxf(m, f);
+  s = s * __expf(m - mn) + __expf(f - mn);
+  m = mn;
+}
+
+__device__ __forceinline__ float ce_row_lse(const float m, const float s, float* red) {
+  const float M = block_max<4>(m, red);
+  const float part = (m == -INFINITY) ? 0.f : s * __expf(m - M);
+  const float S = block_sum<4>(part, red);
+  return M + logf(S);
+}
+
+__device__ __forceinline__ void ce_row_outputs(const bf16_t* x, int V, int row, float lse, const int64_t* labels, int64_t ignore_index,
+                                               float* lse_out, float* loss_row, float* logp_label) {
+  lse_out[row] = lse;
+  const int64_t lab = labels ? labels[row] : ignore_index;
+  float lr = 0.f, lp = 0.f;
+  if (lab != ignore_index && lab >= 0 && lab < V) { lp = bf2f(x[lab]) - lse; lr = -lp; }
+  if (loss_row) loss_row[row] = lr;
+  if (logp_label) logp_label[row] = lp;
+}
+
+__device__ __forceinline__ float ce_grad_diff(const float xf, const float lse, const bool is_label) {
+#pragma clang fp contract(off)
+  return __expf(xf - lse) - (is_label ? 1.f : 0.f);
+}
+__device__ __forceinline__ float ce_grad_elem(const float xf, const float lse, const bool is_label, const float sc) {
+#pragma clang fp contract(off)
+  return ce_grad_diff(xf, lse, is_label) * sc;
+}
 
 __global__ __launch_bounds__(256) void ce_fwd_kernel(const bf16_t* __restrict__ logits, int64_t ld, int V,
                                                      const int64_t* __restrict__ labels, int64_t ignore_index,
@@ -12,36 +56,10 @@
   const bf16_t* x = logits + (int64_t)row * ld;
   const int nv = V >> 3;
   float m = -INFINITY, s = 0.f;
-  for (int i = threadIdx.x; i < nv; i += 256) {
-    const bf16x8_t v = *reinterpret_cast<const bf16x8_t*>(x + i * 8);
-    float f[8], mx = -INFINITY;
-#pragma unroll
-    for (int k = 0; k < 8; ++k) { f[k] = bf2f((bf16_t)v[k]); mx = fmaxf(mx, f[k]); }
-    const float mn = fmaxf(m, mx);
-    float acc = 0.f;
-#pragma unroll
-    for (int k = 0; k < 8; ++k) acc += __expf(f[k] - mn);
-    s = s * __expf(m - mn) + acc;
-    m = mn;
-  }
-  for (int c = (nv << 3) + threadIdx.x; c < V; c += 256) {
-    const float f = bf2f(x[c]);
-    const float mn = fmaxf(m, f);
-    s = s * __expf(m - mn) + __expf(f - mn);
-    m = mn;
-  }
-  const float M = block_max<4>(m, red);
-  const float part = (m == -INFINITY) ? 0.f : s * __expf(m - M);
-  const float S = block_sum<4>(part, red);
-  if (threadIdx.x == 0) {
-    const float lse = M + logf(S);
-    lse_out[row] = lse;
-    const int64_t lab = labels ? labels[row] : ignore_index;
-    float lr = 0.f, lp = 0.f;
-    if (lab != ignore_index && lab >= 0 && lab < V) { lp = bf2f(x[lab]) - lse; lr = -lp; }
-    if (loss_row) loss_row[row] = lr;
-    if (logp_label) logp_label[row] = lp;
-  }
+  for (int i = threadIdx.x; i < nv; i += 256) ce_online8(*reinterpret_cast<const bf16x8_t*>(x + i * 8), m, s);
+  for (int c = (nv << 3) + threadIdx.x; c < V; c += 256) ce_online1(bf2f(x[c]), m, s);
+  const float lse = ce_row_lse(m, s, red);
+  if (threadIdx.x == 0) ce_row_outputs(x, V, row, lse, labels, ignore_index, lse_out, loss_row, logp_label);
 }
 
 __global__ __launch_bounds__(256) void ce_reduce_kernel(const float* __restrict__ loss_row,
@@ -74,13 +92,177 @@
     for (int k = 0; k < 8; ++k) {
       const int c = i * 8 + k;
       float g = 0.f;
-      if (valid && c < V) g = (__expf(bf2f((bf16_t)v[k]) - l) - (c == lab ? 1.f : 0.f)) * sc;
+      if (valid && c < V) g = ce_grad_elem(bf2f((bf16_t)v[k]), l, c == lab, sc);
       v[k] = (short)f2bf(g);
     }
     *reinterpret_cast<bf16x8_t*>(x + i * 8) = v;
   }
 }
 
+constexpr int CE_FUSED_PIECES = UG_CE_FUSED_MAX_LD / 8 / 256;
+constexpr int CE_FUSED_REG = 44, CE_FUSED_LDS = CE_FUSED_PIECES - CE_FUSED_REG;
+static_assert(CE_FUSED_PIECES * 8 * 256 == UG_CE_FUSED_MAX_LD, "the row limit is a whole number of pieces per thread");
+static_assert(CE_FUSED_LDS <= CE_FUSED_REG && CE_FUSED_LDS * 256 * 16 + 64 <= 160 * 1024, "LDS pieces are staged through the piece registers");
+
+__global__ __launch_bounds__(256) void ce_count_kernel(const int64_t* __restrict__ labels, int64_t ignore_index, int R,
+                                                       float* __restrict__ out, uint32_t* __restrict__ dmin) {
+  __shared__ float red[4];
+  float c = 0.f;
+  for (int i = threadIdx.x; i < R; i += 256) {
+    if (labels[i] != ignore_index) c += 1.f;
+  }
+  const float C = block_sum<4>(c, red);
+  if (threadIdx.x == 0) { out[1] = C; *dmin = 0x7f800000u; }
+}
+
+__device__ __forceinline__ bf16x8_t ce_fused_grad8(const bf16x8_t v, const float lse, const float sc, uint32_t& dm1) {
+  typedef uint32_t u32x4_t __attribute__((ext_vector_type(4)));
+  float g[8];
+#pragma unroll
+  for (int k = 0; k < 8; ++k) {
+    const float xf = bf2f((bf16_t)v[k]);
+    g[k] = ce_grad_elem(xf, lse, false, sc);
+    dm1 = min(dm1, __float_as_uint(ce_grad_diff(xf, lse, false)) - 1u);
+  }
+  const u32x4_t o = {pack_bf2(g[0], g[1]), pack_bf2(g[2], g[3]), pack_bf2(g[4], g[5]), pack_bf2(g[6], g[7])};
+  return __builtin_bit_cast(bf16x8_t, o);
+}
+
+__global__ __launch_bounds__(256) void ce_fused_kernel(bf16_t* __restrict__ logits, int64_t ld, int V,
+                                                       const int64_t* __restrict__ labels, int64_t ignore_index,
+                                                       float* __restrict__ lse_out, float* __restrict__ loss_row,
+                                                       const float* __restrict__ loss_cnt, uint32_t* __restrict__ dmin_out) {
+  __shared__ bf16x8_t held[CE_FUSED_LDS * 256];
+  __shared__ float red[4];
+  __shared__ uint32_t dmin_sh;
+  const int row = blockIdx.x, t = threadIdx.x;
+  bf16_t* x = logits + (int64_t)row * ld;
+  const int nv = V >> 3, nvp = (int)(ld >> 3);
+  bf16x8_t reg[CE_FUSED_REG];
+  const auto piece = [&](int i) { return *reinterpret_cast<const bf16x8_t*>(x + (i < nvp ? i : 0) * 8); };
+#pragma unroll
+  for (int j = 0; j < CE_FUSED_REG; ++j) reg[j] = piece(t + (j < CE_FUSED_LDS ? CE_FUSED_REG + j : j) * 256);
+  __builtin_amdgcn_sched_barrier(0);
+#pragma unroll
+  for (int j = 0; j < CE_FUSED_LDS; ++j) {
+    held[j * 256 + t] = reg[j];
+    reg[j] = piece(t + j * 256);
+    __builtin_amdgcn_sched_barrier(0);
+  }
+  if (t == 0) dmin_sh = 0x7f800000u;
+
+  float m = -INFINITY, s = 0.f;
+#pragma unroll
+  for (int j = 0; j < CE_FUSED_REG; ++j) {
+    float m2 = m, s2 = s;
+    ce_online8(reg[j], m2, s2);
+    const bool on = t + j * 256 < nv;
+    m = on ? m2 : m;
+    s = on ? s2 : s;
+    __builtin_amdgcn_sched_barrier(0);
+  }
+  for (int j = 0; t + (CE_FUSED_REG + j) * 256 < nv; ++j) ce_online8(held[j * 256 + t], m, s);
+  for (int c = (nv << 3) + t; c < V; c += 256) ce_online1(bf2f(x[c]), m, s);
+  const float lse = ce_row_lse(m, s, red);
+  const int64_t lab = labels[row];
+  const bool valid = (lab != ignore_index), has_label = valid && lab >= 0 && lab < V;
+  float xlab = 0.f;
+  if (t == 0) {
+    ce_row_outputs(x, V, row, lse, labels, ignore_index, lse_out, loss_row, nullptr);
+    if (has_label) xlab = bf2f(x[lab]);
+  }
+  __syncthreads();
+
+  if (!valid) {
+    const bf16x8_t z = {0, 0, 0, 0, 0, 0, 0, 0};
+    for (int i = t; i < nvp; i += 256) *reinterpret_cast<bf16x8_t*>(x + i * 8) = z;
+    return;
+  }
+  const float sc = 1.f / loss_cnt[1];
+  uint32_t dm1 = 0xffffffffu;
+#pragma unroll
+  for (int j = 0; j < CE_FUSED_REG; ++j) {
+    const int i = t + j * 256;
+    const bf16x8_t gv = ce_fused_grad8(reg[j], lse, sc, dm1);
+    if (i < nvp) *reinterpret_cast<bf16x8_t*>(x + i * 8) = gv;
+    __builtin_amdgcn_sched_barrier(0);
+  }
+  for (int j = 0; t + (CE_FUSED_REG + j) * 256 < nvp; ++j) {
+    const int i = t + (CE_FUSED_REG + j) * 256;
+    *reinterpret_cast<bf16x8_t*>(x + i * 8) = ce_fused_grad8(held[j * 256 + t], lse, sc, dm1);
+  }
+  uint32_t dmin = dm1 + 1u;
+  if (dmin == 0u || dmin > 0x7f800000u) dmin = 0x7f800000u;
+  __syncthreads();
+  for (int c = V + t; c < ld; c += 256) x[c] = 0;
+  if (t == 0) {
+    if (has_label) {
+      x[lab] = f2bf(ce_grad_elem(xlab, lse, true, sc));
+      const uint32_t db = __float_as_uint(ce_grad_diff(xlab, lse, true)) & 0x7fffffffu;
+      if (db) dmin = min(dmin, db);
+    }
+    if (!(fabsf(lse) < INFINITY)) dmin = 1u;
+  }
+  if (dmin != 0x7f800000u) atomicMin(&dmin_sh, dmin);
+  __syncthreads();
+  if (t == 0 && dmin_sh != 0x7f800000u) atomicMin(dmin_out, dmin_sh);
+}
+
+__global__ __launch_bounds__(256) void ce_gscale_kernel(bf16_t* __restrict__ logits, int64_t ld, const float* __restrict__ gp,
+                                                        const float* __restrict__ loss_cnt, const uint32_t* __restrict__ dmin,
+                                                        int* __restrict__ status, int status_bit) {
+  const float g = *gp;
+  if (g == 1.f) return;
+  const uint32_t gb = __float_as_uint(g), gf = gb >> 23;
+  bool ok = (gb & 0x007fffffu) == 0u && gf >= 1u && gf <= 227u;
+  if (ok && *dmin != 0x7f800000u) {
+    const int k = (int)gf - 127;
+    const int ed = (int)(*dmin >> 23) - 127;
+    const int es = (int)((__float_as_uint(1.f / loss_cnt[1]) >> 23) & 0xffu) - 127;
+    ok = ed + es >= -126 && ed + es + k >= -126;
+  }
+  bf16_t* x = logits + (int64_t)blockIdx.x * ld;
+  const int nvp = (int)(ld >> 3);
+  if (!ok && blockIdx.x == 0 && threadIdx.x == 0) atomicOr(status, status_bit);
+  for (int i = threadIdx.x; i < nvp; i += 256) {
+    bf16x8_t v;
+    if (ok) {
+      v = *reinterpret_cast<const bf16x8_t*>(x + i * 8);
+#pragma unroll
+      for (int q = 0; q < 8; ++q) v[q] = (short)f2bf(bf2f((bf16_t)v[q]) * g);
+    } else {
+#pragma unroll
+      for (int q = 0; q < 8; ++q) v[q] = (short)0x7fc0;
+    }
+    *reinterpret_cast<bf16x8_t*>(x + i * 8) = v;
+  }
+}
+
+}
+
+extern "C" int ug_ce_fused(void* logits_inout, int64_t ld, int64_t R, int64_t V, const int64_t* labels, int64_t ignore_index,
+                           float* lse, float* loss_row, float* loss_and_count, uint32_t* dmin, hipStream_t st) {
+  UG_REQUIRE(R > 0 && V > 0 && ld >= V && ld % 8 == 0, "ug_ce_fused: need ld>=V and ld%%8==0 (ld=%ld V=%ld)", (long)ld, (long)V);
+  UG_REQUIRE(ld <= UG_CE_FUSED_MAX_LD, "ug_ce_fused: a row of %ld logits does not fit the register array (limit %d): use ug_ce_fwd + ug_ce_bwd",
+             (long)ld, UG_CE_FUSED_MAX_LD);
+  UG_REQUIRE(ug_aligned16(logits_inout) && labels && lse && loss_row && loss_and_count && dmin, "ug_ce_fused: bad pointers");
+  hipLaunchKernelGGL(ce_count_kernel, dim3(1), dim3(256), 0, st, labels, ignore_index, (int)R, loss_and_count, dmin);
+  UG_CHECK_LAUNCH("ug_ce_fused(count)");
+  hipLaunchKernelGGL(ce_fused_kernel, dim3((unsigned)R), dim3(256), 0, st, (bf16_t*)logits_inout, ld, (int)V, labels, ignore_index,
+                     lse, loss_row, loss_and_count, dmin);
+  UG_CHECK_LAUNCH("ug_ce_fused");
+  hipLaunchKernelGGL(ce_reduce_kernel, dim3(1), dim3(256), 0, st, loss_row, labels, ignore_index, (int)R, loss_and_count);
+  UG_CHECK_LAUNCH("ug_ce_fused(reduce)");
+  return UG_OK;
+}
+
+extern "C" int ug_ce_gscale(void* grad_inout, int64_t ld, int64_t R, const float* g, const float* loss_and_count,
+                            const uint32_t* dmin, int* status, int status_bit, hipStream_t st) {
+  UG_REQUIRE(R > 0 && ld > 0 && ld % 8 == 0, "ug_ce_gscale: need ld%%8==0");
+  UG_REQUIRE(ug_aligned16(grad_inout) && g && loss_and_count && dmin && status, "ug_ce_gscale: bad pointers");
+  hipLaunchKernelGGL(ce_gscale_kernel, dim3((unsigned)R), dim3(256), 0, st, (bf16_t*)grad_inout, ld, g, loss_and_count, dmin, status, status_bit);
+  UG_CHECK_LAUNCH("ug_ce_gscale");
+  return UG_OK;
 }
 
 extern "C" int ug_ce_fwd(const void* logits, int64_t ld, int64_t R, int64_t V, const int64_t* labels,
diff --git a/ml-unigen_amd/models/unigen.py b/ml-unigen_amd/models/unigen.py
--- a/ml-unigen_amd/models/unigen.py
+++ b/ml-unigen_amd/models/unigen.py
@@ -693,7 +693,8 @@
                 r += ix.numel()
             idx = torch.cat([ix for ix, _ in segs]) if r > 0 else torch.zeros(0, dtype=torch.long, device=device)
             lab = torch.cat([ix + s for ix, s in segs]) if r > 0 else idx
-            self._loss_idx_cache[key] = (idx, lab, bounds)
+            rising = bool(r > 1 and (idx[1:] > idx[:-1]).all().item()) or r == 1
+            self._loss_idx_cache[key] = (idx, lab, bounds, rising)
         return self._loss_idx_cache[key]
 
     def forward(
@@ -731,14 +732,14 @@
             return LazyLogits(eng, hn)
         logits = LazyLogits(eng, hn.detach())
         B, L, _ = hn.shape
-        idx, lab_idx, bounds = self._loss_rows(B, L, batch_size_t2i, batch_size_lm, batch_size_mmu, num_vq_tokens,
-                                               t2i_mode, hn.device)
+        idx, lab_idx, bounds, rising = self._loss_rows(B, L, batch_size_t2i, batch_size_lm, batch_size_mmu, num_vq_tokens,
+                                                       t2i_mode, hn.device)
         nan = torch.full((), float("nan"), device=hn.device)
         if idx.numel() == 0:
             return logits, nan, 0., 0.
         lab = labels.to(hn.device).reshape(-1)[lab_idx].contiguous()
         live = [(s, b) for s, b in enumerate(bounds) if b[1] > b[0]]
-        losses = _HeadLossFn.apply(eng._anchor, hn, eng, idx, lab, tuple(b for _, b in live))
+        losses = _HeadLossFn.apply(eng._anchor, hn, eng, idx, lab, tuple(b for _, b in live), rising)
         by_seg = {s: losses[j] for j, (s, _) in enumerate(live)}
         s = 0
         loss_t2i = by_seg.get(s, nan)
@@ -767,10 +768,10 @@
         loss_t2i = _CrossEntropyFn.apply(lg.reshape(-1, C), lb.reshape(-1).contiguous())
         loss_lm, loss_mmu = 0., 0.
         if blm > 0 or bmmu > 0:
-            idx, lab_idx, bounds = self._loss_rows(B, L, 0, blm, bmmu, n, t2i_mode, hn.device, lm_start=bt)
+            idx, lab_idx, bounds, rising = self._loss_rows(B, L, 0, blm, bmmu, n, t2i_mode, hn.device, lm_start=bt)
             lab = labels.reshape(-1)[lab_idx].contiguous()
             live = [(s, b) for s, b in enumerate(bounds) if b[1] > b[0]]
-            losses = _HeadLossFn.apply(eng._anchor, hn, eng, idx, lab, tuple(b for _, b in live))
+            losses = _HeadLossFn.apply(eng._anchor, hn, eng, idx, lab, tuple(b for _, b in live), rising)
             by_seg = {s: losses[j] for j, (s, _) in enumerate(live)}
             s = 1
             if blm > 0:
diff --git a/ml-unigen_amd/unigen_hip/lib.py b/ml-unigen_amd/unigen_hip/lib.py
--- a/ml-unigen_amd/unigen_hip/lib.py
+++ b/ml-unigen_amd/unigen_hip/lib.py
@@ -23,6 +23,7 @@
     "ug_cast_f32_bf16": [P, P, I64, P],
     "ug_rmsnorm_fwd": [P, P, P, P, I64, I64, F32, I32, P],
     "ug_rmsnorm_bwd": [P, P, P, P, P, P, P, I64, I64, P],
+    "ug_rmsnorm_bwd_rows": [P, P, I64, P, P, P, P, P, P, I64, I64, P],
     "ug_rope": [P, P, P, I64, I64, I64, I32, I32, I32, P],
     "ug_swiglu_fwd": [P, P, I64, I64, P],
     "ug_swiglu_bwd": [P, P, P, I64, I64, P],
@@ -79,6 +80,8 @@
     "ug_decode_finish_resid_norm_ord": [P, I64, I64, P, P, P, I64, I64, F32, P, P, P],
     "ug_ce_fwd": [P, I64, I64, I64, P, I64, P, P, P, P, P],
     "ug_ce_bwd": [P, I64, I64, I64, P, I64, P, P, P, P, P],
+    "ug_ce_fused": [P, I64, I64, I64, P, I64, P, P, P, P, P],
+    "ug_ce_gscale": [P, I64, I64, P, P, P, P, I32, P],
     "ug_head_score_ws_bytes": [I64, I64],
     "ug_head_score": [P, I64, I64, P, I64, I64, I64, P, I64, P, P, P, P, P, P],
     "ug_adamw_flat": [P, P, P, P, P, I64, F32, F32, F32, F32, F32, I64, F32, I32, P],
diff --git a/ml-unigen_amd/unigen_hip/modules.py b/ml-unigen_amd/unigen_hip/modules.py
--- a/ml-unigen_amd/unigen_hip/modules.py
+++ b/ml-unigen_amd/unigen_hip/modules.py
@@ -56,6 +56,7 @@
         h_last, hn, rstd = engine.stack_fwd(h0.reshape(B * L, H).float().contiguous(), mb, L, saved)
         if need:
             ctx.engine, ctx.saved, ctx.h_last, ctx.rstd, ctx.mb, ctx.shape = engine, saved, h_last, rstd, mb, (B, L, H)
+            ctx.token = engine._stack_token_out = object()
         return hn.view(B, L, H)
 
     @staticmethod
@@ -67,28 +68,64 @@
         eng._stack_graphs_live = max(0, eng._stack_graphs_live - 1)
         if eng.grad_sync is not None:
             eng.grad_sync.set_overlap(last_writer)
-        dhn = dhn.reshape(B * L, H).to(torch.bfloat16).contiguous()
-        dh0 = eng.stack_bwd(ctx.saved, ctx.h_last, ctx.rstd, dhn, ctx.mb, L)
+        sparse = eng.__dict__.setdefault("_sparse_dhn", {}).pop(ctx.token, None)
+        if sparse is not None and sparse[0].data_ptr() == dhn.data_ptr() and dhn.stride() == sparse[0].stride():
+            dh0 = eng.stack_bwd(ctx.saved, ctx.h_last, ctx.rstd, None, ctx.mb, L, dhn_rows=sparse[1:])
+        else:
+            dhn = dhn.reshape(B * L, H).to(torch.bfloat16).contiguous()
+            if sparse is not None:
+                dhn = dhn.clone().index_add_(0, sparse[2], sparse[1])
+            dh0 = eng.stack_bwd(ctx.saved, ctx.h_last, ctx.rstd, dhn, ctx.mb, L)
         ctx.saved = None
         danchor = torch.zeros_like(anchor_of(eng)) if ctx.needs_input_grad[0] else None
         return danchor, dh0.view(B, L, H), None, None
 
 
+CE_DECLINED_FLAG = 8
+
+
+def _ce_upstream(ctx, dloss):
+    eng, V = ctx.engine, ctx.engine.dims.vocab_size
+    learn = getattr(eng, "_ce_g_mode", None) is None
+    if learn:
+        status = torch.zeros(1, dtype=torch.int32, device=dloss.device)
+    for s, (r0, r1) in enumerate(ctx.bounds):
+        _, lc, dmin = ctx.stats[s]
+        ops.ce_gscale_(ctx.logits[r0:r1], dloss[s:s + 1], lc, dmin, status if learn else eng.err_flag, 1 if learn else CE_DECLINED_FLAG)
+    if not learn:
+        return
+    if int(status.item()) == 0:
+        eng._ce_g_mode = "fused"
+        return
+    eng._ce_g_mode = "plain"
+    ctx.logits = None
+    ctx.logits = eng.logits_rows(ctx.rows)
+    for s, (r0, r1) in enumerate(ctx.bounds):
+        lse, lc, _ = ctx.stats[s]
+        ops.ce_bwd_(ctx.logits[r0:r1], V, ctx.labels[r0:r1], lse, lc, dloss[s:s + 1])
+
+
 class _HeadLossFn(torch.autograd.Function):
 
     @staticmethod
-    def forward(ctx, anchor, hn, engine, idx, labels, bounds):
+    def forward(ctx, anchor, hn, engine, idx, labels, bounds, rows_rising=False):
         B, L, H = hn.shape
         V = engine.dims.vocab_size
         rows = ops.gather_rows(hn.reshape(B * L, H), idx)
         logits = engine.logits_rows(rows)
+        ctx.fused = (ops.CE_FUSED and any(ctx.needs_input_grad) and logits.stride(0) <= ops.CE_FUSED_MAX_LD
+                     and getattr(engine, "_ce_g_mode", None) != "plain")
         outs, stats = [], []
         for (r0, r1) in bounds:
-            lc, lse, _, _ = ops.ce_fwd(logits[r0:r1], V, labels[r0:r1])
+            if ctx.fused:
+                lc, lse, _, dmin = ops.ce_fused_(logits[r0:r1], V, labels[r0:r1])
+            else:
+                (lc, lse, _, _), dmin = ops.ce_fwd(logits[r0:r1], V, labels[r0:r1]), None
             outs.append(lc[:1])
-            stats.append((lse, lc))
+            stats.append((lse, lc, dmin))
         ctx.engine, ctx.rows, ctx.logits, ctx.idx, ctx.labels, ctx.bounds, ctx.stats = engine, rows, logits, idx, labels, bounds, stats
         ctx.shape = (B, L, H)
+        ctx.stack_token = getattr(hn, "_ug_stack_token", None) if rows_rising and ops.norm_rows_pays(idx.numel(), B * L) else None
         if any(ctx.needs_input_grad):
             engine._head_graphs_live += 1
         return torch.cat(outs)
@@ -100,15 +137,26 @@
         V = eng.dims.vocab_size
         eng.begin_grad_pass()
         dloss = dloss.float().contiguous()
-        for s, (r0, r1) in enumerate(ctx.bounds):
-            lse, lc = ctx.stats[s]
-            ops.ce_bwd_(ctx.logits[r0:r1], V, ctx.labels[r0:r1], lse, lc, dloss[s:s + 1])
+        if ctx.fused:
+            _ce_upstream(ctx, dloss)
+        else:
+            for s, (r0, r1) in enumerate(ctx.bounds):
+                lse, lc, _ = ctx.stats[s]
+                ops.ce_bwd_(ctx.logits[r0:r1], V, ctx.labels[r0:r1], lse, lc, dloss[s:s + 1])
         drows = eng.head_bwd(ctx.logits, ctx.rows)
         eng.head_written()
         ctx.logits = None
+        if ctx.stack_token is not None:
+            return None, _row_sparse_dhn(eng, ctx.stack_token, drows, ctx.idx, (B, L, H)), None, None, None, None, None
         dhn = torch.zeros((B * L, H), dtype=torch.bfloat16, device=drows.device)
         ops.scatter_rows_(drows, ctx.idx, dhn)
-        return None, dhn.view(B, L, H), None, None, None, None
+        return None, dhn.view(B, L, H), None, None, None, None, None
+
+
+def _row_sparse_dhn(eng, token, drows, idx, shape):
+    marker = torch.zeros((1, 1, 1), dtype=torch.bfloat16, device=drows.device).expand(*shape)
+    eng.__dict__.setdefault("_sparse_dhn", {})[token] = (marker, drows, idx)
+    return marker
 
 
 class _HeadRowsFn(torch.autograd.Function):
@@ -284,7 +332,9 @@
             inputs_embeds = self.embed_tokens(input_ids)
         B, L, _ = inputs_embeds.shape
         mb = eng.mask_bits(attention_mask, B, L)
+        eng._stack_token_out = None
         hn = _StackFn.apply(eng._anchor, inputs_embeds, eng, mb)
+        hn._ug_stack_token = eng._stack_token_out
         return SimpleNamespace(last_hidden_state=hn, past_key_values=None)
 
 
@@ -406,6 +456,7 @@
 
     def _forward_entry(self):
         self._in_backward = False
+        self.__dict__.get("_sparse_dhn", {}).clear()
         return self._dp_sync()
 
     def _sync_this_pass(self):
@@ -420,6 +471,7 @@
 
     def _end_of_backward(self):
         self._in_backward = False
+        self.__dict__.get("_sparse_dhn", {}).clear()
         self._stack_graphs_live = 0
         self._head_graphs_live = 0
         self._lookup_rows_live = 0
diff --git a/ml-unigen_amd/unigen_hip/ops.py b/ml-unigen_amd/unigen_hip/ops.py
--- a/ml-unigen_amd/unigen_hip/ops.py
+++ b/ml-unigen_amd/unigen_hip/ops.py
@@ -213,6 +213,29 @@
     _l.check(_l.load().ug_rmsnorm_bwd(_p(dy), _p(x), _p(rstd), _p(w), _p(dres), _p(dw), _p(out), rows, cols, _stream()),
              "ug_rmsnorm_bwd")
     return out
+
+
+NORM_ROWS = __import__("os").environ.get("UNIGEN_NORM_ROWS", "1") == "1"
+
+
+def norm_rows_pays(R, M):
+    return NORM_ROWS and 2 * R < M
+
+
+def rmsnorm_bwd_rows(dy_rows, idx, x, rstd, w, dw):
+    M, cols = x.shape
+    R = idx.numel()
+    if not norm_rows_pays(R, M):
+        dy = torch.zeros((M, cols), dtype=torch.bfloat16, device=x.device)
+        if R:
+            scatter_rows_(dy_rows, idx, dy)
+        dres = torch.zeros_like(x)
+        return dres, rmsnorm_bwd(dy, x, rstd, w, dres, dw, want_bf16=True)
+    dres = torch.empty_like(x)
+    out = torch.empty((M, cols), dtype=torch.bfloat16, device=x.device)
+    _l.check(_l.load().ug_rmsnorm_bwd_rows(_p(dy_rows) if R else None, _p(idx) if R else None, R, _p(x), _p(rstd), _p(w), _p(dres),
+                                           _p(dw), _p(out), M, cols, _stream()), "ug_rmsnorm_bwd_rows")
+    return dres, out
 
 
 def rope_inv_freq(head_dim, theta, scaling=None, seq_len=None):
@@ -860,6 +883,30 @@
     return logits
 
 
+CE_FUSED = __import__("os").environ.get("UNIGEN_CE_FUSED", "1") == "1"
+CE_FUSED_MAX_LD = 163840
+
+
+def ce_fused_(logits, V, labels, ignore_index=-100):
+    R, ld = logits.shape[0], logits.stride(0)
+    if ld > CE_FUSED_MAX_LD:
+        raise _l.UniGenHipError(f"ce_fused_: rows of {ld} logits exceed the fused kernel's {CE_FUSED_MAX_LD}; use ce_fwd + ce_bwd_")
+    dev = logits.device
+    lse = torch.empty((R,), dtype=torch.float32, device=dev)
+    loss_row = torch.empty((R,), dtype=torch.float32, device=dev)
+    lc = torch.empty((2,), dtype=torch.float32, device=dev)
+    dmin = torch.empty((1,), dtype=torch.int32, device=dev)
+    _l.check(_l.load().ug_ce_fused(_p(logits), ld, R, V, _p(labels), ignore_index, _p(lse), _p(loss_row), _p(lc), _p(dmin),
+                                   _stream()), "ug_ce_fused")
+    return lc, lse, loss_row, dmin
+
+
+def ce_gscale_(grad, g, lc, dmin, status, status_bit=1):
+    R, ld = grad.shape[0], grad.stride(0)
+    _l.check(_l.load().ug_ce_gscale(_p(grad), ld, R, _p(g), _p(lc), _p(dmin), _p(status), status_bit, _stream()), "ug_ce_gscale")
+    return grad
+
+
 _HEAD_SCORE_WS = {}
 HEAD_SCORE_WANT = ("lse", "best", "best_logit")
 
diff --git a/ml-unigen_amd/unigen_hip/qwen2.py b/ml-unigen_amd/unigen_hip/qwen2.py
--- a/ml-unigen_amd/unigen_hip/qwen2.py
+++ b/ml-unigen_amd/unigen_hip/qwen2.py
@@ -344,7 +344,9 @@
         if v:
             self.err_flag.zero_()
             raise UniGenHipError(f"device-side input check failed (flags={v}): 1=token id out of range, "
-                                 f"2=attention mask value neither 0 nor <= -1e9, 4=VQ code out of range")
+                                 f"2=attention mask value neither 0 nor <= -1e9, 4=VQ code out of range, 8=the upstream gradient of "
+                                 f"a loss changed to a value that is no power of two after the fused cross entropy had been chosen "
+                                 f"(that step's gradients are NaN; run with UNIGEN_CE_FUSED=0)")
 
     def layer_fwd(self, i, h, mb, L, save):
         d, fp = self.dims, self.fp
@@ -428,9 +430,12 @@
         ops.gemm_wgrad_group([w_gu, w_down, w_qkv, w_o] + self._head_wgrad_slice())
         return dh, dnext
 
-    def stack_bwd(self, saved, h_last, rstd_last, dhn, mb, L):
-        dh = torch.zeros_like(h_last)
-        dh16 = ops.rmsnorm_bwd(dhn, h_last, rstd_last, self.fp.p("norm"), dh, self.fp.g("norm"), want_bf16=True)
+    def stack_bwd(self, saved, h_last, rstd_last, dhn, mb, L, dhn_rows=None):
+        if dhn_rows is not None:
+            dh, dh16 = ops.rmsnorm_bwd_rows(dhn_rows[0], dhn_rows[1], h_last, rstd_last, self.fp.p("norm"), self.fp.g("norm"))
+        else:
+            dh = torch.zeros_like(h_last)
+            dh16 = ops.rmsnorm_bwd(dhn, h_last, rstd_last, self.fp.p("norm"), dh, self.fp.g("norm"), want_bf16=True)
         if self.grad_ready_hook:
             self.grad_ready_hook("norm")
         for i in reversed(range(self.dims.num_hidden_layers)):
```

New measurement: 125.0 (median of 3 runs). Within noise of the previous version (+0.0%).
